# Psy-Fer/SquiggleKit

Hardware: AMD Instinct MI355X
Metric: reads/sec MotifSeq DTW (4k-sample read x 200-sample motif) (higher is better)
Workload: dtype f64 results; u32 fixed-point screening

## Files before the change

squigglekit_amd/csrc/sk_common.h:

```cpp
#pragma once
#include <hip/hip_runtime.h>
#include <stdint.h>
#include <stddef.h>
#include <stdarg.h>
#include <vector>
#include "squigglekit_hip.h"

#define SK_MAX_DEVICES 16
#define SK_WAVE 64

struct sk_prep {
    int32_t n;
    int32_t flags;
    double  center;
    double  scale;
    double  top;
    double  bot;
};

#define SK_IFLAG_INPLACE 0x100
#define SK_FLAG_PUBLIC   0xff

enum sk_prep_mode { SK_PREP_MEDMAD = 0, SK_PREP_ZSCALE = 1, SK_PREP_SEGMENT = 2, SK_PREP_DRNA = 3 };

enum sk_redo_route { SK_REDO_NONE = 0, SK_REDO_I16 = 1, SK_REDO_F64 = 2, SK_REDO_PA = 3 };

struct sk_buf {
    void  *p = nullptr;
    size_t cap = 0;
};

struct sk_panel_motif {
    int32_t xoff;
    int32_t P;
    int32_t k;
    int32_t pad;
};
struct sk_panel_group {
    int32_t L, R;
    int32_t first, count;
};

struct sk_pair_entry {
    int64_t toff;
    int64_t xoff;
    int32_t n;
    int32_t P;
    int32_t pair;
    int32_t pad;
};
struct sk_pair_query {
    int64_t src, xoff;
    int32_t N, L, R, pad;
};

struct sk_map_entry {
    int64_t toff;
    int64_t xoff;
    int64_t soff;
    int32_t n;
    int32_t P;
    int32_t rec;
    int32_t cont;
};

struct sk_rowhit_entry {
    int64_t col0;
    int64_t list;
    int32_t n;
    int32_t flags;
};
#define SK_ROWHIT_NOROW 0x100

struct sk_pairpath_entry {
    int64_t qoff, toff;
    int64_t span_off;
    int32_t N, M;
};

struct sk_band_entry {
    int64_t qoff, toff;
    int64_t span_off;
    int32_t N, M;
    int32_t pair, pad;
};

struct sk_ctx {
    int         device = -1;
    bool        ready = false;
    hipStream_t stream = nullptr;
    hipStream_t stream2 = nullptr;
    hipStream_t stream3 = nullptr;
    hipEvent_t  ev_r[2] = {nullptr, nullptr};
    hipStream_t stream4 = nullptr;
    hipEvent_t  ev_a = nullptr;
    hipEvent_t  ev_s[2] = {nullptr, nullptr};
    uint32_t    dtw_sparse_calls = 0;
    uint32_t    dtw_audit_calls = 0;
    hipEvent_t  ev_chunk[9] = {};
    hipEvent_t  ev[4] = {nullptr, nullptr, nullptr, nullptr};
    bool        ev_valid = false;
    int         num_cu = 0;
    sk_buf sig;
    sk_buf len;
    sk_buf rlen;
    sk_buf off;
    sk_buf comp;
    sk_buf prep;
    sk_buf mask;
    sk_buf motif;
    sk_buf out;
    sk_buf out2;
    sk_buf misc;
    sk_buf seghints;
    sk_buf pacal;
    sk_buf pull;
    sk_buf pulltext;
    sk_buf sweep;
    sk_buf sweeprec;
    sk_buf hitrows;
    sk_buf bgrec;
    sk_buf pathcnt;
    bool   path_valid = false;
    sk_buf pathlist;
    sk_buf pathscratch;
    sk_buf pathmotif;
    sk_buf pathspans;
    sk_buf events;
    sk_buf poolev;
    sk_buf pool;
    sk_buf panel;
    sk_buf panelwin;
    sk_buf panelaux;
    sk_buf panelrec;
    sk_buf seglev;
    sk_buf seglevwork;
    sk_buf detect;
    sk_buf detectout;
    sk_buf hmm;
    sk_buf hmmpath;
    sk_buf hmmseg;
    sk_buf hmmpost;
    sk_buf hmmpostout;
    std::vector<double> panel_host;
    std::vector<sk_panel_motif> panel_table;
    std::vector<sk_panel_group> panel_groups;
    std::vector<int32_t> panel_long;
    sk_buf pairs;
    sk_buf pairsval;
    std::vector<sk_pair_query> pairs_query;
    std::vector<sk_pair_entry> pairs_table;
    sk_buf rowhit;
    std::vector<sk_rowhit_entry> rowhit_table;
    std::vector<sk_map_entry>    pairhits_sweep;
    int64_t pairhits_row_bytes = 0, pairhits_slices = 0, pairhits_long_rows = 0;
    sk_buf pairpath;
    std::vector<sk_pairpath_entry> pairpath_table;
    int64_t pairpath_listed = 0, pairpath_slab_bytes = 0, pairpath_waves = 0;
    sk_buf band;
    sk_buf bandslab;
    std::vector<sk_band_entry> band_table;
    int64_t band_slab_bytes = 0, band_waves = 0, band_steps = 0;
    sk_buf ckpt;
    sk_buf motifq;
    sk_buf motif64;
    bool   motif64_valid = false;
    std::vector<double> motif64_host;
    sk_buf lastq;
    sk_buf qflag;
    sk_buf wsoft;
    sk_buf lsum;
    sk_buf wstate;
    sk_buf wrec;
    sk_buf wrecq;
    sk_buf order;
    sk_buf motifw;
    std::vector<double> motifw_host;
    int    motifq_L = 0;
    sk_buf retry;
    sk_buf dtwcnt;
    sk_buf audit;
    sk_buf sib;
    sk_buf sibout;
    sk_buf sibstate;
    bool   retry_dev = false;
    std::vector<unsigned> motifq_host;
    bool   motifq_valid = false;
    sk_buf redo;
    int    redo_route = SK_REDO_NONE;
    std::vector<size_t> redo_off;
    size_t redo_used = 0;
    std::vector<int64_t> pa_off_host;
    int    last_retry = 0;
    std::vector<hipEvent_t> evpool;
    int    prof_chunks = 0;
    int    prof_reads[64] = {0};
    std::vector<double> motif_host;
    std::vector<double> motif_src;
    int    motif_L = 0;
    void  *comm = nullptr;
    void  *sessions[SK_STREAM_MAX_SESSIONS] = {};
    void  *map_sessions[SK_MAP_MAX_SESSIONS] = {};
    int64_t map_state_bytes = 0, map_entries = 0, map_launches = 0;
    void  *evs_sessions[SK_EVS_MAX_SESSIONS] = {};
    sk_buf evscnt;
    int64_t evs_state_bytes = 0, evs_staged = 0;
    bool   evs_valid = false;
    void  *hmms_sessions[SK_HMMS_MAX_SESSIONS] = {};
    sk_buf hmmscnt;
    int64_t hmms_state_bytes = 0;
    bool   hmms_valid = false;
    void  *live_sessions[SK_LIVE_MAX_SESSIONS] = {};
    int64_t live_state_bytes = 0, live_levels = 0, live_launches = 0;
    sk_buf commbuf;
    sk_buf pile;
    sk_buf pileent;
    sk_buf pilealt;
    sk_buf pilein;
    sk_buf pileout;
    int64_t pile_entries = 0, pile_longest = 0, pile_long_lists = 0, pile_scratch_bytes = 0;
};

const char *sk_tune(const char *name);

struct sk_entry {
    sk_ctx *c = nullptr;
    sk_entry();
    explicit sk_entry(int slot);
    ~sk_entry();
    sk_entry(const sk_entry &) = delete;
    sk_entry &operator=(const sk_entry &) = delete;
};
#define SK_ENTER(c)                                                                     \
    sk_entry c##_entry_;                                                                \
    sk_ctx *const c = c##_entry_.c;                                                     \
    if (!c) return SK_ERR_NO_DEVICE
sk_ctx *sk_ctx_of(int device);
int  sk_bound_device(void);
int  sk_fail(int code, const char *fmt, ...);
int  sk_reserve(sk_ctx *c, sk_buf *b, size_t bytes);
int  sk_second_stream(sk_ctx *c);
int64_t sk_dtw_chunk_reads(size_t per_read, int64_t nreads);
void    sk_dtw_scratch_shrink(int reset);
#define SK_HIP(call)                                                                    \
    do {                                                                                \
        hipError_t e_ = (call);                                                         \
        if (e_ != hipSuccess)                                                           \
            return sk_fail(SK_ERR_HIP, "%s failed: %s (%s:%d)", #call,                 \
                           hipGetErrorString(e_), __FILE__, __LINE__);                  \
    } while (0)

int sk_launch_prep_i16(sk_ctx *c, const int16_t *d_sig, int64_t stride, const int32_t *d_len,
                       int32_t nreads, int32_t lo, int32_t hi, int mode, double std_scale,
                       int16_t *d_comp, sk_prep *d_prep, uint64_t *d_mask, int64_t mask_stride,
                       int32_t t0 = 0, int32_t t1 = 0x7fffffff,
                       const int32_t *d_list = nullptr, const int32_t *d_count = nullptr,
                       void *d_mask2 = nullptr, int row16 = 0);
int sk_launch_prepw_medmad(sk_ctx *c, const int16_t *d_sig, int64_t stride, const int32_t *d_len,
                           int32_t nreads, int32_t lo, int32_t hi, int16_t *d_comp, sk_prep *d_prep);
int sk_launch_prep_f64(sk_ctx *c, const double *d_sig, const int64_t *d_off, int32_t nreads,
                       double lo, double hi, int mode, double std_scale,
                       double *d_comp, sk_prep *d_prep, void *d_mask2 = nullptr, int row16 = 0,
                       int32_t *d_len_out = nullptr,
                       const int32_t *d_rlen = nullptr);

enum sk_feed { SK_FEED_I16 = 0,
               SK_FEED_F64_NORM = 1,
               SK_FEED_F64_RAW = 2 };
struct sk_prep_fuse {
    const int16_t *raw = nullptr;
    const int32_t *len = nullptr;
    int32_t lo = 0, hi = 0;
    int     mode = SK_PREP_MEDMAD;
};
bool sk_sdtw_fuse_ok(int32_t lo, int32_t hi, int mode = SK_PREP_MEDMAD, int64_t stride = 0);

struct sk_sdtw_args {
    int           feed;
    const void   *samples;
    int64_t       stride;
    const int64_t *off;
    const sk_prep *prep;
    int32_t       nreads;
    const double *motif;
    int32_t       nmotif;
    sk_hit       *out;
    double       *last_row;
    int64_t       max_len;
    int           force_single;
    int           accumulate = 0;
    const void   *samples_raw = nullptr;
    const sk_prep_fuse *fuse = nullptr;
};
int sk_launch_sdtw(sk_ctx *c, const sk_sdtw_args *a);
void sk_exact_shape(int N, int64_t count, int *L, int *R);
int sk_launch_sdtw_panel(sk_ctx *c, const sk_sdtw_args *a, int L, int R, const double *d_xlay, const sk_panel_motif *d_mt,
                         int32_t count, sk_hit *d_all, int64_t out_stride);
int sk_launch_sdtw_pairs(sk_ctx *c, int L, int R, int global, const double *d_values, const double *d_xlay,
                         const sk_pair_entry *d_pt, int32_t count, sk_hit *d_out);
int sk_launch_sdtw_map(sk_ctx *c, int L, int R, const double *d_targets, const double *d_xlay, const sk_map_entry *d_mp,
                       int32_t count, double *stD, int32_t *stS, sk_hit *d_last);
int sk_launch_pairs_layout(sk_ctx *c, const double *d_values, const sk_pair_query *d_qt, int nq, double *d_lay);
int sk_pairs_check(const int64_t *off, int32_t nseq, const sk_pair *pairs, int64_t npairs, int32_t mode, const void *out);
int sk_pairs_run(sk_ctx *c, const double *d_values, const int64_t *off, int64_t off0, int32_t nseq, const sk_pair *pairs,
                 int64_t npairs, int32_t mode, sk_hit *d_out);
int sk_pair_paths_run(sk_ctx *c, const double *d_values, const int64_t *off, int64_t off0, int32_t nseq, const sk_pair *pairs,
                      int64_t npairs, int32_t mode, sk_hit *d_rec, int32_t have_records, int32_t *d_spans);
int sk_launch_sdtw_rows(sk_ctx *c, const sk_sdtw_args *a, double *rowD, int32_t *rowS);
int sk_launch_hits_select(sk_ctx *c, const double *rowD, const int32_t *rowS, int64_t row_stride, const sk_hit *rec,
                          int32_t nreads, int32_t K, double max_dist, sk_hit *out, int32_t *count);
int sk_rowhits_reserve(sk_ctx *c, int64_t nrows);
int sk_launch_rowhits(sk_ctx *c, sk_rowhit_entry *tab, int64_t at, int32_t nrows, const double *rowD, const int32_t *rowS,
                      int32_t K, double max_dist, sk_hit *out, int32_t *count, int64_t *long_rows);
int sk_pairs_hits_run(sk_ctx *c, const double *d_values, const int64_t *off, int64_t off0, int32_t nseq, const sk_pair *pairs,
                      int64_t npairs, int32_t K, double max_dist, sk_hit *d_out, int32_t *d_count);
int sk_launch_row_background(sk_ctx *c, const double *rowD, int64_t row_stride, const sk_hit *rec, int32_t nreads,
                             sk_bg_rec *out);
struct sk_path_args {
    int            feed;
    const void    *samples;
    const void    *samples_raw = nullptr;
    int64_t        stride = 0;
    const int64_t *off = nullptr;
    const sk_prep *prep = nullptr;
    int32_t        nreads = 0;
    int64_t        max_len = 0;
    const double  *d_motif = nullptr;
    int32_t        nmotif = 0;
    const sk_hit  *hits = nullptr;
    int32_t        K = 1;
    int32_t       *spans = nullptr;
};
int sk_path_begin(sk_ctx *c);
int sk_launch_paths(sk_ctx *c, const sk_path_args *p);
int sk_launch_events(sk_ctx *c, const sk_path_args *p, sk_event *events);
int sk_launch_events_pool(sk_ctx *c, const sk_event *d_ev, const uint8_t *d_use, int64_t nhits, int32_t N,
                          int32_t *d_idx, int32_t *d_cnt, sk_pool_rec *d_out);
int sk_launch_sdtw_screen(sk_ctx *c, const sk_sdtw_args *a, int ck, int span, int span2,
                          int32_t *d_retry_cnt, int32_t *d_retry, int32_t *d_early_cnt, int32_t *d_early);

int sk_band_check(const int64_t *off, int32_t nseq, const sk_pair *pairs, int64_t npairs, int32_t band, int32_t end_mode,
                  const void *out);
int sk_band_run(sk_ctx *c, const double *d_values, const int64_t *off, int64_t off0, int32_t nseq, const sk_pair *pairs,
                int64_t npairs, int32_t band, int32_t end_mode, sk_hit *d_rec, int32_t *d_spans);

__host__ __device__ static inline void sk_slice_indices(int32_t len, int32_t begin, int32_t end, int32_t *lo, int32_t *hi, int *clamped = nullptr)
{
    int64_t s = begin, e = end;
    int cl = 0;
    if (s < 0) { s += len; if (s < 0) { s = 0; cl |= 1; } } else if (s > len) { s = len; cl |= 1; }
    if (e < 0) { e += len; if (e < 0) { e = 0; cl |= 2; } } else if (e > len) { e = len; cl |= 2; }
    *lo = (int32_t)s; *hi = (int32_t)e;
    if (clamped) *clamped = cl;
}
int sk_launch_region_rows_i16(sk_ctx *c, const int16_t *d_sig, int64_t stride, const int32_t *d_len, int32_t nreads,
                              int32_t begin, int32_t end, const int32_t *d_win, int16_t *d_rows, int64_t wstride,
                              int32_t *d_wlen, int32_t *d_from);
int sk_launch_region_rows_f64(sk_ctx *c, const double *d_sig, const int64_t *d_src, const int64_t *d_woff, int32_t nreads,
                              double *d_out);
int sk_panel_plan(sk_ctx *c, const double *motifs, const int32_t *motif_off, int32_t nmotifs, const double *mean,
                  const double *sd, int64_t pairs);
int sk_launch_panel_dtw(sk_ctx *c, const sk_sdtw_args *base, const double *motifs, const int32_t *motif_off,
                        sk_hit *d_all, int64_t out_stride);
int sk_launch_panel_rank(sk_ctx *c, const sk_hit *d_all, int64_t out_stride, int32_t nreads, int32_t nmotifs,
                         sk_panel_rec *d_out);

struct sk_roll_params;
bool sk_roll_stream_ok(int64_t stride, int32_t w, int32_t lo, int32_t hi);
int sk_launch_roll_stream(sk_ctx *c, const int16_t *d_sig, int64_t stride, const int32_t *d_len, int32_t nreads, int32_t lo,
                          int32_t hi, int32_t w, double std_scale, sk_prep *d_prep, uint64_t *d_below, uint64_t *d_above,
                          int32_t *d_redo );
size_t sk_roll_one_lds(int64_t stride, int32_t w);
int sk_launch_roll_one(sk_ctx *c, const int16_t *d_sig, int64_t stride, const int32_t *d_len, int32_t nreads, int32_t lo,
                       int32_t hi, int32_t w, double std_scale, sk_prep *d_prep, uint64_t *d_below, uint64_t *d_above);
int sk_launch_roll_stats(sk_ctx *c, const int16_t *d_comp, int64_t stride, sk_prep *d_prep, int32_t nreads,
                         int32_t w, double std_scale, int64_t *d_psum, uint64_t *d_below, uint64_t *d_above);
int sk_launch_roll_walk(sk_ctx *c, const uint64_t *d_below, const uint64_t *d_above, const sk_prep *d_prep,
                        int32_t nreads, const sk_roll_params *p, int32_t *d_xy, int32_t *d_found, int64_t row_words = 0);

int  sk_segment_fast_row16(int64_t stride);
bool sk_segment_fast_applies(const void *d_sig, int64_t stride, int32_t lo, int32_t hi, double std_scale);
int  sk_launch_segment_fast(sk_ctx *c, const int16_t *d_sig, int64_t stride, const int32_t *d_len, int32_t nreads,
                            const sk_seg_params *p, int32_t lo, int32_t hi, sk_prep *d_prep, void *d_mask2,
                            int32_t *d_retry, int32_t *d_segs, int32_t *d_nsegs, int32_t max_segs,
                            const double *d_cal = nullptr, double *d_scratch = nullptr);
bool sk_segment_pa_applies(const void *d_sig, int64_t stride, double std_scale);
int  sk_launch_prep_pa_listed(sk_ctx *c, const int16_t *d_sig, int64_t stride, const int32_t *d_len, const double *d_cal,
                              const int32_t *d_list, const int32_t *d_count, int grid, double lo, double hi, double std_scale,
                              double *d_scratch, int64_t scratch_stride, sk_prep *d_prep, void *d_mask2, int row16);

int  sk_launch_segment_masks(sk_ctx *c, const int16_t *d_sig, int64_t stride, const int32_t *d_len, int32_t nreads,
                             double std_scale, int32_t lo, int32_t hi, sk_prep *d_prep, void *d_mask2, int32_t *d_retry);

struct sk_sweep_lane {
    int32_t error, corrector, window, seg_dist, first_len, stall_start, gap_dist, index;
};
struct sk_sweep_group {
    int32_t rep, first, nfast, ngen;
};
void sk_sweep_plan(const sk_seg_sweep_set *sets, int32_t nsets, std::vector<sk_sweep_group> &groups,
                   std::vector<sk_sweep_lane> &lanes);
int  sk_launch_seg_sweep_walk(sk_ctx *c, const void *d_mask2, int row16, const int32_t *d_len, int64_t mmax, int32_t nreads,
                              const sk_sweep_lane *d_lanes, int32_t nlanes, bool fast, sk_seg_sweep_sum *d_sums,
                              sk_seg_sweep_rec *d_recs, int64_t rec_stride);

struct sk_drna_params;
int sk_launch_drna_walk(sk_ctx *c, const uint64_t *d_mask, int64_t mask_rows, const sk_prep *d_prep,
                        int32_t nreads, const sk_drna_params *p, int32_t *d_segs, int32_t *d_nsegs,
                        int32_t max_segs);

int sk_launch_synth(sk_ctx *c, int16_t *d_sig, int64_t stride, int32_t nreads, int32_t nsamples,
                    uint64_t seed, const int16_t *d_motif_i16, int32_t nmotif, int64_t row0 = 0,
                    int hit_pm = 500, int stretch_pm = 0, int stretch = 1);
int sk_launch_synth_windows(sk_ctx *c, int16_t *d_sig, int64_t stride, int32_t nreads, int32_t nsamples,
                            uint64_t seed, int64_t row0, const int16_t *d_tmpl, int32_t ntmpl, float sigma);
int sk_launch_raw_to_pa(sk_ctx *c, const int16_t *d_sig, int64_t stride, int32_t nreads, int32_t nsamples,
                        double offset, double raw_unit, double *d_out, int64_t *d_off);
int sk_launch_centi_to_f64(sk_ctx *c, const int32_t *d_centi, int64_t total, double *d_out);
int sk_launch_rows_to_pa(sk_ctx *c, const int16_t *d_sig, int64_t stride, int32_t nreads, const int64_t *d_off,
                         const double *d_cal, double *d_out);

bool sk_f64_fast_applies(int64_t maxlen, double std_scale);
int  sk_f64_row16(int64_t maxlen);
int  sk_launch_f64_stats(sk_ctx *c, const double *d_sig, const int64_t *d_off, const int32_t *d_rlen, int32_t nreads, int64_t maxlen,
                         double lo, double hi, int mode, double std_scale, sk_prep *d_prep, void *d_mask2, int row16,
                         int32_t *d_len, int32_t *d_retry, double *d_comp);
int  sk_launch_prep_f64_listed(sk_ctx *c, const double *d_sig, const int64_t *d_off, const int32_t *d_list,
                               const int32_t *d_count, int grid, double lo, double hi, int mode, double std_scale,
                               double *d_comp_or_scratch, int64_t scratch_stride, sk_prep *d_prep, void *d_mask2,
                               int row16, const int32_t *d_rlen = nullptr);
int  sk_launch_seg_walk_masks(sk_ctx *c, const void *d_mask2, int row16, const int32_t *d_len, int32_t nreads,
                              const sk_seg_params *p, int32_t *d_segs, int32_t *d_nsegs, int32_t max_segs);

size_t sk_seglev_work_bytes(sk_ctx *c, int32_t nreads, int32_t max_segs, int64_t mmax);
int sk_launch_seg_levels(sk_ctx *c, int feed, const void *samples, int64_t stride, const int64_t *d_off,
                         const void *d_mask2, int row16, const int32_t *d_len, int64_t mmax, int32_t nreads,
                         const int32_t *d_segs, const int32_t *d_nsegs, int32_t max_segs, void *d_work,
                         sk_seg_level *levels, sk_seg_level *read_level);

int64_t sk_detect_words(int64_t stride);
size_t  sk_detect_work_bytes(int32_t nreads, int64_t stride);
int sk_launch_detect_mark(sk_ctx *c, const int16_t *d_sig, int64_t stride, const int32_t *d_len, int32_t nreads,
                          const sk_det_params *p, void *d_words, int64_t *d_cnt);
int sk_launch_detect_scan(sk_ctx *c, int32_t nreads, int64_t *d_bsum, int64_t *d_off);
int sk_launch_detect_fill(sk_ctx *c, const int16_t *d_sig, int64_t stride, const int32_t *d_len, int32_t nreads,
                          const sk_det_params *p, const void *d_words, const int64_t *d_off, sk_det_event *d_rec, int64_t cap);

__host__ __device__ static inline double sk_raw_to_pa(double raw, double offset, double unit)
{
    const double x = raw + offset;
    return x * unit;
}
const char *sk_hmm_model_error(const sk_hmm_model *m);
int sk_launch_hmm_i16(sk_ctx *c, const int16_t *d_sig, int64_t stride, const int32_t *d_len, int32_t nreads,
                      const double *d_cal, const sk_hmm_model *m, int32_t limit, sk_hmm_rec *d_rec);
int sk_launch_hmm_f64(sk_ctx *c, const double *d_values, const int64_t *d_off, int32_t nreads, const sk_hmm_model *m,
                      int32_t limit, sk_hmm_rec *d_rec);
int64_t sk_hmm_npad(int64_t maxlen, int32_t limit);
int64_t sk_hmm_slice_groups(int32_t nreads, int64_t npad);
size_t  sk_hmm_path_work_bytes(int32_t nreads, int64_t npad);
int sk_launch_hmm_paths(sk_ctx *c, int feed, const void *d_sig, int64_t stride, const int32_t *d_len, const int64_t *d_roff,
                        int32_t nreads, const double *d_cal, const sk_hmm_model *m, int32_t limit, int64_t npad, void *d_work,
                        int first, sk_hmm_rec *d_rec, int64_t *d_off, sk_hmm_seg *d_seg, int64_t cap);
int sk_launch_hmm_stats(sk_ctx *c, int feed, const void *d_sig, int64_t stride, const int64_t *d_roff, int32_t nreads,
                        const double *d_cal, const sk_hmm_model *m, const int64_t *d_off, void *d_seg, int64_t cap);

size_t sk_hmm_post_work_bytes(int32_t nreads, int64_t npad);
int sk_launch_hmm_post(sk_ctx *c, int feed, const void *d_sig, int64_t stride, const int32_t *d_len, const int64_t *d_roff,
                       int32_t nreads, const double *d_cal, const sk_hmm_model *m, int32_t limit, int64_t npad, void *d_work,
                       sk_hmm_post *d_post, sk_hmm_counts *d_counts, const int64_t *d_goff, double *d_gamma);

int sk_stream_session_open(sk_ctx *c, const double *motifs, const int32_t *motif_off, int32_t nmotifs,
                           const sk_stream_params *p, int32_t *handle);
int sk_stream_session_info(sk_ctx *c, int32_t handle, int32_t *nslots, int32_t *nmotifs);
int sk_stream_session_push(sk_ctx *c, int32_t handle, const int32_t *d_slots, int32_t m, const int16_t *d_rows,
                           int64_t stride, const int32_t *d_len, int flush, sk_stream_rec *d_out);
int sk_stream_session_reset(sk_ctx *c, int32_t handle, const int32_t *d_slots, int32_t m, const double *d_center,
                            const double *d_scale);
int sk_stream_session_stage(sk_ctx *c, int32_t handle, int which, size_t bytes, void **p);
int sk_stream_session_close(sk_ctx *c, int32_t handle);
void sk_stream_close_all(sk_ctx *c);

int sk_map_session_open(sk_ctx *c, const double *targets, const int64_t *target_off, int32_t ntargets, int32_t nslots,
                        int32_t *handle);
int sk_map_session_info(sk_ctx *c, int32_t handle, int32_t *nslots, int32_t *ntargets);
int sk_map_session_check_slots(sk_ctx *c, int32_t handle, const int32_t *slots, int32_t m);
int sk_map_session_push(sk_ctx *c, int32_t handle, const int32_t *slots, int32_t m, const double *d_values,
                        const int64_t *off, sk_map_rec *d_out);
int sk_map_session_reset(sk_ctx *c, int32_t handle, const int32_t *slots, int32_t m);
int sk_map_session_hits(sk_ctx *c, int32_t handle, const int32_t *slots, int32_t m, int32_t K, double max_dist, sk_hit *d_out,
                        int32_t *d_count);
int sk_map_session_stage(sk_ctx *c, int32_t handle, int which, size_t bytes, void **p);
int sk_map_session_close(sk_ctx *c, int32_t handle);
void sk_map_close_all(sk_ctx *c);

int64_t sk_evs_session_rows(sk_ctx *c, int32_t handle, int64_t maxlen);
int sk_evs_session_open(sk_ctx *c, const sk_det_params *p, int32_t nslots, int32_t *handle);
int sk_evs_session_info(sk_ctx *c, int32_t handle, int32_t *nslots);
int sk_evs_session_check(sk_ctx *c, int32_t handle, const int32_t *slots, int32_t m, const int32_t *len);
int sk_evs_session_check_cap(sk_ctx *c, int32_t handle, const int32_t *slots, int32_t m, const int32_t *len, int64_t cap);
int sk_evs_session_stage(sk_ctx *c, int32_t handle, int which, size_t bytes, void **p);
int sk_evs_session_push(sk_ctx *c, int32_t handle, const int32_t *d_slots, int32_t m, const int16_t *d_rows, int64_t stride,
                        const int32_t *d_len, const int32_t *d_end, int64_t per, int64_t *d_off, const int32_t *host_slots,
                        const int32_t *host_len, const int32_t *host_end);
int sk_evs_session_gather(sk_ctx *c, int32_t handle, sk_det_event *d_rec, int64_t cap);
int sk_evs_session_last(sk_ctx *c, int32_t handle, const int64_t **d_off, int32_t *m);
int sk_evs_session_staging(sk_ctx *c, int32_t handle, const sk_det_event **d_stage, int64_t *per);
int sk_evs_session_reset(sk_ctx *c, int32_t handle, const int32_t *slots, int32_t m);
int sk_evs_session_close(sk_ctx *c, int32_t handle);
void sk_evs_close_all(sk_ctx *c);

#define SK_HMMS_CAP 0x7fffff00
void sk_hmms_close_all(sk_ctx *c);
int sk_hmms_session_open(sk_ctx *c, const sk_hmm_model *model, int32_t nslots, int32_t *handle);
int sk_hmms_session_push_dev_i16(sk_ctx *c, int32_t handle, const int32_t *d_slots, int32_t m, const int16_t *d_rows,
                                 int64_t stride, const int32_t *d_len, sk_hmms_rec *d_out);
int sk_hmms_session_reset_dev(sk_ctx *c, int32_t handle, const int32_t *d_slots, int32_t m, const double *d_cal2);
int64_t sk_hmms_session_bytes(sk_ctx *c, int32_t handle);
int sk_hmms_session_close(sk_ctx *c, int32_t handle);

int sk_live_session_open(sk_ctx *c, const sk_det_params *p, int32_t calib, const double *targets, const int64_t *target_off,
                         int32_t ntargets, int32_t nslots, const sk_hmm_model *model ,
                         const sk_live_gate *gate, int32_t *handle);
int sk_live_session_info(sk_ctx *c, int32_t handle, int32_t *nslots, int32_t *ntargets, int32_t *evs, int32_t *map);
int sk_live_session_gate_last(sk_ctx *c, int32_t handle, const sk_live_gate_info **d_gate, const sk_hmms_rec **d_rec, int32_t *m);
int sk_live_session_check(sk_ctx *c, int32_t handle, const int32_t *slots, int32_t m, int64_t stride, const int32_t *len);
int sk_live_session_stage(sk_ctx *c, int32_t handle, int which, size_t bytes, void **p);
int sk_live_session_push(sk_ctx *c, int32_t handle, const int32_t *host_slots, const int32_t *d_slots, int32_t m,
                         const int16_t *d_rows, int64_t stride, const int32_t *d_len, const int32_t *d_end, int64_t per,
                         const int32_t *host_len, const int32_t *host_end, const sk_live_rule *rule, sk_map_rec *d_out,
                         sk_live_info *d_info, sk_live_best *d_best);
int sk_live_session_last(sk_ctx *c, int32_t handle, const int64_t **d_off, const double **d_values, int32_t *m);
int sk_live_session_best_ms(sk_ctx *c, int32_t handle, float *ms);
int sk_live_session_gate_ms(sk_ctx *c, int32_t handle, float *hmm_ms, float *gate_ms);
int sk_live_session_reset(sk_ctx *c, int32_t handle, const int32_t *slots, int32_t m, const double *cal2 );
int sk_live_session_close(sk_ctx *c, int32_t handle);
void sk_live_close_all(sk_ctx *c);

struct sk_gate_slot {
    sk_live_gate_info g;
    int32_t last_drop;
    int32_t pad;
};
struct sk_gate_args {
    sk_gate_slot        *state;
    sk_det_event        *ring;
    const sk_live_info  *live;
    int32_t              nslots, G;
    const int32_t       *slots;
    int32_t              m;
    const int32_t       *len, *end;
    const sk_hmms_rec   *hrec;
    const sk_det_event  *stage;
    int64_t              per;
    const int64_t       *eoff;
    sk_det_event        *rel;
    int64_t             *rcnt;
    sk_live_gate_info   *ginfo;
    sk_live_gate         rule;
};
int sk_livegate_reset(sk_ctx *c, sk_gate_slot *state, int32_t nslots, const int32_t *d_slots, int32_t m);
int sk_livegate_lengths(sk_ctx *c, const sk_gate_args &a, int32_t *d_hlen);
int sk_livegate_release(sk_ctx *c, const sk_gate_args &a);

int sk_pileup_run(sk_ctx *c, const int64_t *d_span_off, const int32_t *d_spans, const double *d_value, const int32_t *d_dwell,
                  const int32_t *d_target, const int32_t *d_shift, const uint8_t *d_use, int32_t npairs, int64_t nrows,
                  const int64_t *tlen, int32_t ntargets, sk_pile_rec *d_out, int64_t *d_ent_off, int32_t *d_ent_row,
                  int64_t ent_cap);

int64_t sk_scan_blocks(int64_t n);
int     sk_launch_scan_i64(sk_ctx *c, const int64_t *v, int64_t n, int64_t *bsum, int64_t *out);
int64_t sk_pull_tile_cap(int32_t nreads, int64_t stride);
int sk_launch_pull_count(sk_ctx *c, const int16_t *d_sig, int64_t stride, const int32_t *d_len, int32_t nreads,
                         const double *d_cal, const int64_t *d_poff, int64_t *d_tile0, int64_t *d_tb, int64_t tile_cap,
                         int64_t *d_bsum, int64_t *d_line_off, int32_t *d_err);
int sk_launch_pull_write(sk_ctx *c, const int16_t *d_sig, int64_t stride, const int32_t *d_len, int32_t nreads,
                         const double *d_cal, const char *d_prefix, const int64_t *d_poff, const int64_t *d_tile0,
                         const int64_t *d_tb, int64_t tile_cap, const int64_t *d_line_off, char *d_out);
```

squigglekit_amd/csrc/sk_runtime.hip:

```cpp
#include "sk_common.h"
#include <string>
#include <string.h>
#include <mutex>
#include <stdio.h>
#include <stdlib.h>
#include <string.h>

static thread_local char  g_err[512] = "";
static thread_local int   g_cur = -1;
static sk_ctx             g_ctx[SK_MAX_DEVICES];
static std::mutex         g_mu;
static std::recursive_mutex g_ctx_mu[SK_MAX_DEVICES];

int sk_fail(int code, const char *fmt, ...)
{
    va_list ap;
    va_start(ap, fmt);
    vsnprintf(g_err, sizeof g_err, fmt, ap);
    va_end(ap);
    return code;
}

sk_entry::sk_entry() : sk_entry(g_cur) {}

sk_entry::sk_entry(int slot)
{
    if (slot >= 0 && slot < SK_MAX_DEVICES) {
        g_ctx_mu[slot].lock();
        sk_ctx *ctx = &g_ctx[slot];
        if (ctx->ready) {
            if (hipSetDevice(ctx->device) == hipSuccess) { c = ctx; return; }
            sk_fail(SK_ERR_NO_DEVICE, "hipSetDevice(%d) failed", ctx->device);
            g_ctx_mu[slot].unlock();
            return;
        }
        g_ctx_mu[slot].unlock();
    }
    sk_fail(SK_ERR_NO_DEVICE, "no device bound: call sk_init(device) first (no CPU fallback exists)");
}

sk_entry::~sk_entry() { if (c) g_ctx_mu[c - g_ctx].unlock(); }

sk_ctx *sk_ctx_of(int device) { return (device >= 0 && device < SK_MAX_DEVICES) ? &g_ctx[device] : nullptr; }
int sk_bound_device(void) { return g_cur; }

int sk_reserve(sk_ctx *c, sk_buf *b, size_t bytes)
{
    (void)c;
    if (bytes <= b->cap) return SK_OK;
    if (b->p) { SK_HIP(hipFree(b->p)); b->p = nullptr; b->cap = 0; }
    size_t want = bytes + bytes / 8 + 256;
    hipError_t e = hipMalloc(&b->p, want);
    if (e != hipSuccess) {
        b->p = nullptr;
        return sk_fail(SK_ERR_NOMEM, "hipMalloc(%zu) failed: %s", want, hipGetErrorString(e));
    }
    b->cap = want;
    return SK_OK;
}

int sk_second_stream(sk_ctx *c)
{
    if (!c->stream2) {
        SK_HIP(hipStreamCreateWithFlags(&c->stream2, hipStreamNonBlocking));
        for (int i = 0; i < 9; i++) SK_HIP(hipEventCreateWithFlags(&c->ev_chunk[i], hipEventDisableTiming));
    }
    return SK_OK;
}

struct sk_tunable { const char *name, *test_values, *what; };
static const sk_tunable SK_TUNABLES[] = {
    {"SK_DTW_SCHEME",         "full exact2", "DTW scheme: full = one exact pass, exact2 = two exact passes (default: fixed-point screening + certified window)"},
    {"SK_DTW_QL",             "8 16 64",     "lanes per read of the screening scheme (default: by motif length and batch size)"},
    {"SK_DTW_NOFUSE",         "1",           "filter + medmad as their own kernel instead of the screening pass's prologue"},
    {"SK_DTW_FORCE_RETRY_PM", "100 1000",    "per-mille of reads sent through the exact retry whatever the window pass certified (sensitivity runs)"},
    {"SK_DTW_SPAN",           "150 300",     "look-back of the window pass in columns (one tier)"},
    {"SK_DTW_SPAN2",          "0 500",       "look-back of the window pass's second tier (0: none)"},
    {"SK_DTW_CK",             "64 256",      "steps between checkpoints of the screening pass (multiple of 64)"},
    {"SK_DTW_NOSORT",         "1",           "window passes take the reads in file order"},
    {"SK_DTW_NOHINT",         "1",           "no start hint: the plain screening sweep, every read's exact window looks back the same number of columns"},
    {"SK_DTW_HINT_MIN",       "1",           "the start hint is on for calls of at least this many reads (default 500000)"},
    {"SK_DTW_SORT_MIN",       "1",           "window passes sort chunks of at least this many reads"},
    {"SK_DTW_NO_EARLY",       "1",           "no early exact retry beside the window passes"},
    {"SK_DTW_NO_SIBLINGS",    "1",           "reads whose candidate columns fall into two clusters take the exact pass (no second window)"},
    {"SK_DTW_NOGUARD",        "1",           "screening scheme without its run-time guard (premise test in the window pass, audit, gated exact fallback): A/B cost runs"},
    {"SK_DTW_AUDIT_PERIOD",   "0 1 64",      "the audit re-runs one read in this many with the exact pass (default 4096; 0: no audit)"},
    {"SK_DTW_HOLE",           "qerr1 fma64 fma64x", "tests: a known precision hole put back (E = 1; the fma sample image for float64 reads, with / without the image-error guard) -- the guard has to notice and the records must not change"},
    {"SK_DTW_SCRATCH_MB",     "8 64",        "checkpoint scratch budget in MB (small values force many chunks)"},
    {"SK_DTW_NO_SMALL",       "1",           "small batches keep the batch lane layout"},
    {"SK_DTW_SMALL_MAX",      "0 100000",    "largest batch that spreads a read over 64 lanes"},
    {"SK_PREP_BLOCK",         "1",           "medmad statistics by the workgroup-per-read kernel"},
    {"SK_PREP_ROUNDS",        "1 3",         "grid rounds of the persistent statistics kernels"},
    {"SK_PREP_PERCU",         "1 2",         "workgroups per CU of the persistent statistics kernels"},
    {"SK_SEG_OLD",            "1",           "segmenter: numpy-order statistics kernels for every read"},
    {"SK_SEG_DELTA_SCALE",    "1e13",        "segmenter: certification margin multiplier (large: every read takes the numpy-order redo)"},
    {"SK_SEG_PA_F64",         "1",           "segmenter, raw reads through the pA conversion: expand to float64 and take the float64 kernels instead of the raw-domain kernel"},
    {"SK_SEG_NO_WG",          "1",           "segmenter, reads of 4 097 .. 65 536 samples: the wavefront-per-read statistics kernel (two looks at a read) instead of the workgroup-per-read one"},
    {"SK_SEG_WG_ALL",         "1",           "segmenter: the workgroup-per-read statistics kernel for every row of 4 097 .. 65 536 samples (default: where it is faster)"},
    {"SK_SEG_OCC",            "7 8",         "segmenter statistics kernel: waves per SIMD the registers are sized for"},
    {"SK_SEG_CHUNKS",         "2 8",         "segmenter: chunks of a large batch (walk of one beside the statistics of the next)"},
    {"SK_WALK_GENERAL",       "1",           "segmenter walk: general step (corrector test live)"},
    {"SK_WALK_SYNC",          "1",           "segmenter walk: run hopping with the 64 lanes of a wavefront on the same word (k_seg_walk3)"},
    {"SK_WALK_OWNPASS",       "1",           "segmenter walk: finds the quiet stretches and anchors in a pass of its own instead of taking the statistics kernel's hints"},
    {"SK_WALK_NOJUMP",        "1",           "segmenter walk: every run is hopped through, no jumps between the stretches of quiet entries"},
    {"SK_WALK_NOWAVE",        "1",           "segmenter walk: a lane per read also for long rows / small batches (no wavefront-per-read walk)"},
    {"SK_WALK_WAVE_MAXREADS", "0 1000000",   "segmenter walk: batches of up to this many reads take the wavefront-per-read walk (default: 16384, 131072 for rows beyond 4 096 samples)"},
    {"SK_DRNA_STEP",          "1",           "dRNA_segmenter, both branches: the per-sample scans instead of the scans by runs / by transitions"},
    {"SK_ROLL_TWO_KERNELS",   "1",           "dRNA_segmenter rolling-mean branch: filter kernel + prefix sums through HBM instead of the one-look kernel (prefix sums in LDS)"},
    {"SK_ROLL_ONE_LOOK",      "1",           "dRNA_segmenter rolling-mean branch: the workgroup-per-read kernel in numpy's order for every read instead of the streaming kernel with certified thresholds"},
    {"SK_ROLL_DELTA_SCALE",   "1e13",        "dRNA_segmenter rolling-mean branch: multiplier of the certification margin (large: every read is redone in numpy's order)"},
    {"SK_HITS_ROW_BYTES",     "1000000",     "hit lists: bytes of the last-row buffer (12 B per column and read; default 2 GiB; small values force many chunks of reads)"},
    {"SK_ROWHITS_ONE_WAVE",   "1",           "pair / session hit lists: rows beyond 4 096 columns through one wavefront each instead of a workgroup of 16 (A/B runs)"},
    {"SK_PANEL_EXACT",        "1",           "motif panel: the one-grid exact kernel also for long windows over many reads (default: those take the screening scheme, one launch set per motif)"},
    {"SK_PATH_LDS_BYTES",     "0",           "alignment paths: bytes of direction words a hit may keep in LDS (default and most 25600; 0: every hit takes the scratch tier)"},
    {"SK_PATH_SCRATCH_BYTES", "1000000",     "alignment paths: byte budget of the scratch tier's slabs (default 1 GiB; small values leave one wavefront)"},
    {"SK_BAND_WAVES",         "1",           "adaptive-band DTW: wavefronts of the launch (default: one per pair up to what the device holds at a time and the slab budget; 1: one wavefront with one slab works through the list)"},
    {"SK_PILE_LDS_ENTRIES",   "64",          "reference pile-up: entries of a point's list that are put in order inside one wavefront's LDS (default and most 4096, at least 2; longer lists take the merge tier)"},
    {"SK_INGEST_MB",          "1 4",        "sub-batch size of the host entry points in MB"},
    {"SK_HMM_SCRATCH_MB",     "1",           "signal HMM state paths and posteriors: scratch budget in MB (default 16384; small values force slices of one or two 64-read groups)"},
    {"SK_HMM_POST_BLOCK",     "256",         "signal HMM posteriors: samples between alpha checkpoints, a multiple of 128 (default 128)"},
    {"SK_F64_OLD",            "1",           "float64 reads: numpy-order statistics kernel for every read"},
    {"SK_F64_LONG_LOOKS",     "1",           "float64 reads of 4 097 .. 40 960 samples: the window-by-window kernel (three to five looks at a read) instead of the workgroup-per-read one (one look)"},
};

const char *sk_tune(const char *name)
{
    const char *on = getenv("SK_TUNING");
    if (!on || on[0] != '1') return nullptr;
    for (const sk_tunable &t : SK_TUNABLES)
        if (strcmp(t.name, name) == 0) return getenv(name);
    return nullptr;
}

static thread_local int g_dtw_shrink = 0;
void sk_dtw_scratch_shrink(int reset) { g_dtw_shrink = reset ? 0 : (g_dtw_shrink < 12 ? g_dtw_shrink + 1 : 12); }

int64_t sk_dtw_chunk_reads(size_t per_read, int64_t nreads)
{
    size_t budget = (size_t)64 << 30;
    int64_t floor_reads = 1024;
    if (const char *e = sk_tune("SK_DTW_SCRATCH_MB")) {
        const long v = atol(e);
        if (v > 0) { budget = (size_t)v << 20; floor_reads = 64; }
    }
    budget >>= g_dtw_shrink;
    int64_t chunk = (int64_t)(budget / (per_read ? per_read : 1));
    if (chunk < floor_reads) chunk = floor_reads;
    if (chunk > nreads) chunk = nreads;
    return chunk > 0 ? chunk : 1;
}

extern "C" {

int sk_tunables(char *buf, int cap)
{
    std::string out;
    for (const sk_tunable &t : SK_TUNABLES) { out += t.name; out += '\t'; out += t.test_values; out += '\t'; out += t.what; out += '\n'; }
    if (buf && cap > 0) { const size_t n = out.size() < (size_t)cap - 1 ? out.size() : (size_t)cap - 1; memcpy(buf, out.data(), n); buf[n] = 0; }
    return (int)out.size() + 1;
}

const char *sk_version(void) { return "squigglekit-hip 0.1.0 (gfx950)"; }
const char *sk_last_error(void) { return g_err; }

int sk_device_count(void)
{
    int n = 0;
    hipError_t e = hipGetDeviceCount(&n);
    if (e != hipSuccess) {
        sk_fail(SK_ERR_NO_DEVICE, "hipGetDeviceCount: %s", hipGetErrorString(e));
        return 0;
    }
    return n;
}

int sk_init(int device) { return sk_init_slot(device, device); }

int sk_init_slot(int slot, int device)
{
    int n = sk_device_count();
    if (n <= 0) return sk_fail(SK_ERR_NO_DEVICE, "no HIP device visible (this library has no CPU fallback)");
    if (device < 0 || device >= n || device >= SK_MAX_DEVICES)
        return sk_fail(SK_ERR_INVALID, "device %d out of range (0..%d)", device, n - 1);
    if (slot < 0 || slot >= SK_MAX_DEVICES)
        return sk_fail(SK_ERR_INVALID, "context slot %d out of range (0..%d)", slot, SK_MAX_DEVICES - 1);
    std::lock_guard<std::mutex> lk(g_mu);
    sk_ctx *c = &g_ctx[slot];
    std::lock_guard<std::recursive_mutex> c_lock(g_ctx_mu[slot]);
    if (c->ready && c->device != device)
        return sk_fail(SK_ERR_INVALID, "context slot %d already serves device %d", slot, c->device);
    SK_HIP(hipSetDevice(device));
    if (!c->ready) {
        hipDeviceProp_t prop;
        SK_HIP(hipGetDeviceProperties(&prop, device));
        if (strncmp(prop.gcnArchName, "gfx950", 6) != 0)
            return sk_fail(SK_ERR_NO_DEVICE, "device %d is %s; this build targets gfx950 only",
                           device, prop.gcnArchName);
        c->device = device;
        c->num_cu = prop.multiProcessorCount;
        SK_HIP(hipStreamCreateWithFlags(&c->stream, hipStreamNonBlocking));
        for (int i = 0; i < 4; i++) SK_HIP(hipEventCreate(&c->ev[i]));
        c->ready = true;
    }
    g_cur = slot;
    return SK_OK;
}

static void free_buf(sk_buf *b) { if (b->p) (void)hipFree(b->p); b->p = nullptr; b->cap = 0; }

int sk_shutdown(void)
{
    std::lock_guard<std::mutex> lk(g_mu);
    for (int d = 0; d < SK_MAX_DEVICES; d++) {
        sk_ctx *c = &g_ctx[d];
        std::lock_guard<std::recursive_mutex> c_lock(g_ctx_mu[d]);
        if (!c->ready) continue;
        (void)hipSetDevice(c->device);
        (void)hipStreamSynchronize(c->stream);
        sk_stream_close_all(c);
        sk_live_close_all(c);
        sk_map_close_all(c);
        sk_evs_close_all(c);
        sk_hmms_close_all(c);
        sk_buf *bufs[] = {&c->sig, &c->len, &c->off, &c->comp, &c->prep, &c->mask,
                          &c->motif, &c->out, &c->out2, &c->misc, &c->ckpt, &c->retry, &c->motifq, &c->lastq, &c->qflag,
                          &c->motif64, &c->commbuf, &c->dtwcnt, &c->wsoft, &c->wstate, &c->wrec, &c->motifw, &c->lsum, &c->wrecq, &c->order, &c->pacal, &c->seghints, &c->audit, &c->rlen, &c->redo, &c->sib, &c->sibout, &c->sibstate, &c->pull, &c->pulltext, &c->sweep, &c->sweeprec, &c->hitrows, &c->bgrec, &c->pathcnt, &c->pathlist, &c->pathscratch, &c->pathmotif, &c->pathspans, &c->events, &c->poolev, &c->pool, &c->panel, &c->panelwin, &c->panelaux, &c->panelrec, &c->seglev, &c->seglevwork, &c->detect, &c->detectout, &c->hmm, &c->hmmpath, &c->hmmseg, &c->hmmpost, &c->hmmpostout, &c->pairs, &c->pairsval, &c->pairpath, &c->rowhit, &c->band, &c->bandslab, &c->evscnt, &c->hmmscnt,
                          &c->pile, &c->pileent, &c->pilealt, &c->pilein, &c->pileout};
        for (sk_buf *b : bufs) free_buf(b);
        for (int i = 0; i < 4; i++) (void)hipEventDestroy(c->ev[i]);
        for (hipEvent_t e : c->evpool) (void)hipEventDestroy(e);
        if (c->stream2) {
            (void)hipStreamSynchronize(c->stream2);
            for (int i = 0; i < 9; i++) if (c->ev_chunk[i]) (void)hipEventDestroy(c->ev_chunk[i]);
            (void)hipStreamDestroy(c->stream2);
        }
        if (c->stream3) {
            (void)hipStreamSynchronize(c->stream3);
            for (int i = 0; i < 2; i++) if (c->ev_r[i]) (void)hipEventDestroy(c->ev_r[i]);
            (void)hipStreamDestroy(c->stream3);
        }
        for (int i = 0; i < 2; i++) if (c->ev_s[i]) (void)hipEventDestroy(c->ev_s[i]);
        if (c->stream4) {
            (void)hipStreamSynchronize(c->stream4);
            if (c->ev_a) (void)hipEventDestroy(c->ev_a);
            (void)hipStreamDestroy(c->stream4);
        }
        (void)hipStreamDestroy(c->stream);
        *c = sk_ctx();
    }
    g_cur = -1;
    return SK_OK;
}

int sk_sync(void)
{
    SK_ENTER(c);
    SK_HIP(hipStreamSynchronize(c->stream));
    return SK_OK;
}

int sk_device_name(char *buf, int cap)
{
    SK_ENTER(c);
    if (!buf || cap <= 0) return sk_fail(SK_ERR_INVALID, "bad buffer");
    hipDeviceProp_t prop;
    SK_HIP(hipGetDeviceProperties(&prop, c->device));
    snprintf(buf, (size_t)cap, "%s (%s, %d CUs)", prop.name, prop.gcnArchName, prop.multiProcessorCount);
    return SK_OK;
}

int sk_device_pci_bus_id(char *buf, int cap)
{
    SK_ENTER(c);
    if (!buf || cap < 16) return sk_fail(SK_ERR_INVALID, "bad buffer");
    SK_HIP(hipDeviceGetPCIBusId(buf, cap, c->device));
    return SK_OK;
}

void *sk_dev_alloc(size_t bytes)
{
    sk_entry entry;
    if (!entry.c) return nullptr;
    void *p = nullptr;
    hipError_t e = hipMalloc(&p, bytes ? bytes : 1);
    if (e != hipSuccess) {
        sk_fail(SK_ERR_NOMEM, "hipMalloc(%zu) failed: %s", bytes, hipGetErrorString(e));
        return nullptr;
    }
    return p;
}

int sk_dev_free(void *dptr)
{
    SK_ENTER(c);
    if (dptr) SK_HIP(hipFree(dptr));
    return SK_OK;
}

int sk_dev_upload(void *dst_dev, const void *src_host, size_t bytes)
{
    SK_ENTER(c);
    if (bytes && (!dst_dev || !src_host)) return sk_fail(SK_ERR_INVALID, "NULL pointer");
    SK_HIP(hipMemcpyAsync(dst_dev, src_host, bytes, hipMemcpyHostToDevice, c->stream));
    SK_HIP(hipStreamSynchronize(c->stream));
    return SK_OK;
}

int sk_dev_download(void *dst_host, const void *src_dev, size_t bytes)
{
    SK_ENTER(c);
    if (bytes && (!dst_host || !src_dev)) return sk_fail(SK_ERR_INVALID, "NULL pointer");
    SK_HIP(hipMemcpyAsync(dst_host, src_dev, bytes, hipMemcpyDeviceToHost, c->stream));
    SK_HIP(hipStreamSynchronize(c->stream));
    return SK_OK;
}

int sk_last_kernel_ms(float *prep_ms, float *main_ms)
{
    SK_ENTER(c);
    if (!c->ev_valid) return sk_fail(SK_ERR_INVALID, "no timed call yet");
    SK_HIP(hipEventSynchronize(c->ev[3]));
    float a = 0.f, b = 0.f;
    SK_HIP(hipEventElapsedTime(&a, c->ev[0], c->ev[1]));
    SK_HIP(hipEventElapsedTime(&b, c->ev[2], c->ev[3]));
    if (prep_ms) *prep_ms = a;
    if (main_ms) *main_ms = b;
    return SK_OK;
}

int sk_last_dtw_profile(float *dist_ms, int *dist_launches, float *start_ms, int *start_launches,
                        int *reads_per_launch)
{
    SK_ENTER(c);
    float a = 0.f, b = 0.f;
    int mx = 0;
    for (int i = 0; i < c->prof_chunks; i++) {
        hipEvent_t *ev = &c->evpool[3 * (size_t)i];
        SK_HIP(hipEventSynchronize(ev[2]));
        float t = 0.f;
        SK_HIP(hipEventElapsedTime(&t, ev[0], ev[1])); a += t;
        SK_HIP(hipEventElapsedTime(&t, ev[1], ev[2])); b += t;
        const int rr = c->prof_reads[i < 64 ? i : 63];
        if (rr > mx) mx = rr;
    }
    if (dist_ms) *dist_ms = a;
    if (start_ms) *start_ms = b;
    if (dist_launches) *dist_launches = c->prof_chunks;
    if (start_launches) *start_launches = c->prof_chunks;
    if (reads_per_launch) *reads_per_launch = mx;
    return SK_OK;
}

int sk_last_dtw_retries(void)
{
    SK_ENTER(c);
    if (c->retry_dev && c->dtwcnt.p) {
        int32_t n = 0;
        if (hipMemcpyAsync(&n, c->dtwcnt.p, sizeof n, hipMemcpyDeviceToHost, c->stream) != hipSuccess ||
            hipStreamSynchronize(c->stream) != hipSuccess)
            return sk_fail(SK_ERR_HIP, "reading the retry count failed");
        c->last_retry = n;
    }
    return c->last_retry;
}

int sk_last_dtw_clock(double *ghz)
{
    SK_ENTER(c);
    if (!ghz) return sk_fail(SK_ERR_INVALID, "NULL pointer");
    *ghz = 0.0;
    if (!(c->retry_dev && c->dtwcnt.p)) return SK_OK;
    unsigned long long t[2] = {0, 0};
    if (hipMemcpyAsync(t, (const char *)c->dtwcnt.p + 16, sizeof t, hipMemcpyDeviceToHost, c->stream) != hipSuccess ||
        hipStreamSynchronize(c->stream) != hipSuccess)
        return sk_fail(SK_ERR_HIP, "reading the clock sample failed");
    if (t[1]) *ghz = (double)t[0] / ((double)t[1] / 100e6) / 1e9;
    return SK_OK;
}

int sk_last_dtw_guard(int32_t *out)
{
    SK_ENTER(c);
    if (!out) return sk_fail(SK_ERR_INVALID, "NULL pointer");
    memset(out, 0, 8 * sizeof(int32_t));
    if (!(c->retry_dev && c->dtwcnt.p)) return SK_OK;
    if (hipMemcpyAsync(out, (const int32_t *)c->dtwcnt.p + 8, 8 * sizeof(int32_t), hipMemcpyDeviceToHost, c->stream) != hipSuccess ||
        hipStreamSynchronize(c->stream) != hipSuccess)
        return sk_fail(SK_ERR_HIP, "reading the guard counters failed");
    return SK_OK;
}

int sk_last_dtw_premise_violations(void)
{
    int32_t g[8];
    const int rc = sk_last_dtw_guard(g);
    return rc ? rc : g[0];
}

int sk_last_dtw_audit_mismatches(void)
{
    int32_t g[8];
    const int rc = sk_last_dtw_guard(g);
    return rc ? rc : g[2];
}

int sk_last_dtw_window_steps(uint64_t *out)
{
    SK_ENTER(c);
    if (!out) return sk_fail(SK_ERR_INVALID, "NULL pointer");
    out[0] = out[1] = 0;
    if (!(c->retry_dev && c->dtwcnt.p && c->dtwcnt.cap >= 128)) return SK_OK;
    if (hipMemcpyAsync(out, (const char *)c->dtwcnt.p + 64, 16, hipMemcpyDeviceToHost, c->stream) != hipSuccess ||
        hipStreamSynchronize(c->stream) != hipSuccess)
        return sk_fail(SK_ERR_HIP, "reading the window-step counters failed");
    return SK_OK;
}

int sk_last_dtw_tier2(void)
{
    SK_ENTER(c);
    if (!(c->retry_dev && c->dtwcnt.p)) return 0;
    int32_t n = 0;
    if (hipMemcpyAsync(&n, (const int32_t *)c->dtwcnt.p + 1, sizeof n, hipMemcpyDeviceToHost, c->stream) != hipSuccess ||
        hipStreamSynchronize(c->stream) != hipSuccess)
        return sk_fail(SK_ERR_HIP, "reading the second-tier count failed");
    return n;
}

}
```

squigglekit_amd/csrc/sk_sdtw.hip:

```cpp
#include "sk_sdtw_dev.h"
#include <math.h>
#include <stdlib.h>
#include <string.h>
#include <vector>

namespace {

template <int L, int R, int FEED, int MODE>
__global__ __launch_bounds__(256)
void k_sdtw(const sdtw_kargs a)
{
    static_assert(L == 16 || L == 64, "lanes per read");
    constexpr int G = 64 / L;
    constexpr int SHR = (L == 16) ? DPP_ROW_SHR1 : DPP_WAVE_SHR1;
    constexpr int ROL = (L == 16) ? DPP_ROW_ROL1 : DPP_WAVE_ROL1;
    constexpr bool PAIRS = (MODE == MODE_PAIRS || MODE == MODE_PAIRS_GLOBAL);
    constexpr bool GLOBAL = (MODE == MODE_PAIRS_GLOBAL);
    constexpr bool MAPC = (MODE == MODE_PAIRS_CHAIN);
    static_assert(!(PAIRS || MAPC) || FEED == SK_FEED_F64_RAW, "pair lists take the pool as given");
    constexpr bool TRACK = (MODE != MODE_DIST && !GLOBAL);
    constexpr int CKW = R + 3;
    const double INF = __builtin_huge_val();

    const int lane = threadIdx.x & 63;
    const int wave = blockIdx.x * (blockDim.x >> 6) + (threadIdx.x >> 6);
    const int g = lane / L, l = lane % L;
    int slot = wave * G + g;
    int nreads = a.nreads;
    if constexpr (MODE != MODE_PANEL && !PAIRS && !MAPC) {
        if (a.gate_ptr) {
            if (*a.gate_ptr == 0) return;
            if (a.guard && blockIdx.x == 0 && threadIdx.x == 0) a.guard[SK_GUARD_FELLBACK] = 1;
        }
        if (a.count_ptr) {
            const int cnt = *a.count_ptr;
            if (a.total_ptr && blockIdx.x == 0 && threadIdx.x == 0) atomicAdd(a.total_ptr, cnt);
            nreads = min(cnt - a.list_off, a.nreads);
            if (nreads <= 0) return;
        }
    }
    const bool live = slot < nreads;
    if (!live) slot = nreads - 1;
    int r;
    if constexpr (MODE == MODE_PANEL || PAIRS || MAPC) r = slot;
    else r = a.ridx ? a.ridx[a.list_off + slot] : a.read0 + slot;
    sk_panel_motif mt = {};
    if constexpr (MODE == MODE_PANEL) mt = a.mt[blockIdx.y];
    sk_pair_entry pe = {};
    if constexpr (PAIRS) pe = a.pt[r];
    sk_map_entry me = {};
    if constexpr (MAPC) me = a.mp[r];

    int n, flags = 0;
    double center = 0.0, scale = 1.0, rc1 = 0.0, rc2 = 0.0;
    const int16_t *s16 = nullptr;
    const double  *s64 = nullptr;
    if constexpr (FEED == SK_FEED_I16) {
        const sk_prep pr = a.prep[r];
        n = pr.n; flags = pr.flags & SK_FLAG_PUBLIC; center = pr.center; scale = pr.scale;
        s16 = (const int16_t *)a.samples + (int64_t)r * a.stride;
    } else if constexpr (FEED == SK_FEED_F64_NORM) {
        const sk_prep pr = a.prep[r];
        n = pr.n; flags = pr.flags & SK_FLAG_PUBLIC; center = pr.center; scale = pr.scale;
        rc1 = pr.top; rc2 = pr.bot;
        s64 = (const double *)(((pr.flags & SK_IFLAG_INPLACE) && a.samples_raw) ? a.samples_raw : a.samples) + a.off[r];
    } else if constexpr (PAIRS) {
        n = pe.n;
        if (n == 0) flags = SK_FLAG_EMPTY;
        s64 = (const double *)a.samples + pe.toff;
    } else if constexpr (MAPC) {
        n = me.n;
        s64 = (const double *)a.samples + me.toff;
    } else {
        n = (int)(a.off[r + 1] - a.off[r]);
        if (n == 0) flags = SK_FLAG_EMPTY;
        s64 = (const double *)a.samples + a.off[r];
    }
    if (!live) n = 0;

    int tbase = 0, tlast = n - 1 + L - 1, end = -1, c0 = 0;
    if (n <= 0) tlast = -1;
    if constexpr (MODE == MODE_START) {
        end = a.out[r].end;
        if (n > 0 && end >= 0) {
            c0 = max(0, end - a.span) / a.ck;
            if (c0 > a.nck) c0 = a.nck;
            tbase = c0 * a.ck;
            tlast = end + L - 1;
        } else {
            tlast = -1;
        }
    }
    int nsteps = tlast - tbase + 1;
    if (nsteps < 0) nsteps = 0;
#pragma unroll
    for (int d = L; d < 64; d <<= 1) nsteps = max(nsteps, __shfl_xor(nsteps, d));
    nsteps = __builtin_amdgcn_readfirstlane(nsteps);
    const int nblk = (nsteps + L - 1) / L;

    double x[R];
#pragma unroll
    for (int k = 0; k < R; k++) {
        if constexpr (MODE == MODE_PANEL) x[k] = a.xlay[mt.xoff + l * R + k];
        else if constexpr (PAIRS) x[k] = a.xlay[pe.xoff + l * R + k];
        else if constexpr (MAPC) x[k] = a.xlay[me.xoff + l * R + k];
        else x[k] = a.xlay[l * R + k];
    }
    const bool shortlane = l < (MODE == MODE_PANEL ? mt.P : PAIRS ? pe.P : MAPC ? me.P : a.P);

    double D[R];
    int    S[R];
#pragma unroll
    for (int k = 0; k < R; k++) { D[k] = INF; S[k] = -1; }
    double botD = (R == 1 && l == 0 && shortlane) ? 0.0 : INF;
    int    botS = (R == 1 && l == 0 && shortlane) ? 0 : -1;
    double diagD = (l == 0) ? 0.0 : INF;
    int    diagS = (l == 0) ? tbase : -1;
    bool chained = false;
    const double *pD = nullptr;  const int32_t *pS = nullptr;
    double PFD = 0.0;  int PFS = 0;
    if constexpr (MODE == MODE_CHAIN) {
        chained = a.prevD != nullptr;
        if (chained) {
            pD = a.prevD + (int64_t)(r - a.read0) * a.row_stride;
            pS = a.prevS + (int64_t)(r - a.read0) * a.row_stride;
            if (l == 0) { diagD = INF; diagS = -1; }
            if (R == 1 && l == 0 && shortlane) { botD = INF; botS = -1; }
            PFD = (l < n) ? pD[l] : INF;
            PFS = (l < n) ? pS[l] : -1;
        }
    }
    if constexpr (MAPC) {
        chained = me.cont != 0;
        if (chained) {
            pD = a.rowD + me.soff;
            pS = a.rowS + me.soff;
            if (l == 0) { diagD = INF; diagS = -1; }
            if (R == 1 && l == 0 && shortlane) { botD = INF; botS = -1; }
            PFD = (l < n) ? pD[l] : INF;
            PFS = (l < n) ? pS[l] : -1;
        }
    }
    double y = INF;
    double best = INF;  int bestS = -1, bestJ = -1;

    if constexpr (MODE == MODE_START) {
        if (c0 > 0) {
            const double *cp = a.ckpt + (((int64_t)(r - a.read0) * a.nck + (c0 - 1)) * L + l) * CKW;
#pragma unroll
            for (int k = 0; k < R; k++) D[k] = cp[k];
            y = cp[R]; botD = cp[R + 1]; diagD = cp[R + 2];
        }
    }

    auto fetch = [&](int idx) -> double {
        if constexpr (FEED == SK_FEED_I16) {
            int16_t raw = (idx < n) ? s16[idx] : (int16_t)0;
            double v = ((double)raw - center) / scale;
            return (idx < n) ? v : INF;
        } else if constexpr (FEED == SK_FEED_F64_NORM) {
            double raw = (idx < n) ? s64[idx] : 0.0;
            double v = ((raw - center) - rc1) / scale - rc2;
            return (idx < n) ? v : INF;
        } else {
            return (idx < n) ? s64[idx] : INF;
        }
    };

    double F = fetch(tbase + l);
    for (int blk = 0; blk < nblk; blk++) {
        const double Fnext = fetch(tbase + (blk + 1) * L + l);
        double PFDn = 0.0;  int PFSn = 0;
        if constexpr (MODE == MODE_CHAIN || MAPC) {
            if (chained) {
                const int idx = tbase + (blk + 1) * L + l;
                PFDn = (idx < n) ? pD[idx] : INF;
                PFSn = (idx < n) ? pS[idx] : -1;
            }
        }
        if constexpr (MODE == MODE_DIST) {
            const int t0 = blk * L;
            if (t0 > 0 && (t0 % a.ck) == 0 && t0 / a.ck <= a.nck && live) {
                double *cp = a.ckpt + (((int64_t)(r - a.read0) * a.nck + (t0 / a.ck - 1)) * L + l) * CKW;
#pragma unroll
                for (int k = 0; k < R; k++) cp[k] = D[k];
                cp[R] = y; cp[R + 1] = botD; cp[R + 2] = diagD;
            }
        }
#pragma unroll 2
        for (int q = 0; q < L; q++) {
            const int t = tbase + blk * L + q;
            y = dpp_f64<SHR>(F, y);
            F = dpp_f64<ROL>(F, F);
            double topD = 0.0;  int topS = t + 1;
            if constexpr (GLOBAL) topD = INF;
            if constexpr (MODE == MODE_CHAIN || MAPC) {
                if (chained) { topD = PFD; topS = PFS; }
                PFD = dpp_f64<ROL>(PFD, PFD);
                PFS = dpp_i32<ROL>(PFS, PFS);
            }
            const double upD = dpp_f64<SHR>(topD, botD);
            int upS = 0;
            if constexpr (TRACK) upS = dpp_i32<SHR>(topS, botS);
            double dgD = diagD;  int dgS = diagS;
            double uD = upD;     int uS = upS;
#pragma unroll
            for (int k = 0; k < R; k++) {
                const double lfD = D[k];
                const double c = fabs(x[k] - y);
                double nd;
                if constexpr (TRACK) {
                    const int lfS = S[k];
                    const bool lt1 = lfD < dgD;
                    double m1;
                    if constexpr (FEED == SK_FEED_I16) m1 = vmin(lfD, dgD); else m1 = lt1 ? lfD : dgD;
                    const int    s1 = lt1 ? lfS : dgS;
                    const bool lt2 = uD < m1;
                    double m;
                    if constexpr (FEED == SK_FEED_I16) m = vmin(uD, m1); else m = lt2 ? uD : m1;
                    const int    s = lt2 ? uS : s1;
                    nd = c + m;
                    dgS = lfS;  S[k] = s;  uS = s;
                } else {
                    nd = c + vmin(vmin(dgD, lfD), uD);
                }
                dgD = lfD;
                D[k] = nd;
                uD = nd;
            }
            diagD = upD;  diagS = upS;
            if constexpr (R >= 2) {
                botD = shortlane ? D[R - 2] : D[R - 1];
                if constexpr (TRACK) botS = shortlane ? S[R - 2] : S[R - 1];
            } else {
                botD = shortlane ? upD : D[0];
                if constexpr (TRACK) botS = shortlane ? upS : S[0];
            }
            const int j = t - l;
            if constexpr (MODE == MODE_START) {
                if (j == end) bestS = S[R - 1];
            } else if constexpr (GLOBAL) {
                if (j == n - 1) best = D[R - 1];
            } else {
                if (D[R - 1] < best) {
                    best = D[R - 1]; bestJ = j;
                    if constexpr (TRACK) bestS = S[R - 1];
                }
                if constexpr (MODE == MODE_FULL || MODE == MODE_CHAIN) {
                    if (a.last_row != nullptr) {
                        if (l == L - 1 && slot == 0 && j >= 0 && j < n) a.last_row[j] = D[R - 1];
                    }
                }
                if constexpr (MODE == MODE_CHAIN || MODE == MODE_ROWS) {
                    if (a.rowD != nullptr && live && l == L - 1 && j >= 0 && j < n) {
                        a.rowD[(int64_t)(r - a.read0) * a.row_stride + j] = D[R - 1];
                        a.rowS[(int64_t)(r - a.read0) * a.row_stride + j] = S[R - 1];
                    }
                }
                if constexpr (MAPC) {
                    if (live && l == L - 1 && j >= 0 && j < n) {
                        a.rowD[me.soff + j] = D[R - 1];
                        a.rowS[me.soff + j] = S[R - 1];
                    }
                }
            }
        }
        F = Fnext;
        if constexpr (MODE == MODE_CHAIN || MAPC) { PFD = PFDn; PFS = PFSn; }
    }

    if (live && l == L - 1) {
        if constexpr (MODE == MODE_START) {
            if (n > 0 && end >= 0) {
                if (bestS >= 0) a.out[r].start = bestS;
                else a.retry[atomicAdd(a.retry_cnt, 1)] = r;
            }
        } else {
            sk_hit h;
            if (n > 0) { h.dist = best; h.start = GLOBAL ? 0 : bestS; h.end = GLOBAL ? n - 1 : bestJ; }
            else       { h.dist = __builtin_nan(""); h.start = -1; h.end = -1; }
            h.n = n;
            h.flags = flags;
            if constexpr (MODE == MODE_PANEL) a.out[(int64_t)mt.k * a.out_stride + r] = h;
            else if constexpr (PAIRS) a.out[pe.pair] = h;
            else if constexpr (MAPC) a.out[me.rec] = h;
            else a.out[a.out_by_slot ? a.list_off + slot : r] = h;
        }
    }
}

__global__ void k_audit_pick(int32_t *list, int naudit, int period, int nreads, unsigned salt)
{
    const int s = blockIdx.x * blockDim.x + threadIdx.x;
    if (s == 0) { list[0] = naudit; list[1] = 0; }
    if (s >= naudit) return;
    const int64_t base = (int64_t)s * period;
    const int span = (int)min((int64_t)period, (int64_t)nreads - base);
    unsigned h = (unsigned)s * 2654435761u + 0x9E3779B9u;
    h ^= salt * 0x9E3779B9u;
    h ^= h >> 15; h *= 0x85EBCA6Bu; h ^= h >> 13;
    list[2 + s] = (int)(base + (int64_t)(h % (unsigned)span));
}

__global__ void k_audit_compare(const int32_t *list, const sk_hit *exact, sk_hit *out, int naudit, int32_t *guard)
{
    const int s = blockIdx.x * blockDim.x + threadIdx.x;
    if (s >= naudit) return;
    const int r = list[2 + s];
    const sk_hit e = exact[s], g = out[r];
    const bool same_d = (__double_as_longlong(e.dist) == __double_as_longlong(g.dist)) || (e.dist != e.dist && g.dist != g.dist);
    if (same_d && e.start == g.start && e.end == g.end && e.n == g.n) return;
    out[r] = e;
    atomicAdd(&guard[SK_GUARD_MISMATCH], 1);
    atomicAdd(&guard[SK_GUARD_ALARM], 1);
}

static void sk_audit_pick(int32_t *list, int naudit, int period, int nreads, unsigned salt, hipStream_t st)
{
    hipLaunchKernelGGL(k_audit_pick, dim3((naudit + 255) / 256), dim3(256), 0, st, list, naudit, period, nreads, salt);
}
static void sk_audit_compare(const int32_t *list, const sk_hit *exact, sk_hit *out, int naudit, int32_t *guard, hipStream_t st)
{
    hipLaunchKernelGGL(k_audit_compare, dim3((naudit + 255) / 256), dim3(256), 0, st, list, exact, out, naudit, guard);
}

typedef void (*sdtw_fn)(const sdtw_kargs);

template <int L, int FEED, int MODE>
sdtw_fn pick_r(int R)
{
#define SK_KERNEL(RR) k_sdtw<L, RR, FEED, MODE>
    switch (R) { SK_R_CASES_1_16(SK_KERNEL) }
#undef SK_KERNEL
    return nullptr;
}

template <int FEED>
sdtw_fn pick(int L, int R, int mode)
{
    if (L == 16) {
        if (mode == MODE_FULL) return pick_r<16, FEED, MODE_FULL>(R);
        if (mode == MODE_DIST) return pick_r<16, FEED, MODE_DIST>(R);
        if (mode == MODE_ROWS) return pick_r<16, FEED, MODE_ROWS>(R);
        return pick_r<16, FEED, MODE_START>(R);
    }
    if (mode == MODE_FULL) return pick_r<64, FEED, MODE_FULL>(R);
    if (mode == MODE_ROWS) return pick_r<64, FEED, MODE_ROWS>(R);
    if (mode == MODE_DIST) return pick_r<64, FEED, MODE_DIST>(R);
    if (mode == MODE_CHAIN) return pick_r<64, FEED, MODE_CHAIN>(R);
    return pick_r<64, FEED, MODE_START>(R);
}

sdtw_fn pick_any(int feed, int L, int R, int mode)
{
    switch (feed) {
        case SK_FEED_I16:      return pick<SK_FEED_I16>(L, R, mode);
        case SK_FEED_F64_NORM: return pick<SK_FEED_F64_NORM>(L, R, mode);
        case SK_FEED_F64_RAW:  return pick<SK_FEED_F64_RAW>(L, R, mode);
    }
    return nullptr;
}

int launch(sk_ctx *c, sdtw_fn fn, const sdtw_kargs &k, int L, hipStream_t stream = nullptr)
{
    if (k.nreads <= 0) return SK_OK;
    const int reads_per_block = 4 * (64 / L);
    const int grid = (k.nreads + reads_per_block - 1) / reads_per_block;
    hipLaunchKernelGGL(fn, dim3(grid), dim3(256), 0, stream ? stream : c->stream, k);
    SK_HIP(hipGetLastError());
    return SK_OK;
}

}

static int launch_chained(sk_ctx *c, const sk_sdtw_args *a, double *finD = nullptr, int32_t *finS = nullptr)
{
    const int N = a->nmotif;
    const int CH = 64 * 16;
    const int nchunks = (N + CH - 1) / CH;
    std::vector<size_t> lay_off(nchunks);
    std::vector<int> Rc(nchunks), Pc(nchunks);
    size_t total = 0;
    for (int i = 0; i < nchunks; i++) {
        const int rows = (i + 1 < nchunks) ? CH : N - i * CH;
        Rc[i] = (rows + 63) / 64;
        Pc[i] = 64 * Rc[i] - rows;
        lay_off[i] = total;
        total += (size_t)64 * Rc[i];
    }
    const bool same = c->motif.p && c->motif_L == -1 && c->motif_src.size() == (size_t)N &&
                      memcmp(c->motif_src.data(), a->motif, (size_t)N * sizeof(double)) == 0;
    if (!same) {
        SK_HIP(hipStreamSynchronize(c->stream));
        c->motif_host.assign(total, 0.0);
        for (int i = 0; i < nchunks; i++)
            if (!sk_lane_layout(a->motif + (size_t)i * CH, 64 * Rc[i] - Pc[i], 64, Rc[i], &c->motif_host[lay_off[i]]))
                return sk_fail(SK_ERR_INVALID, "internal: motif layout mismatch");
        int rc = sk_reserve(c, &c->motif, total * sizeof(double));
        if (rc) return rc;
        SK_HIP(hipMemcpyAsync(c->motif.p, c->motif_host.data(), total * sizeof(double), hipMemcpyHostToDevice,
                              c->stream));
        c->motif_src.assign(a->motif, a->motif + N);
        c->motif_L = -1;
        c->motif64_valid = false;
        c->motifq_valid = false;
    }
    const int64_t row_stride = (a->max_len > 0 ? a->max_len : 1);
    const size_t per_read = (size_t)row_stride * 12 * 2;
    int64_t batch = (int64_t)(((size_t)6 << 30) / per_read);
    if (batch > a->nreads) batch = a->nreads;
    if (batch < 1) batch = 1;
    int rc = sk_reserve(c, &c->ckpt, (size_t)batch * per_read);
    if (rc) return rc;
    double  *bufD[2] = {(double *)c->ckpt.p, (double *)c->ckpt.p + (size_t)batch * row_stride};
    int32_t *bufS[2] = {(int32_t *)(bufD[1] + (size_t)batch * row_stride),
                        (int32_t *)(bufD[1] + (size_t)batch * row_stride) + (size_t)batch * row_stride};
    sdtw_kargs k = kargs_of(a);
    k.out = a->out; k.last_row = nullptr; k.row_stride = row_stride;
    c->last_retry = 0;
    c->retry_dev = false;
    c->prof_chunks = 0;
    SK_HIP(hipEventRecord(c->ev[2], c->stream));
    for (int64_t r0 = 0; r0 < a->nreads; r0 += batch) {
        k.read0 = (int)r0;
        k.nreads = (int)((a->nreads - r0 < batch) ? a->nreads - r0 : batch);
        for (int i = 0; i < nchunks; i++) {
            sdtw_fn fn = pick_any(a->feed, 64, Rc[i], MODE_CHAIN);
            if (!fn) return sk_fail(SK_ERR_UNSUPPORTED, "no chained kernel for R=%d", Rc[i]);
            k.xlay = (const double *)c->motif.p + lay_off[i];
            k.P = Pc[i];
            k.prevD = (i > 0) ? bufD[(i - 1) & 1] : nullptr;
            k.prevS = (i > 0) ? bufS[(i - 1) & 1] : nullptr;
            k.rowD = (i + 1 < nchunks) ? bufD[i & 1] : (finD ? finD + r0 * row_stride : nullptr);
            k.rowS = (i + 1 < nchunks) ? bufS[i & 1] : (finS ? finS + r0 * row_stride : nullptr);
            k.last_row = (i + 1 == nchunks && r0 == 0) ? a->last_row : nullptr;
            if ((rc = launch(c, fn, k, 64))) return rc;
        }
    }
    SK_HIP(hipEventRecord(c->ev[3], c->stream));
    return SK_OK;
}

bool sk_sdtw_fuse_ok(int32_t lo, int32_t hi, int mode, int64_t stride)
{
    if (sk_tune("SK_PREP_BLOCK") || sk_tune("SK_DTW_NOFUSE")) return false;
    if (mode == SK_PREP_ZSCALE) return stride > 0 && stride <= 4096 && hi > lo;
    const int64_t nbins = (int64_t)hi - lo - 1;
    return nbins > 1024 && nbins <= 1280;
}

static bool screens(const sk_sdtw_args *a, int span, int ck)
{
    const int N = a->nmotif;
    if (N > 64 * 16 || a->last_row || a->force_single || a->nreads < 256) return false;
    if (a->max_len < 4 * (int64_t)(span + ck)) return false;
    if (const char *e = sk_tune("SK_DTW_SCHEME")) if (strcmp(e, "full") == 0 || strcmp(e, "exact2") == 0) return false;
    for (int i = 0; i < N; i++) if (!(fabs(a->motif[i]) < QLIM)) return false;
    return true;
}

static int upload_layout(sk_ctx *c, const double *motif, int N, int L, int R)
{
    const bool same = c->motif.p && c->motif_L == L && c->motif_src.size() == (size_t)N &&
                      memcmp(c->motif_src.data(), motif, (size_t)N * sizeof(double)) == 0;
    if (!same) {
        SK_HIP(hipStreamSynchronize(c->stream));
        c->motif_host.resize((size_t)L * R);
        if (!sk_lane_layout(motif, N, L, R, c->motif_host.data()))
            return sk_fail(SK_ERR_INVALID, "internal: motif layout mismatch");
        int rc = sk_reserve(c, &c->motif, c->motif_host.size() * sizeof(double));
        if (rc) return rc;
        SK_HIP(hipMemcpyAsync(c->motif.p, c->motif_host.data(), c->motif_host.size() * sizeof(double),
                              hipMemcpyHostToDevice, c->stream));
        c->motif_src.assign(motif, motif + N);
        c->motif_L = L;
        c->motif64_valid = false;
        c->motifq_valid = false;
    }
    return SK_OK;
}

void sk_exact_shape(int N, int64_t count, int *L, int *R)
{
    if (N <= 16 * 16) { *L = 16; *R = (N + 15) / 16; }
    else              { *L = 64; *R = (N + 63) / 64; }
    int small_max = 2048;
    if (const char *e = sk_tune("SK_DTW_SMALL_MAX")) { int v = atoi(e); if (v >= 0) small_max = v; }
    if (*L == 16 && N >= 32 && count <= small_max && !sk_tune("SK_DTW_NO_SMALL")) { *L = 64; *R = (N + 63) / 64; }
}

int sk_launch_sdtw_rows(sk_ctx *c, const sk_sdtw_args *a, double *rowD, int32_t *rowS)
{
    const int N = a->nmotif;
    if (N <= 0) return sk_fail(SK_ERR_INVALID, "empty motif");
    if (a->nreads <= 0) return SK_OK;
    if (a->fuse) return sk_fail(SK_ERR_INVALID, "internal: fused prologue without a screening pass");
    if (N > 64 * 16) return launch_chained(c, a, rowD, rowS);
    int L, R;
    sk_exact_shape(N, a->nreads, &L, &R);
    int rc = upload_layout(c, a->motif, N, L, R);
    if (rc) return rc;
    sdtw_kargs k = kargs_of(a);
    k.nreads = a->nreads; k.read0 = 0; k.xlay = (const double *)c->motif.p; k.P = L * R - N;
    k.out = a->out; k.rowD = rowD; k.rowS = rowS; k.row_stride = a->max_len > 0 ? a->max_len : 1;
    sdtw_fn fn = pick_any(a->feed, L, R, MODE_ROWS);
    if (!fn) return sk_fail(SK_ERR_UNSUPPORTED, "no kernel for L=%d R=%d", L, R);
    return launch(c, fn, k, L);
}

int sk_launch_sdtw_panel(sk_ctx *c, const sk_sdtw_args *a, int L, int R, const double *d_xlay, const sk_panel_motif *d_mt,
                         int32_t count, sk_hit *d_all, int64_t out_stride)
{
    sdtw_fn fn = nullptr;
    if (a->feed == SK_FEED_I16)
        fn = L == 16 ? pick_r<16, SK_FEED_I16, MODE_PANEL>(R) : pick_r<64, SK_FEED_I16, MODE_PANEL>(R);
    else if (a->feed == SK_FEED_F64_NORM)
        fn = L == 16 ? pick_r<16, SK_FEED_F64_NORM, MODE_PANEL>(R) : pick_r<64, SK_FEED_F64_NORM, MODE_PANEL>(R);
    if (!fn) return sk_fail(SK_ERR_UNSUPPORTED, "no panel kernel for L=%d R=%d", L, R);
    sdtw_kargs k = kargs_of(a);
    k.nreads = a->nreads; k.xlay = d_xlay; k.mt = d_mt; k.out = d_all; k.out_stride = out_stride;
    const int reads_per_block = 4 * (64 / L);
    const dim3 grid((a->nreads + reads_per_block - 1) / reads_per_block, count);
    hipLaunchKernelGGL(fn, grid, dim3(256), 0, c->stream, k);
    SK_HIP(hipGetLastError());
    return SK_OK;
}

int sk_launch_sdtw_pairs(sk_ctx *c, int L, int R, int global, const double *d_values, const double *d_xlay,
                         const sk_pair_entry *d_pt, int32_t count, sk_hit *d_out)
{
    sdtw_fn fn;
    if (global) fn = L == 16 ? pick_r<16, SK_FEED_F64_RAW, MODE_PAIRS_GLOBAL>(R) : pick_r<64, SK_FEED_F64_RAW, MODE_PAIRS_GLOBAL>(R);
    else        fn = L == 16 ? pick_r<16, SK_FEED_F64_RAW, MODE_PAIRS>(R) : pick_r<64, SK_FEED_F64_RAW, MODE_PAIRS>(R);
    if (!fn || (L != 16 && L != 64)) return sk_fail(SK_ERR_UNSUPPORTED, "no pairs kernel for L=%d R=%d", L, R);
    sdtw_kargs k;
    memset(&k, 0, sizeof k);
    k.samples = d_values; k.nreads = count; k.xlay = d_xlay; k.pt = d_pt; k.out = d_out;
    return launch(c, fn, k, L);
}

int sk_launch_sdtw_map(sk_ctx *c, int L, int R, const double *d_targets, const double *d_xlay, const sk_map_entry *d_mp,
                       int32_t count, double *stD, int32_t *stS, sk_hit *d_last)
{
    sdtw_fn fn = L == 16 ? pick_r<16, SK_FEED_F64_RAW, MODE_PAIRS_CHAIN>(R) : pick_r<64, SK_FEED_F64_RAW, MODE_PAIRS_CHAIN>(R);
    if (!fn || (L != 16 && L != 64)) return sk_fail(SK_ERR_UNSUPPORTED, "no mapping-session kernel for L=%d R=%d", L, R);
    sdtw_kargs k;
    memset(&k, 0, sizeof k);
    k.samples = d_targets; k.nreads = count; k.xlay = d_xlay; k.mp = d_mp; k.rowD = stD; k.rowS = stS; k.out = d_last;
    return launch(c, fn, k, L);
}

int sk_launch_sdtw(sk_ctx *c, const sk_sdtw_args *a_in)
{
    const sk_sdtw_args *a = a_in;
    sk_sdtw_args a_unfused;
    const int N = a->nmotif;
    if (N <= 0) return sk_fail(SK_ERR_INVALID, "empty motif");
    if (a->nreads <= 0) return SK_OK;
    if (a->fuse) {
        int ck0 = 128, span0 = N + N / 8 + 8;
        if (const char *e = sk_tune("SK_DTW_CK")) { int v = atoi(e); if (v >= 64 && v % 64 == 0) ck0 = v; }
        if (const char *e = sk_tune("SK_DTW_SPAN")) { int v = atoi(e); if (v > 0) span0 = v; }
        if (!screens(a, span0, ck0) || !sk_sdtw_fuse_ok(a->fuse->lo, a->fuse->hi, a->fuse->mode, a->stride)) {
            SK_HIP(hipEventRecord(c->ev[0], c->stream));
            int rc0 = sk_launch_prep_i16(c, a->fuse->raw, a->stride, a->fuse->len, a->nreads, a->fuse->lo, a->fuse->hi,
                                         a->fuse->mode, 0.0, (int16_t *)a->samples, (sk_prep *)a->prep, nullptr, 0);
            if (rc0) return rc0;
            SK_HIP(hipEventRecord(c->ev[1], c->stream));
            a_unfused = *a;
            a_unfused.fuse = nullptr;
            a = &a_unfused;
        }
    }
    if (N > 64 * 16) return launch_chained(c, a);
    int L, R;
    sk_exact_shape(N, a->nreads, &L, &R);
    const int P = L * R - N;

    if (int rc = upload_layout(c, a->motif, N, L, R)) return rc;

    sdtw_kargs k = kargs_of(a);
    k.nreads = a->nreads; k.read0 = 0; k.ridx = nullptr; k.xlay = (const double *)c->motif.p; k.P = P;
    k.out = a->out; k.last_row = a->last_row;

    int ck = 128;
    int span = N + N / 8 + 8, span_q = N + 8, span2 = 2 * N + N / 4 + 16;
    if (const char *e = sk_tune("SK_DTW_CK")) { int v = atoi(e); if (v >= 64 && v % 64 == 0) ck = v; }
    if (const char *e = sk_tune("SK_DTW_SPAN")) { int v = atoi(e); if (v > 0) { span = span_q = v; span2 = 0; } }
    if (const char *e = sk_tune("SK_DTW_SPAN2")) { int v = atoi(e); if (v >= 0) span2 = v; }
    const int64_t maxlen = a->max_len;
    const char *scheme = sk_tune("SK_DTW_SCHEME");
    const bool two_pass = !a->last_row && !a->force_single && maxlen >= 4 * (int64_t)(span + ck) &&
                          a->nreads >= 256 && !(scheme && strcmp(scheme, "full") == 0);
    SK_HIP(hipEventRecord(c->ev[2], c->stream));
    if (a->fuse && !two_pass) return sk_fail(SK_ERR_INVALID, "internal: fused prologue without a screening pass");
    if (!two_pass) {
        c->last_retry = 0;
        c->retry_dev = false;
        c->prof_chunks = 0;
        sdtw_fn fn = pick_any(a->feed, L, R, MODE_FULL);
        if (!fn) return sk_fail(SK_ERR_UNSUPPORTED, "no kernel for L=%d R=%d", L, R);
        int rc = launch(c, fn, k, L);
        if (rc) return rc;
        SK_HIP(hipEventRecord(c->ev[3], c->stream));
        return SK_OK;
    }

    sdtw_fn fa = pick_any(a->feed, L, R, MODE_DIST);
    sdtw_fn fb = pick_any(a->feed, L, R, MODE_START);
    sdtw_fn ff = pick_any(a->feed, L, R, MODE_FULL);
    if (!fa || !fb || !ff) return sk_fail(SK_ERR_UNSUPPORTED, "no kernel for L=%d R=%d", L, R);

    bool qok = true;
    for (int i = 0; i < N; i++) qok = qok && (fabs(a->motif[i]) < QLIM);
    if (const char *e = sk_tune("SK_DTW_SCHEME")) qok = qok && strcmp(e, "exact2") != 0;
    int rc;
    if ((rc = sk_reserve(c, &c->retry, 2 * ((size_t)a->nreads + 2) * sizeof(int32_t)))) return rc;
    if ((rc = sk_reserve(c, &c->dtwcnt, 128))) return rc;
    int32_t *cnt = (int32_t *)c->retry.p;
    int32_t *ecnt = cnt + a->nreads + 2;
    SK_HIP(hipMemsetAsync(cnt, 0, sizeof(int32_t), c->stream));
    SK_HIP(hipMemsetAsync(ecnt, 0, sizeof(int32_t), c->stream));
    if (!a->accumulate) SK_HIP(hipMemsetAsync(c->dtwcnt.p, 0, 128, c->stream));
    c->retry_dev = true;
    if (L == 16 && !c->motif64_valid && pick_any(a->feed, 64, (N + 63) / 64, MODE_FULL)) {
        const int R64 = (N + 63) / 64;
        SK_HIP(hipStreamSynchronize(c->stream));
        if (c->stream3) SK_HIP(hipStreamSynchronize(c->stream3));
        if (c->stream4) SK_HIP(hipStreamSynchronize(c->stream4));
        c->motif64_host.resize((size_t)64 * R64);
        if (!sk_lane_layout(a->motif, N, 64, R64, c->motif64_host.data()))
            return sk_fail(SK_ERR_INVALID, "internal: motif layout mismatch");
        if ((rc = sk_reserve(c, &c->motif64, c->motif64_host.size() * sizeof(double)))) return rc;
        SK_HIP(hipMemcpyAsync(c->motif64.p, c->motif64_host.data(),
                              c->motif64_host.size() * sizeof(double), hipMemcpyHostToDevice, c->stream));
        c->motif64_valid = true;
    }
    auto launch_retry = [&](int32_t *list = nullptr, hipStream_t stream = nullptr) -> int {
        if (!list) list = cnt;
        sdtw_kargs kr = k;
        kr.read0 = 0; kr.ridx = list + 2; kr.count_ptr = list; kr.ckpt = nullptr;
        kr.total_ptr = (int32_t *)c->dtwcnt.p; kr.list_off = 0;
        const int R64 = (N + 63) / 64, P64 = 64 * R64 - N;
        sdtw_fn f64 = (L == 16) ? pick_any(a->feed, 64, R64, MODE_FULL) : nullptr;
        if (f64) {
            sdtw_kargs k64 = kr;
            k64.xlay = (const double *)c->motif64.p; k64.P = P64;
            k64.nreads = a->nreads < 8192 ? a->nreads : 8192;
            int rc2;
            if ((rc2 = launch(c, f64, k64, 64, stream))) return rc2;
            if (a->nreads <= 8192) return SK_OK;
            kr.list_off = 8192; kr.total_ptr = nullptr; kr.nreads = a->nreads - 8192;
            return launch(c, ff, kr, L, stream);
        }
        kr.nreads = a->nreads;
        return launch(c, ff, kr, L, stream);
    };
    if (a->fuse && !qok) return sk_fail(SK_ERR_INVALID, "internal: fused prologue without a screening pass");
    int32_t *guard = (int32_t *)c->dtwcnt.p + 8;
    const bool guarded = qok && sk_tune("SK_DTW_NOGUARD") == nullptr;
    int audit_period = 4096;
    if (const char *e = sk_tune("SK_DTW_AUDIT_PERIOD")) { const int v = atoi(e); if (v >= 0) audit_period = v; }
    int naudit = (guarded && audit_period > 0) ? (int)((a->nreads + audit_period - 1) / audit_period) : 0;
    if (naudit && sk_tune("SK_DTW_AUDIT_PERIOD") == nullptr) {
        const double audit_ms = (double)(maxlen + 64) * (8.0 * ((N + 63) / 64) + 20.0) * 5.0 / 2.4e6;
        const double window_ms = (double)a->nreads * N * 5.85e-8;
        const double call_ms = (double)a->nreads * (double)maxlen * N * 7.4e-11;
        const double exposed = audit_ms - window_ms;
        if (exposed > 0.02 * call_ms) {
            double kd = exposed / (0.02 * call_ms + 1e-9);
            const uint32_t K = kd > 64.0 ? 64u : (uint32_t)kd + 1u;
            if (c->dtw_sparse_calls++ % K) naudit = 0;
        }
    }
    int32_t *alist = nullptr;  sk_hit *aout = nullptr;
    if (naudit) {
        if ((rc = sk_reserve(c, &c->audit, ((size_t)naudit + 2) * sizeof(int32_t) + 16 + (size_t)naudit * sizeof(sk_hit)))) return rc;
        alist = (int32_t *)c->audit.p;
        aout = (sk_hit *)((char *)c->audit.p + ((((size_t)naudit + 2) * sizeof(int32_t) + 15) & ~(size_t)15));
    }
    auto launch_audit = [&](hipStream_t stream) -> int {
        if (!naudit) return SK_OK;
        sk_audit_pick(alist, naudit, audit_period, a->nreads, c->dtw_audit_calls++, stream ? stream : c->stream);
        SK_HIP(hipGetLastError());
        sdtw_kargs kr = k;
        kr.read0 = 0; kr.ridx = alist + 2; kr.count_ptr = alist; kr.ckpt = nullptr; kr.out = aout; kr.out_by_slot = 1;
        kr.total_ptr = guard + SK_GUARD_AUDITED; kr.list_off = 0;
        const int R64 = (N + 63) / 64, P64 = 64 * R64 - N;
        sdtw_fn f64 = (L == 16) ? pick_any(a->feed, 64, R64, MODE_FULL) : nullptr;
        if (f64) {
            sdtw_kargs k64 = kr;
            k64.xlay = (const double *)c->motif64.p; k64.P = P64;
            k64.nreads = naudit < 8192 ? naudit : 8192;
            int rc2;
            if ((rc2 = launch(c, f64, k64, 64, stream))) return rc2;
            if (naudit <= 8192) return SK_OK;
            kr.list_off = 8192; kr.total_ptr = nullptr; kr.nreads = naudit - 8192;
            return launch(c, ff, kr, L, stream);
        }
        kr.nreads = naudit;
        return launch(c, ff, kr, L, stream);
    };
    auto finish_guard = [&]() -> int {
        if (!guarded) return SK_OK;
        if (naudit) {
            sk_audit_compare(alist, aout, a->out, naudit, guard, c->stream);
            SK_HIP(hipGetLastError());
        }
        sdtw_kargs kf = k;
        kf.read0 = 0; kf.nreads = a->nreads; kf.ridx = nullptr; kf.count_ptr = nullptr; kf.ckpt = nullptr;
        kf.gate_ptr = guard + SK_GUARD_ALARM; kf.guard = guard;
        return launch(c, ff, kf, L);
    };
    if (qok) {
        const bool early = sk_tune("SK_DTW_NO_EARLY") == nullptr;
        if (early && !c->stream3) {
            SK_HIP(hipStreamCreateWithFlags(&c->stream3, hipStreamNonBlocking));
            for (int i = 0; i < 2; i++) SK_HIP(hipEventCreateWithFlags(&c->ev_r[i], hipEventDisableTiming));
        }
        if (early && naudit && !c->stream4) {
            SK_HIP(hipStreamCreateWithFlags(&c->stream4, hipStreamNonBlocking));
            SK_HIP(hipEventCreateWithFlags(&c->ev_a, hipEventDisableTiming));
        }
        if ((rc = sk_launch_sdtw_screen(c, a, ck, span_q, span2, cnt, cnt + 2, early ? ecnt : nullptr,
                                        early ? ecnt + 2 : nullptr))) return rc;
        if (early) {
            SK_HIP(hipStreamWaitEvent(c->stream3, c->ev_r[0], 0));
            if ((rc = launch_retry(ecnt, c->stream3))) return rc;
            SK_HIP(hipEventRecord(c->ev_r[1], c->stream3));
            if (naudit) {
                SK_HIP(hipStreamWaitEvent(c->stream4, c->ev_r[0], 0));
                if ((rc = launch_audit(c->stream4))) return rc;
                SK_HIP(hipEventRecord(c->ev_a, c->stream4));
            }
        }
        if ((rc = launch_retry())) return rc;
        if (early) {
            SK_HIP(hipStreamWaitEvent(c->stream, c->ev_r[1], 0));
            if (naudit) SK_HIP(hipStreamWaitEvent(c->stream, c->ev_a, 0));
        } else if ((rc = launch_audit(nullptr))) return rc;
        if ((rc = finish_guard())) return rc;
        SK_HIP(hipEventRecord(c->ev[3], c->stream));
        return SK_OK;
    }
    const int nck = (int)((maxlen + L - 1) / ck);
    const size_t per_read = (size_t)(nck > 0 ? nck : 1) * L * (R + 3) * sizeof(double);
    int64_t chunk;
    while (true) {
        chunk = sk_dtw_chunk_reads(per_read, a->nreads);
        rc = sk_reserve(c, &c->ckpt, (size_t)chunk * per_read);
        if (rc != SK_ERR_NOMEM || chunk <= 1024) break;
        sk_dtw_scratch_shrink(0);
    }
    if (rc) return rc;
    k.ckpt = (double *)c->ckpt.p; k.nck = nck; k.ck = ck; k.span = span;
    k.retry = cnt + 2; k.retry_cnt = cnt;
    const size_t nchunks = (size_t)((a->nreads + chunk - 1) / chunk);
    while (c->evpool.size() < 3 * nchunks) {
        hipEvent_t e;
        SK_HIP(hipEventCreate(&e));
        c->evpool.push_back(e);
    }
    c->prof_chunks = 0;
    for (int64_t r0 = 0; r0 < a->nreads; r0 += chunk) {
        k.read0 = (int)r0;
        k.nreads = (int)((a->nreads - r0 < chunk) ? a->nreads - r0 : chunk);
        hipEvent_t *ev = &c->evpool[3 * (size_t)c->prof_chunks];
        SK_HIP(hipEventRecord(ev[0], c->stream));
        if ((rc = launch(c, fa, k, L))) return rc;
        SK_HIP(hipEventRecord(ev[1], c->stream));
        if ((rc = launch(c, fb, k, L))) return rc;
        SK_HIP(hipEventRecord(ev[2], c->stream));
        c->prof_reads[c->prof_chunks < 64 ? c->prof_chunks : 63] = k.nreads;
        c->prof_chunks++;
    }
    if ((rc = launch_retry())) return rc;
    SK_HIP(hipEventRecord(c->ev[3], c->stream));
    return SK_OK;
}
```

squigglekit_amd/csrc/sk_sdtwq.hip:

```cpp
#include "sk_sdtw_dev.h"
#include "sk_prepw_dev.h"
#include <math.h>
#include <stdlib.h>
#include <string.h>
#include <vector>

#ifndef SK_SDTWQ_FEED
#define SK_SDTWQ_FEED 0
#define SK_SDTWQ_MAIN 1
#endif

namespace {

template <int R>
__device__ __forceinline__ void qcolumn(const unsigned (&old)[R], unsigned (&nw)[R], const unsigned (&xq)[R],
                                        unsigned yq, unsigned dg, unsigned up)
{
    constexpr int R4 = R & ~3;
#pragma unroll
    for (int k = 0; k < R4; k += 4) {
        asm("v_min3_u32 %0, %12, %4, %13\n\t"
            "v_sad_u32 %0, %8, %14, %0 clamp\n\t"
            "v_min3_u32 %1, %4, %5, %0\n\t"
            "v_sad_u32 %1, %9, %14, %1 clamp\n\t"
            "v_min3_u32 %2, %5, %6, %1\n\t"
            "v_sad_u32 %2, %10, %14, %2 clamp\n\t"
            "v_min3_u32 %3, %6, %7, %2\n\t"
            "v_sad_u32 %3, %11, %14, %3 clamp"
            : "=&v"(nw[k]), "=&v"(nw[k + 1]), "=&v"(nw[k + 2]), "=&v"(nw[k + 3])
            : "v"(old[k]), "v"(old[k + 1]), "v"(old[k + 2]), "v"(old[k + 3]),
              "v"(xq[k]), "v"(xq[k + 1]), "v"(xq[k + 2]), "v"(xq[k + 3]),
              "v"(dg), "v"(up), "v"(yq));
        dg = old[k + 3];
        up = nw[k + 3];
    }
#pragma unroll
    for (int k = R4; k < R; k++) {
        asm("v_min3_u32 %0, %3, %1, %4\n\t"
            "v_sad_u32 %0, %2, %5, %0 clamp"
            : "=&v"(nw[k])
            : "v"(old[k]), "v"(xq[k]), "v"(dg), "v"(up), "v"(yq));
        dg = old[k];
        up = nw[k];
    }
}

__device__ __forceinline__ unsigned qimg(double v)
{
    return (unsigned)((int)rint(v * QSCALE)) + 0x80000000u;
}

template <int L>
__device__ __forceinline__ unsigned shr0(unsigned v, unsigned notfirst)
{
    if constexpr (L >= 16) {
        (void)notfirst;
        return (unsigned)__builtin_amdgcn_update_dpp(0, (int)v, (L == 16) ? DPP_ROW_SHR1 : DPP_WAVE_SHR1, 0xF, 0xF, true);
    } else {
        unsigned r;
        asm("s_nop 1\n\t"
            "v_and_b32_dpp %0, %1, %2 row_shr:1 row_mask:0xf bank_mask:0xf bound_ctrl:0"
            : "=v"(r) : "v"(v), "v"(notfirst));
        return r;
    }
}

constexpr int HINT_T = 5, HINT_G = 4, HINT_MARGIN = 8;
constexpr int HINT_MAX_PLEN = 8192;
constexpr int HINT_MIN_READS = 500000;
constexpr int HINT_MAX_R = 25;
constexpr int HINT_MIN_N = 1 << HINT_G;
constexpr unsigned HINT_MASK = (1u << HINT_T) - 1u;

template <int L>
__device__ __forceinline__ unsigned shrtag(unsigned v, unsigned tag)
{
    static_assert(L == 8 || L == 16, "groups of 8 or 16 lanes in DPP rows of 16");
    unsigned r;
    asm("s_mov_b32 vcc_lo, %3\n\t"
        "s_mov_b32 vcc_hi, %3\n\t"
        "v_cndmask_b32_dpp %0, %1, %2, vcc row_shr:1 row_mask:0xf bank_mask:0xf bound_ctrl:0"
        : "=v"(r) : "v"(v), "v"(tag), "i"(L == 8 ? 0x01010101 : 0x00010001) : "vcc");
    return r;
}

struct wrec {
    int32_t tbase;
    int32_t jlo, jhi;
    int32_t flags;
};
struct sibrec {
    int32_t r;
    int32_t jlo, jhi;
    int32_t pad;
};

template <int L>
__device__ __forceinline__ void candidate_columns(const sdtw_kargs &a, int r, int n, unsigned b, int l, int &jlo_out, int &jhi_out,
                                                  int clo = 0, int chi = 0x7fffffff)
{
    const unsigned *lastq = a.lastq + (int64_t)(r - a.read0) * a.lq_stride;
    const unsigned *ls = a.lsum + (int64_t)(r - a.read0) * (a.nck + 1) * L + l;
    const unsigned thr = (b > QINF - 2u * a.qerr) ? QINF : b + 2u * a.qerr;
    int jlo = 0x7fffffff, jhi = -1;
    if (n > 0 && b < QSAFE) {
        for (int cc = 0; cc <= a.nck; cc++) {
            if (ls[(int64_t)cc * L] > thr) continue;
            const int j0 = cc * a.ck + l - (L - 1);
            for (int q = 0; q < a.ck / L; q++) {
                const int j = j0 + q * L;
                if (j >= clo && j <= chi && j >= 0 && j < n && lastq[j + L] <= thr) { jlo = min(jlo, j); jhi = max(jhi, j); }
            }
        }
    }
#pragma unroll
    for (int d = 1; d < L; d <<= 1) { jlo = min(jlo, __shfl_xor(jlo, d)); jhi = max(jhi, __shfl_xor(jhi, d)); }
    jlo_out = jlo; jhi_out = jhi;
}

template <int L>
__device__ __forceinline__ int hint_start(const sdtw_kargs &a, int r, unsigned b, int l, int jlo, int jhi)
{
    const unsigned *lastq = a.lastq + (int64_t)(r - a.read0) * a.lq_stride;
    const unsigned *ls = a.lsum + (int64_t)(r - a.read0) * (a.nck + 1) * L + l;
    const unsigned thr = (b > QINF - 2u * a.qerr) ? QINF : b + 2u * a.qerr;
    int hs = 0x7fffffff;
    for (int cc = jlo / a.ck; cc <= min(a.nck, (jhi + L - 1) / a.ck); cc++) {
        if (ls[(int64_t)cc * L] > thr) continue;
        const int j0 = cc * a.ck + l - (L - 1);
        for (int q = 0; q < a.ck / L; q++) {
            const int j = j0 + q * L;
            if (j < jlo || j > jhi) continue;
            const unsigned w = lastq[j + L];
            if (w > thr) continue;
            const int gj = j >> HINT_G;
            const int gs = gj - (int)((unsigned)(gj - (int)(w & HINT_MASK)) & HINT_MASK);
            hs = min(hs, max(gs, 0) << HINT_G);
        }
    }
#pragma unroll
    for (int d = 1; d < L; d <<= 1) hs = min(hs, __shfl_xor(hs, d));
    return hs;
}

#ifndef SK_Q_WAVES
#define SK_Q_WAVES(R) 4
#endif
#ifdef SK_SDTWQ_HINT
#define SK_Q_KERNEL k_sdtw_qh
#define SK_P_KERNEL k_sdtw_ph
constexpr bool HINT = true;
#else
#define SK_Q_KERNEL k_sdtw_q
#define SK_P_KERNEL k_sdtw_p
constexpr bool HINT = false;
#endif
template <int L, int R, int FEED, bool P0>
__global__ __launch_bounds__(256) __attribute__((amdgpu_waves_per_eu(SK_Q_WAVES(R), 8)))
void SK_Q_KERNEL(const sdtw_kargs a)
{
    static_assert(L == 8 || L == 16 || L == 64, "lanes per read");
    static_assert(!HINT || (FEED == SK_FEED_I16 && L <= (1 << HINT_G) && (1 << HINT_G) % L == 0),
                  "tagged sweep: int16 feed, a block of L steps inside one granule");
    constexpr int G = 64 / L;
    constexpr int CKH = (R + 3) / 2;
    constexpr int U = (L < 16) ? L : 16;

    const int lane = threadIdx.x & 63;
    const int wave = blockIdx.x * (blockDim.x >> 6) + (threadIdx.x >> 6);
    const int g = lane / L, l = lane % L;
    int slot = wave * G + g;
    const bool live = slot < a.nreads;
    if (!live) slot = a.nreads - 1;
    const int r = a.read0 + slot;
    const bool timer = a.clk && blockIdx.x == 0 && threadIdx.x < 64;
    unsigned long long tc0 = 0, tr0 = 0;
    if (timer) { tc0 = __builtin_amdgcn_s_memtime(); tr0 = __builtin_amdgcn_s_memrealtime(); }

    extern __shared__ __align__(16) unsigned char lds_dyn[];
    __shared__ __align__(16) unsigned lds_all[4][5 * 64];
    int n;
    double center = 0.0, scale = 1.0;
    const int16_t *s16 = nullptr;
    const double  *s64 = nullptr;
    if constexpr (FEED == SK_FEED_I16) {
        if (a.fz_raw) {
            unsigned *wlds = (unsigned *)lds_dyn + (size_t)(threadIdx.x >> 6) * a.lds_wave_words;
            n = 0;
            if (a.fz_mode == 0) {
                const prepw_env E = prepw_setup<5>(wlds, lane, a.fz_lo, a.fz_hi, a.fz_vec);
                for (int gg = 0; gg < G; gg++) {
                    if (wave * G + gg >= a.nreads) break;
                    const sk_prep pr = prepw_read<5>(E, a.fz_raw, a.stride, a.fz_len, a.read0 + wave * G + gg, lane,
                                                     (int16_t *)a.samples, (sk_prep *)a.prep);
                    if (g == gg) { n = pr.n; center = pr.center; scale = pr.scale; }
                }
            } else {
                const zs_env E = zs_setup((int16_t *)wlds, (double *)lds_all[threadIdx.x >> 6], a.fz_lo, a.fz_hi, a.fz_vec);
#pragma unroll 1
                for (int gg = 0; gg < G; gg++) {
                    if (wave * G + gg >= a.nreads) break;
                    const sk_prep pr = zs_read(E, a.fz_raw, a.stride, a.fz_len, a.read0 + wave * G + gg, lane,
                                               (int16_t *)a.samples, (sk_prep *)a.prep);
                    if (g == gg) { n = pr.n; center = pr.center; scale = pr.scale; }
                    __builtin_amdgcn_wave_barrier();
                }
            }
            __builtin_amdgcn_fence(__ATOMIC_RELEASE, "workgroup");
            __builtin_amdgcn_fence(__ATOMIC_ACQUIRE, "workgroup");
        } else {
            const sk_prep pr = a.prep[r];
            n = pr.n; center = pr.center; scale = pr.scale;
        }
        s16 = (const int16_t *)a.samples + (int64_t)r * a.stride;
    } else if constexpr (FEED == SK_FEED_F64_NORM) {
        const sk_prep pr = a.prep[r];
        n = pr.n; center = pr.center; scale = pr.scale;
        s64 = (const double *)(((pr.flags & SK_IFLAG_INPLACE) && a.samples_raw) ? a.samples_raw : a.samples) + a.off[r];
    } else {
        n = (int)(a.off[r + 1] - a.off[r]);
        s64 = (const double *)a.samples + a.off[r];
    }
    if (!live) n = 0;
    const double inv_scale = 1.0 / scale;

    int nsteps = (n > 0) ? n - 1 + L : 0;
#pragma unroll
    for (int d = L; d < 64; d <<= 1) nsteps = max(nsteps, __shfl_xor(nsteps, d));
    nsteps = __builtin_amdgcn_readfirstlane(nsteps);
    const int nblk = (nsteps + L - 1) / L;

    unsigned xq[R];
#pragma unroll
    for (int k = 0; k < R; k++) xq[k] = HINT ? (a.xlayq[l * R + k] & ~HINT_MASK) : a.xlayq[l * R + k];
    const bool shortlane = l < a.P;
    const unsigned notfirst = (l == 0) ? 0u : 0xffffffffu;
    [[maybe_unused]] unsigned tagv = 0;

    unsigned Da[R], Db[R];
#pragma unroll
    for (int k = 0; k < R; k++) { Da[k] = QINF; Db[k] = QINF; }
    unsigned botq = (R == 1 && l == 0 && shortlane) ? 0u : QINF;
    unsigned diagq = (l == 0) ? 0u : QINF;
    int bad = 0;
    if constexpr (FEED == SK_FEED_F64_NORM) {
        if (live && (a.prep[r].flags & SK_FLAG_RECENTRE)) bad = 1;
    }
    unsigned qmin = QINF;
    unsigned smin = QINF;

    const int nlast = max(n - 1, 0);
    if (n == 0) { s16 = (const int16_t *)a.xlayq; s64 = (const double *)a.xlayq; }
    auto loadraw = [&](int idx) {
        if constexpr (FEED == SK_FEED_I16) return (int)s16[min(idx, nlast)];
        else                               return s64[min(idx, nlast)];
    };
    const double qa = inv_scale * QSCALE, qb = -center * qa;
    const bool fma64 = FEED == SK_FEED_F64_NORM && a.hole >= SK_HOLE_FMA64;
    if (live && n > 0) {
        double imgerr = 0.0;
        if (FEED == SK_FEED_I16 || fma64)            imgerr = 3.8e-7 + fabs(center) * qa * 1.2e-16;
        else if constexpr (FEED == SK_FEED_F64_NORM) imgerr = 5.7e-7;
        const bool rej = !(imgerr * (double)(HINT ? a.qplen : a.qerr) <= 1.0) && a.hole != SK_HOLE_FMA64_UNGUARDED;
        if (rej) {
            bad = 1;
            if (l == 0 && a.guard) atomicAdd(&a.guard[SK_GUARD_IMGREJ], 1);
        }
    }
    auto toq = [&](auto raw_, int idx) -> unsigned {
        const double raw = (double)raw_;
        double t;
        if constexpr (FEED == SK_FEED_I16)           t = __builtin_fma(raw, qa, qb);
        else if constexpr (FEED == SK_FEED_F64_NORM) t = fma64 ? __builtin_fma(raw, qa, qb) : (raw - center) * qa;
        else                                         t = raw * QSCALE;
        const bool ok = fabs(t) < QLIM * QSCALE;
        unsigned q = (unsigned)__double2loint(t + 6755399441055744.0) ^ 0x80000000u;
        if constexpr (HINT) q &= ~HINT_MASK;
        const bool in = idx < n;
        bad |= (in && !ok) ? 1 : 0;
        return (in && ok) ? q : QINF;
    };

    const unsigned smask = shortlane ? 0xffffffffu : 0u;
    unsigned *lastq = a.lastq + (int64_t)(r - a.read0) * a.lq_stride;
    unsigned *ybuf = lds_all[threadIdx.x >> 6] + g * 5 * L;
    unsigned *dump = ybuf + 3 * L;
    unsigned *ibuf = (unsigned *)lds_dyn + (size_t)(threadIdx.x >> 6) * a.lds_wave_words + g * a.ck;
    int ioff = 0;
    unsigned gmin = QINF;
    ybuf[L + l] = QINF;
    unsigned F = toq(loadraw(l), l);
    auto step = [&](const unsigned (&old)[R], unsigned (&nw)[R], unsigned yq, unsigned *hslot) {
        unsigned upq;
        if constexpr (HINT) upq = shrtag<L>(botq, tagv);
        else                upq = shr0<L>(botq, notfirst);
        qcolumn<R>(old, nw, xq, yq, diagq, upq);
        diagq = upq;
        if constexpr (P0)          botq = nw[R - 1];
        else if constexpr (R >= 2) asm("v_bitop3_b32 %0, %1, %2, %3 bitop3:0xe4" : "=v"(botq) : "v"(nw[R - 2]), "v"(nw[R - 1]), "v"(smask));
        else                       asm("v_bitop3_b32 %0, %1, %2, %3 bitop3:0xe4" : "=v"(botq) : "v"(upq), "v"(nw[0]), "v"(smask));
        *hslot = nw[R - 1];
    };
    auto flush = [&](int c, int nb) {
        unsigned im = smin;
#pragma unroll
        for (int d = 1; d < L; d <<= 1) im = min(im, (unsigned)__shfl_xor((int)im, d));
        const unsigned lim = (gmin > QINF - 2u * a.qerr) ? QINF : gmin + 2u * a.qerr;
        const bool keep = live && im <= lim;
        gmin = min(gmin, im);
        if (keep) {
            unsigned *dst = lastq + (int64_t)c * a.ck + l + 1;
            for (int q = 0; q < nb; q++) dst[q * L] = ibuf[q * L + l];
        }
    };
    for (int blk = 0; blk < nblk; blk++) {
        const auto rawnext = loadraw((blk + 1) * L + l);
        const int t0 = blk * L;
        if (t0 > 0 && (t0 % a.ck) == 0) {
          if (t0 / a.ck <= a.nck && live) {
            unsigned *cp = a.ckq + (((int64_t)(r - a.read0) * a.nck + (t0 / a.ck - 1)) * L + l) * CKH;
            auto hi2 = [](unsigned lo_word, unsigned hi_word) -> unsigned {
                return __builtin_amdgcn_perm(hi_word, lo_word, 0x07060302u);
            };
#pragma unroll
            for (int k = 0; k + 1 < R; k += 2) cp[k / 2] = hi2(Da[k], Da[k + 1]);
            if constexpr (R % 2) { cp[R / 2] = hi2(Da[R - 1], botq); cp[R / 2 + 1] = hi2(diagq, 0u); }
            else                 { cp[R / 2] = hi2(botq, diagq); }
            a.lsum[((int64_t)(r - a.read0) * (a.nck + 1) + (t0 / a.ck - 1)) * L + l] = smin;
          }
            flush(t0 / a.ck - 1, a.ck / L);
            smin = QINF;
            ioff = 0;
        }
        unsigned *hw = (l == L - 1) ? ibuf + ioff : dump;
        if constexpr (HINT) tagv = (unsigned)(t0 >> HINT_G) & HINT_MASK;
        const unsigned *yr;
        if (blk & 1) { ybuf[L + l] = F; yr = ybuf + L - l; }
        else         { ybuf[l] = F; ybuf[2 * L + l] = F; yr = ybuf + 2 * L - l; }
#pragma unroll 1
        for (int qq = 0; qq < L; qq += U) {
            unsigned yv[U];
#pragma unroll
            for (int q = 0; q < U; q++) yv[q] = yr[qq + q];
#pragma unroll
            for (int q = 0; q < U; q += 2) {
                step(Da, Db, yv[q], hw + qq + q);
                step(Db, Da, yv[q + 1], hw + qq + q + 1);
            }
        }
        F = toq(rawnext, (blk + 1) * L + l);
        { const unsigned hv = ibuf[ioff + l]; smin = min(smin, hv); }
        ioff += L;
    }
    {
        const int cl = nblk > 0 ? min((nblk * L - 1) / a.ck, a.nck) : 0;
        if (live) a.lsum[((int64_t)(r - a.read0) * (a.nck + 1) + cl) * L + l] = smin;
        if (nblk > 0) flush(cl, ioff / L);
        for (int cc = cl + 1; cc <= a.nck; cc++)
            if (live) a.lsum[((int64_t)(r - a.read0) * (a.nck + 1) + cc) * L + l] = QINF;
    }
    if (live) {
        const unsigned *ls = a.lsum + (int64_t)(r - a.read0) * (a.nck + 1) * L + l;
        for (int cc = 0; cc <= a.nck; cc++) qmin = min(qmin, ls[(int64_t)cc * L]);
    }
#pragma unroll
    for (int d = 1; d < L; d <<= 1) {
        bad |= __shfl_xor(bad, d);
        qmin = min(qmin, (unsigned)__shfl_xor((int)qmin, d));
    }
    const unsigned bq = bad ? QINF : qmin;
    if (live && l == 0) a.qflag[r - a.read0] = (int32_t)bq;
    if (a.wrec_q) {
        int jlo, jhi;
        candidate_columns<L>(a, r, n, bq, l, jlo, jhi);
        int sjlo = 0, sjhi = -1;
        if (a.sib && live && bq < QSAFE && jhi >= jlo && jhi - jlo > a.wmax) {
            int alo, ahi, blo, bhi;
            candidate_columns<L>(a, r, n, bq, l, alo, ahi, jlo, jlo + a.wmax);
            candidate_columns<L>(a, r, n, bq, l, blo, bhi, jlo + a.wmax + 1);
            if (bhi >= blo && bhi - blo <= a.wmax) {
                int slot_ok = 0;
                if (l == 0) {
                    const int idx = atomicAdd(a.sib_cnt, 1);
                    if (idx < a.sib_cap) {
                        sibrec sb;
                        sb.r = r; sb.jlo = blo; sb.jhi = bhi; sb.pad = 0;
                        ((sibrec *)a.sib)[idx] = sb;
                        slot_ok = 1;
                    }
                }
                slot_ok = __shfl(slot_ok, lane - l);
                if (slot_ok) { jhi = ahi; sjlo = blo; sjhi = bhi; }
            }
        }
        int tx = 0;
        if constexpr (HINT) {
            tx = max(0, jlo - a.span);
            if (live && bq < QSAFE && jhi >= jlo && jhi - jlo <= a.wmax && sjhi < sjlo) {
                const int hs = hint_start<L>(a, r, bq, l, jlo, jhi);
                if (hs <= jlo) tx = min(max(hs - HINT_MARGIN, 0), max(jlo - 1, 0));
            }
        }
        if (live && l == 0) {
            wrec w;
            w.tbase = tx; w.jlo = jlo; w.jhi = jhi; w.flags = (sjhi >= sjlo) ? 4 : 0;
            ((wrec *)a.wrec_q)[r - a.read0] = w;
            const bool screened = (bq < QSAFE) && (jhi >= jlo) && (jhi - jlo <= a.wmax);
            if (a.early_cnt && n > 0 && !screened) a.early[atomicAdd(a.early_cnt, 1)] = r;
        }
    }
    if (timer && lane == 0) {
        a.clk[0] = __builtin_amdgcn_s_memtime() - tc0;
        a.clk[1] = __builtin_amdgcn_s_memrealtime() - tr0;
    }
}

template <int L, int R, int FEED>
__global__ __launch_bounds__(256)
void SK_P_KERNEL(const sdtw_kargs a)
{
    constexpr int G = 64 / L;
    constexpr int CKW = R + 2;

    const int lane = threadIdx.x & 63;
    const int wave = blockIdx.x * (blockDim.x >> 6) + (threadIdx.x >> 6);
    const int g = lane / L, l = lane % L;
    int slot = wave * G + g;
    int nreads = a.nreads;
    if (a.wl_count) {
        nreads = min(*a.wl_count, a.nreads);
        if (a.total_ptr && blockIdx.x == 0 && threadIdx.x == 0) atomicAdd(a.total_ptr, nreads);
        if (nreads <= 0) return;
    }
    const bool live = slot < nreads;
    if (!live) slot = nreads - 1;
    const int r = a.tier2 == 2 ? ((const sibrec *)a.sib)[slot].r : a.wl_list ? a.wl_list[slot] : a.read0 + slot;

    int n;
    double center = 0.0, scale = 1.0;
    const int16_t *s16 = nullptr;
    const double  *s64 = nullptr;
    if constexpr (FEED == SK_FEED_I16) {
        const sk_prep pr = a.prep[r];
        n = pr.n; center = pr.center; scale = pr.scale;
        s16 = (const int16_t *)a.samples + (int64_t)r * a.stride;
    } else if constexpr (FEED == SK_FEED_F64_NORM) {
        const sk_prep pr = a.prep[r];
        n = pr.n; center = pr.center; scale = pr.scale;
        s64 = (const double *)(((pr.flags & SK_IFLAG_INPLACE) && a.samples_raw) ? a.samples_raw : a.samples) + a.off[r];
    } else {
        n = (int)(a.off[r + 1] - a.off[r]);
        s64 = (const double *)a.samples + a.off[r];
    }
    if (!live) n = 0;

    const unsigned b = (unsigned)a.qflag[r - a.read0];
    int jlo, jhi, clustered = 0;
    [[maybe_unused]] int txq = 0;
    if (!a.tier2) {
        const wrec q = ((const wrec *)a.wrec_q)[r - a.read0];
        jlo = q.jlo; jhi = q.jhi; clustered = q.flags & 4; txq = q.tbase;
    } else if (a.tier2 == 2) {
        const sibrec q = ((const sibrec *)a.sib)[slot];
        jlo = q.jlo; jhi = q.jhi; clustered = 4;
    } else {
        candidate_columns<L>(a, r, n, b, l, jlo, jhi);
    }
    const bool screened = (n > 0) && (b < QSAFE) && (jhi >= jlo) && (jhi - jlo <= a.wmax);

    int tbase = 0, c0 = 0, npre = 0;
    if (screened) {
        const int tx = (HINT && !a.tier2) ? min(max(txq, 0), jlo) : max(0, jlo - a.span);
        c0 = tx / a.ck;
        if (c0 > a.nck) c0 = a.nck;
        tbase = c0 * a.ck;
        if (c0 > 0) npre = (tx - tbase) / L;
    }
    const bool shortlane = l < a.P;
    const unsigned notfirst = (l == 0) ? 0u : 0xffffffffu;

    unsigned Qs[R];
    unsigned botq = QINF, diagq = QINF;
#pragma unroll
    for (int k = 0; k < R; k++) Qs[k] = QINF;
    constexpr int CKH = (R + 3) / 2;
    const unsigned *cp = a.ckq + (((int64_t)(r - a.read0) * a.nck + (c0 > 0 ? c0 - 1 : 0)) * L + l) * CKH;
    auto load_ckpt = [&]() {
        auto word = [&](int k) -> unsigned { const unsigned w2 = cp[k / 2]; return (k & 1) ? (w2 & 0xffff0000u) : (w2 << 16); };
#pragma unroll
        for (int k = 0; k < R; k++) Qs[k] = word(k);
        botq = word(R); diagq = word(R + 1);
    };
    int maxpre = npre;
#pragma unroll
    for (int d = L; d < 64; d <<= 1) maxpre = max(maxpre, __shfl_xor(maxpre, d));
    maxpre = __builtin_amdgcn_readfirstlane(maxpre);
    if (maxpre > 0) {
        const double inv_scale = 1.0 / scale;
        const int nlast = max(n - 1, 0);
        if (n == 0) { s16 = (const int16_t *)a.xlayq; s64 = (const double *)a.xlayq; }
        auto toq = [&](int idx) -> unsigned {
            const int ci = min(max(idx, 0), nlast);
            double v;
            if constexpr (FEED == SK_FEED_I16)           v = ((double)s16[ci] - center) * inv_scale;
            else if constexpr (FEED == SK_FEED_F64_NORM) v = (s64[ci] - center) * inv_scale;
            else                                         v = s64[ci];
            return (idx >= 0 && idx < n && fabs(v) < QLIM) ? qimg(v) : QINF;
        };
        unsigned xq[R];
#pragma unroll
        for (int k = 0; k < R; k++) xq[k] = a.xlayq[l * R + k];
        unsigned Qn[R];
#pragma unroll
        for (int k = 0; k < R; k++) Qn[k] = QINF;
        const unsigned smask = shortlane ? 0xffffffffu : 0u;
        __shared__ unsigned lds_p[4][3 * 64];
        unsigned *ybuf = lds_p[threadIdx.x >> 6] + g * 3 * L;
        unsigned Fq = QINF;
        const int startblk = maxpre - npre;
        auto qstep = [&](const unsigned (&old)[R], unsigned (&nw)[R], unsigned yq) {
            const unsigned upq = shr0<L>(botq, notfirst);
            qcolumn<R>(old, nw, xq, yq, diagq, upq);
            diagq = upq;
            if constexpr (R >= 2) asm("v_bitop3_b32 %0, %1, %2, %3 bitop3:0xe4" : "=v"(botq) : "v"(nw[R - 2]), "v"(nw[R - 1]), "v"(smask));
            else                  asm("v_bitop3_b32 %0, %1, %2, %3 bitop3:0xe4" : "=v"(botq) : "v"(upq), "v"(nw[0]), "v"(smask));
        };
        for (int pb = 0; pb < maxpre; pb++) {
            const int t0 = tbase + (pb - startblk) * L;
            if (pb == startblk && npre > 0) {
                load_ckpt();
                const unsigned prev = toq(t0 - L + l);
                if (pb & 1) ybuf[l] = prev; else ybuf[L + l] = prev;
                Fq = toq(t0 + l);
            }
            const unsigned Fnext = toq(t0 + L + l);
            const unsigned *yr;
            if (pb & 1) { ybuf[L + l] = Fq; yr = ybuf + L - l; }
            else        { ybuf[l] = Fq; ybuf[2 * L + l] = Fq; yr = ybuf + 2 * L - l; }
#pragma unroll 1
            for (int q = 0; q < L; q += 2) {
                const unsigned y0 = yr[q], y1 = yr[q + 1];
                qstep(Qs, Qn, y0);
                qstep(Qn, Qs, y1);
            }
            Fq = Fnext;
        }
    }
    if (c0 > 0 && npre == 0) load_ckpt();
    tbase += npre * L;

    if (live) {
        if (c0 > 0) {
            unsigned *ws = a.wstate + ((int64_t)slot * L + l) * CKW;
#pragma unroll
            for (int k = 0; k < R; k++) ws[k] = Qs[k];
            ws[R] = botq; ws[R + 1] = diagq;
        }
        if (l == 0) {
            wrec w;
            w.tbase = tbase; w.jlo = jlo; w.jhi = jhi;
            w.flags = (screened ? 1 : 0) | (c0 > 0 ? 2 : 0) | clustered;
            ((wrec *)a.wrec)[slot] = w;
        }
    }
}

template <int L, int R, int FEED>
__global__ __launch_bounds__(256) __attribute__((amdgpu_waves_per_eu(R <= 13 ? 4 : (R <= 26 ? 3 : 2), 8)))
void k_sdtw_w(const sdtw_kargs a)
{
    constexpr int G = 64 / L;
    constexpr bool XLDS = R > 16;
    constexpr int SHR = (L == 64) ? DPP_WAVE_SHR1 : DPP_ROW_SHR1;
    constexpr int CKW = R + 2;
    constexpr int U = (L < 16) ? L : 8;
    const double INF = __builtin_huge_val();

    const int lane = threadIdx.x & 63;
    const int wave = blockIdx.x * (blockDim.x >> 6) + (threadIdx.x >> 6);
    const int g = lane / L, l = lane % L;
    int slot = wave * G + g;
    int nreads = a.nreads;
    if (a.wl_count) {
        nreads = min(*a.wl_count, a.nreads);
        if (nreads <= 0) return;
    }
    const bool live = slot < nreads;
    if (!live) slot = nreads - 1;
    const int r = a.tier2 == 2 ? ((const sibrec *)a.sib)[slot].r : a.wl_list ? a.wl_list[slot] : a.read0 + slot;

    int n, flags = 0;
    double center = 0.0, scale = 1.0;
    const int16_t *s16 = nullptr;
    const double  *s64 = nullptr;
    if constexpr (FEED == SK_FEED_I16) {
        const sk_prep pr = a.prep[r];
        n = pr.n; flags = pr.flags & SK_FLAG_PUBLIC; center = pr.center; scale = pr.scale;
        s16 = (const int16_t *)a.samples + (int64_t)r * a.stride;
    } else if constexpr (FEED == SK_FEED_F64_NORM) {
        const sk_prep pr = a.prep[r];
        n = pr.n; flags = pr.flags & SK_FLAG_PUBLIC; center = pr.center; scale = pr.scale;
        s64 = (const double *)(((pr.flags & SK_IFLAG_INPLACE) && a.samples_raw) ? a.samples_raw : a.samples) + a.off[r];
    } else {
        n = (int)(a.off[r + 1] - a.off[r]);
        if (n == 0) flags = SK_FLAG_EMPTY;
        s64 = (const double *)a.samples + a.off[r];
    }
    if (!live) n = 0;

    const wrec rec = ((const wrec *)a.wrec)[slot];
    const bool screened = live && (rec.flags & 1);
    const bool restored = screened && (rec.flags & 2);
    const int tbase = screened ? rec.tbase : 0;
    const int jlo = rec.jlo, jhi = rec.jhi;
    const int tlast = screened ? jhi + L - 1 : -1;
    const bool shortlane = l < a.P;
    const unsigned notfirst = (l == 0) ? 0u : 0xffffffffu;
    const unsigned first = ~notfirst;

    int nsteps = tlast - tbase + 1;
    if (nsteps < 0) nsteps = 0;
    const int own_steps = nsteps;
#pragma unroll
    for (int d = L; d < 64; d <<= 1) nsteps = max(nsteps, __shfl_xor(nsteps, d));
    nsteps = __builtin_amdgcn_readfirstlane(nsteps);
    const int nblk = (nsteps + L - 1) / L;
    if (a.wsteps) {
        if (lane == 0 && nblk > 0) atomicAdd(&a.wsteps[0], (unsigned long long)(nblk * L));
        if (live && l == 0 && own_steps > 0) atomicAdd(&a.wsteps[1], (unsigned long long)own_steps);
    }

    double x[XLDS ? 1 : R];
    constexpr int RP = R | 1;
    __shared__ double lds_x[XLDS ? L * RP : 1];
    if constexpr (XLDS) {
        for (int i = threadIdx.x; i < L * R; i += blockDim.x) lds_x[(i / R) * RP + i % R] = a.xlay[i];
        __syncthreads();
    } else {
#pragma unroll
        for (int k = 0; k < R; k++) x[k] = a.xlay[l * R + k];
    }
    const double *xl = lds_x + (XLDS ? l * RP : 0);

    const int nlast = max(n - 1, 0);
    if (n == 0) { s16 = (const int16_t *)a.xlay; s64 = (const double *)a.xlay; }
    auto fetch = [&](int idx) -> double {
        const int ci = min(max(idx, 0), nlast);
        double v;
        if constexpr (FEED == SK_FEED_I16)           v = ((double)s16[ci] - center) / scale;
        else if constexpr (FEED == SK_FEED_F64_NORM) v = (s64[ci] - center) / scale;
        else                                         v = s64[ci];
        return (idx < 0 || idx >= n) ? INF : v;
    };
    auto lb = [&](unsigned q) -> double { return (double)(q > a.qerr ? q - a.qerr : 0u) * QUNIT; };

    double D[R];
    int    S[R];
#pragma unroll
    for (int k = 0; k < R; k++) { D[k] = INF; S[k] = -1; }
    double botD = (R == 1 && l == 0 && shortlane) ? 0.0 : INF;
    int    botS = (R == 1 && l == 0 && shortlane) ? 0 : -1;
    double diagD = (l == 0) ? 0.0 : INF;
    int    diagS = (l == 0) ? tbase : -1;
    if (restored) {
        const unsigned *ws = a.wstate + ((int64_t)slot * L + l) * CKW;
#pragma unroll
        for (int k = 0; k < R; k++) D[k] = lb(ws[k]);
        botD = lb(ws[R]);
        if (l > 0) diagD = lb(ws[R + 1]);
        if (R == 1 && l == 0 && shortlane) { botD = 0.0; botS = tbase; }
    }
    double best = INF;  int bestS = -1, bestJ = -1;
    int s0 = screened ? max(jlo - tbase + L - 1, 0) : 0x7fffffff;
#pragma unroll
    for (int d = L; d < 64; d <<= 1) s0 = min(s0, __shfl_xor(s0, d));
    s0 = __builtin_amdgcn_readfirstlane(s0);

    __shared__ double lds_w[4][3 * 64];
    double *ybuf = lds_w[threadIdx.x >> 6] + g * 3 * L;
    ybuf[L + l] = fetch(tbase - L + l);
    double F = fetch(tbase + l);
    for (int blk = 0; blk < nblk; blk++) {
        const double Fnext = fetch(tbase + (blk + 1) * L + l);
        const double *yr;
        if (blk & 1) { ybuf[L + l] = F; yr = ybuf + L - l; }
        else         { ybuf[l] = F; ybuf[2 * L + l] = F; yr = ybuf + 2 * L - l; }
#pragma unroll 1
        for (int qq = 0; qq < L; qq += U) {
            double yv[U];
#pragma unroll
            for (int q = 0; q < U; q++) yv[q] = yr[qq + q];
#pragma unroll
            for (int q = 0; q < U; q++) {
                const int t = tbase + blk * L + qq + q;
                const double y = yv[q];
                double upD;  int upS;
                if constexpr (L >= 16) {
                    upD = dpp_f64<SHR>(0.0, botD);
                    upS = dpp_i32<SHR>(t + 1, botS);
                } else {
                    const unsigned lo = shr0<L>((unsigned)__double2loint(botD), notfirst);
                    const unsigned hi = shr0<L>((unsigned)__double2hiint(botD), notfirst);
                    upD = __hiloint2double((int)hi, (int)lo);
                    upS = (int)(shr0<L>((unsigned)botS, notfirst) | (first & (unsigned)(t + 1)));
                }
                double dgD = diagD;  int dgS = diagS;
                double uD = upD;     int uS = upS;
#pragma unroll
                for (int k = 0; k < R; k++) {
                    const double lfD = D[k];  const int lfS = S[k];
                    const double xk = XLDS ? xl[k] : x[k];
                    const double c = fabs(xk - y);
                    const bool lt1 = lfD < dgD;
                    const double m1 = vmin(lfD, dgD);
                    const int    s1 = lt1 ? lfS : dgS;
                    const bool lt2 = uD < m1;
                    const double m = vmin(uD, m1);
                    const int    s = lt2 ? uS : s1;
                    const double nd = c + m;
                    dgD = lfD;  dgS = lfS;
                    D[k] = nd;  S[k] = s;
                    uD = nd;    uS = s;
                }
                diagD = upD;  diagS = upS;
                if constexpr (R >= 2) {
                    botD = shortlane ? D[R - 2] : D[R - 1];
                    botS = shortlane ? S[R - 2] : S[R - 1];
                } else {
                    botD = shortlane ? upD : D[0];
                    botS = shortlane ? upS : S[0];
                }
                if (blk * L + qq + q >= s0) {
                    const int j = t - l;
                    if (j >= jlo && j <= jhi && D[R - 1] < best) { best = D[R - 1]; bestS = S[R - 1]; bestJ = j; }
                }
            }
        }
        F = Fnext;
    }

    auto premise_holds = [&](double bestD, int j) -> bool {
        if (!a.guard) return true;
        const unsigned lq = a.lastq[(int64_t)(r - a.read0) * a.lq_stride + j + L];
        const unsigned bq = (unsigned)a.qflag[r - a.read0];
        const double u = bestD * QSCALE, e = (double)a.qerr;
        const double e2 = (rec.flags & 4) ? 3.0 * e : e;
        const bool ok = fabs(u - (double)lq) <= e && u <= (double)bq + e2;
        if (!ok) { atomicAdd(&a.guard[SK_GUARD_VIOL], 1); atomicAdd(&a.guard[SK_GUARD_ALARM], 1); }
        return ok;
    };
    if (live && l == L - 1) {
        sk_hit h;
        h.n = n; h.flags = flags;
        const bool forced = a.force_retry && (((unsigned)r * 2654435761u) >> 22) < (unsigned)a.force_retry;
        bool certified = false;
        if (a.tier2 == 2) {
            h.dist = best; h.start = bestS; h.end = bestJ;
            h.n = (n > 0 && screened && bestS >= 0 && !forced && premise_holds(best, bestJ)) ? 1 : 0;
            a.sib_out[slot] = h;
        } else if (n <= 0) {
            h.dist = __builtin_nan(""); h.start = -1; h.end = -1;
            a.out[r] = h;
        } else if (screened && bestS >= 0 && !forced && (certified = premise_holds(best, bestJ))) {
            h.dist = best; h.start = bestS; h.end = bestJ;
            a.out[r] = h;
        } else if (!screened && a.early_cnt && !a.tier2) {
        } else {
            h.dist = __builtin_nan(""); h.start = -1; h.end = -1;
            a.out[r] = h;
            const bool violated = screened && bestS >= 0 && !forced && !certified;
            if (screened && a.soft && !forced && !violated) a.soft[atomicAdd(a.soft_cnt, 1)] = r;
            else                                            a.retry[atomicAdd(a.retry_cnt, 1)] = r;
        }
    }
}

typedef void (*sdtw_fn)(const sdtw_kargs);

template <int L, int FEED, int WHICH>
sdtw_fn pick_r(int R)
{
#ifndef SK_SDTWQ_HINT
#define SK_KERNEL(RR) (WHICH == 0 ? (sdtw_fn)SK_Q_KERNEL<L, RR, FEED, false> :     \
                       WHICH == 3 ? (sdtw_fn)SK_Q_KERNEL<L, RR, FEED, (RR >= 2)> : \
                       WHICH == 1 ? (sdtw_fn)SK_P_KERNEL<L, RR, FEED> : (sdtw_fn)k_sdtw_w<L, RR, FEED>)
#else
#define SK_KERNEL(RR) (WHICH == 0 ? (sdtw_fn)SK_Q_KERNEL<L, RR, FEED, false> :     \
                       WHICH == 3 ? (sdtw_fn)SK_Q_KERNEL<L, RR, FEED, (RR >= 2)> : (sdtw_fn)SK_P_KERNEL<L, RR, FEED>)
#endif
    switch (R) { SK_R_CASES_1_16(SK_KERNEL) }
    if constexpr (L != 64) {
        switch (R) { SK_R_CASES_17_32(SK_KERNEL) }
    }
#undef SK_KERNEL
    return nullptr;
}

template <int WHICH, int FEED>
sdtw_fn pick_l(int L, int R)
{
    if (L == 8)  return pick_r<8, FEED, WHICH>(R);
    if (L == 16) return pick_r<16, FEED, WHICH>(R);
#ifndef SK_SDTWQ_HINT
    return pick_r<64, FEED, WHICH>(R);
#else
    return nullptr;
#endif
}

}

#if defined(SK_SDTWQ_HINT)
void *sk_sdtwq_pick_hint(int which, int L, int R)
#elif SK_SDTWQ_FEED == 0
void *sk_sdtwq_pick_feed0(int which, int L, int R)
#elif SK_SDTWQ_FEED == 1
void *sk_sdtwq_pick_feed1(int which, int L, int R)
#else
void *sk_sdtwq_pick_feed2(int which, int L, int R)
#endif
{
    switch (which) {
    case 0: return (void *)pick_l<0, SK_SDTWQ_FEED>(L, R);
    case 1: return (void *)pick_l<1, SK_SDTWQ_FEED>(L, R);
    case 3: return (void *)pick_l<3, SK_SDTWQ_FEED>(L, R);
#ifndef SK_SDTWQ_HINT
    default: return (void *)pick_l<2, SK_SDTWQ_FEED>(L, R);
#else
    default: return nullptr;
#endif
    }
}

#ifdef SK_SDTWQ_MAIN
void *sk_sdtwq_pick_feed1(int which, int L, int R);
void *sk_sdtwq_pick_feed2(int which, int L, int R);
void *sk_sdtwq_pick_hint(int which, int L, int R);

static void screen_layout(int N, int64_t nreads, int64_t maxlen, int *L, int *R)
{
    int l = (N <= 8 * 32 && nreads >= (maxlen > 8192 ? 65536 : 49152)) ? 8 : (N <= 16 * 32) ? 16 : 64;
    if (const char *e = sk_tune("SK_DTW_QL")) {
        const int v = atoi(e);
        if ((v == 8 && N <= 8 * 32) || (v == 16 && N <= 16 * 32) || v == 64) l = v;
    }
    *L = l;
    *R = (N + l - 1) / l;
}

constexpr int ORDER_BINS = 1024;

struct order_args {
    const wrec    *rec;
    const int32_t *qflag;
    int nreads, read0, span, ck, nck, L, wmax;
    int hint;
    int32_t *hist;
    int32_t *order;
};

__device__ __forceinline__ int order_key(const order_args &a, int i)
{
    const wrec q = a.rec[i];
    const unsigned b = (unsigned)a.qflag[i];
    if (!((b < QSAFE) && (q.jhi >= q.jlo) && (q.jhi - q.jlo <= a.wmax))) return ORDER_BINS - 1;
    const int tx = a.hint ? min(max(q.tbase, 0), q.jlo) : max(0, q.jlo - a.span);
    int c0 = tx / a.ck;
    if (c0 > a.nck) c0 = a.nck;
    const int npre = c0 > 0 ? (tx - c0 * a.ck) / a.L : 0;
    const int tbase = c0 * a.ck + npre * a.L;
    const int nblk = (q.jhi + a.L - tbase + a.L - 1) / a.L;
    return ORDER_BINS - 1 - (min(max(nblk, 1), 63) * 16 + min(npre, 15));
}

constexpr int ORDER_TPB = 1024, ORDER_IPT = 4;

__global__ __launch_bounds__(ORDER_TPB) void k_order_count(const order_args a)
{
    __shared__ int h[ORDER_BINS];
    for (int b = threadIdx.x; b < ORDER_BINS; b += ORDER_TPB) h[b] = 0;
    __syncthreads();
#pragma unroll
    for (int u = 0; u < ORDER_IPT; u++) {
        const int i = (blockIdx.x * ORDER_IPT + u) * ORDER_TPB + threadIdx.x;
        if (i < a.nreads) atomicAdd(&h[order_key(a, i)], 1);
    }
    __syncthreads();
    for (int b = threadIdx.x; b < ORDER_BINS; b += ORDER_TPB)
        if (h[b]) atomicAdd(&a.hist[b], h[b]);
}

__global__ __launch_bounds__(ORDER_BINS) void k_order_scan(int32_t *hist)
{
    __shared__ int s[ORDER_BINS];
    const int t = threadIdx.x;
    const int v = hist[t];
    s[t] = v;
    __syncthreads();
    for (int d = 1; d < ORDER_BINS; d <<= 1) {
        const int add = t >= d ? s[t - d] : 0;
        __syncthreads();
        s[t] += add;
        __syncthreads();
    }
    hist[t] = s[t] - v;
}

__global__ __launch_bounds__(ORDER_TPB) void k_order_scatter(const order_args a)
{
    __shared__ int h[ORDER_BINS];
    for (int b = threadIdx.x; b < ORDER_BINS; b += ORDER_TPB) h[b] = 0;
    __syncthreads();
    int key[ORDER_IPT], rank[ORDER_IPT];
#pragma unroll
    for (int u = 0; u < ORDER_IPT; u++) {
        const int i = (blockIdx.x * ORDER_IPT + u) * ORDER_TPB + threadIdx.x;
        key[u] = 0; rank[u] = 0;
        if (i < a.nreads) { key[u] = order_key(a, i); rank[u] = atomicAdd(&h[key[u]], 1); }
    }
    __syncthreads();
    for (int b = threadIdx.x; b < ORDER_BINS; b += ORDER_TPB)
        if (h[b]) h[b] = atomicAdd(&a.hist[b], h[b]);
    __syncthreads();
#pragma unroll
    for (int u = 0; u < ORDER_IPT; u++) {
        const int i = (blockIdx.x * ORDER_IPT + u) * ORDER_TPB + threadIdx.x;
        if (i < a.nreads) a.order[h[key[u]] + rank[u]] = a.read0 + i;
    }
}

__global__ void k_sib_combine(const sibrec *sib, const int32_t *cnt, int cap, const sk_hit *so, sk_hit *out,
                              int32_t *retry, int32_t *retry_cnt, int32_t *nsib_total)
{
    const int s = blockIdx.x * blockDim.x + threadIdx.x;
    if (s == 0 && nsib_total) atomicAdd(nsib_total, min(*cnt, cap));
    if (s >= min(*cnt, cap)) return;
    const int r = sib[s].r;
    sk_hit A = out[r];
    const sk_hit B = so[s];
    if (A.start < 0) return;
    if (B.n == 1) {
        if (B.dist < A.dist) { A.dist = B.dist; A.start = B.start; A.end = B.end; out[r] = A; }
    } else {
        A.dist = __builtin_nan(""); A.start = -1; A.end = -1;
        out[r] = A;
        retry[atomicAdd(retry_cnt, 1)] = r;
    }
}

int sk_launch_sdtw_screen(sk_ctx *c, const sk_sdtw_args *a, int ck, int span, int span2,
                          int32_t *d_retry_cnt, int32_t *d_retry, int32_t *d_early_cnt, int32_t *d_early)
{
    const int N = a->nmotif;
    int L, R;
    screen_layout(N, a->nreads, a->max_len, &L, &R);
    const int P = L * R - N;
    int rc;
    if (!c->motifq_valid || c->motifq_L != L) {
        SK_HIP(hipStreamSynchronize(c->stream));
        std::vector<unsigned> &layq = c->motifq_host;
        std::vector<double> &layw = c->motifw_host;
        layq.resize((size_t)L * R);
        layw.resize((size_t)L * R);
        if (!sk_lane_layout(a->motif, N, L, R, layw.data())) return sk_fail(SK_ERR_INVALID, "internal: motif layout mismatch");
        for (size_t i = 0; i < layw.size(); i++)
            layq[i] = (unsigned)((int)rint(layw[i] * QSCALE)) + 0x80000000u;
        if ((rc = sk_reserve(c, &c->motifq, layq.size() * sizeof(unsigned)))) return rc;
        if ((rc = sk_reserve(c, &c->motifw, layw.size() * sizeof(double)))) return rc;
        SK_HIP(hipMemcpyAsync(c->motifq.p, layq.data(), layq.size() * sizeof(unsigned), hipMemcpyHostToDevice, c->stream));
        SK_HIP(hipMemcpyAsync(c->motifw.p, layw.data(), layw.size() * sizeof(double), hipMemcpyHostToDevice, c->stream));
        c->motifq_valid = true;
        c->motifq_L = L;
    }

    const int64_t maxlen = a->max_len;
    const int nck = (int)((maxlen + L - 1) / ck);
    const size_t lq_stride = (size_t)((maxlen + 3 * L + 7) & ~(int64_t)3);
    const size_t state_bytes = (size_t)L * (R + 2) * sizeof(unsigned);
    const size_t ck_bytes = (size_t)L * ((R + 3) / 2) * sizeof(unsigned);
    const size_t per_read = (size_t)(nck > 0 ? nck : 1) * ck_bytes + lq_stride * sizeof(unsigned) + state_bytes +
                            (size_t)(nck + 1) * L * sizeof(unsigned) + 64;
    int64_t chunk;
    while (true) {
        chunk = sk_dtw_chunk_reads(per_read, a->nreads);
        rc = sk_reserve(c, &c->ckpt, (size_t)chunk * (size_t)(nck > 0 ? nck : 1) * ck_bytes);
        if (!rc) rc = sk_reserve(c, &c->lastq, (size_t)chunk * lq_stride * sizeof(unsigned));
        if (!rc) rc = sk_reserve(c, &c->wstate, (size_t)chunk * state_bytes);
        if (!rc) rc = sk_reserve(c, &c->lsum, (size_t)chunk * (size_t)(nck + 1) * L * sizeof(unsigned));
        if (rc != SK_ERR_NOMEM || chunk <= 1024) break;
        sk_dtw_scratch_shrink(0);
    }
    if (rc) return rc;
    if ((rc = sk_reserve(c, &c->qflag, (size_t)chunk * sizeof(int32_t)))) return rc;
    if ((rc = sk_reserve(c, &c->wrec, (size_t)chunk * sizeof(wrec)))) return rc;
    if ((rc = sk_reserve(c, &c->wrecq, (size_t)chunk * sizeof(wrec)))) return rc;
    int sort_min = 32768;
    if (const char *e = sk_tune("SK_DTW_SORT_MIN")) { const int v = atoi(e); if (v > 0) sort_min = v; }
    const bool sorted = chunk >= sort_min && sk_tune("SK_DTW_NOSORT") == nullptr;
    if (sorted && (rc = sk_reserve(c, &c->order, ((size_t)chunk + ORDER_BINS) * sizeof(int32_t)))) return rc;
    const bool tiers = span2 > span;
    if (tiers && (rc = sk_reserve(c, &c->wsoft, ((size_t)chunk + 1) * sizeof(int32_t)))) return rc;
    const bool siblings = sk_tune("SK_DTW_NO_SIBLINGS") == nullptr;
    const int sib_cap = (int)(chunk / 64 + 1024);
    if (siblings) {
        if ((rc = sk_reserve(c, &c->sib, 16 + (size_t)sib_cap * sizeof(sibrec)))) return rc;
        if ((rc = sk_reserve(c, &c->sibout, (size_t)sib_cap * sizeof(sk_hit)))) return rc;
        if ((rc = sk_reserve(c, &c->sibstate, (size_t)sib_cap * (state_bytes + sizeof(wrec))))) return rc;
        if (c->stream3 && !c->ev_s[0])
            for (int i = 0; i < 2; i++) SK_HIP(hipEventCreateWithFlags(&c->ev_s[i], hipEventDisableTiming));
    }

    typedef void *(*pick_fn)(int, int, int);
    const pick_fn pk = a->feed == SK_FEED_I16 ? (pick_fn)sk_sdtwq_pick_feed0
                     : a->feed == SK_FEED_F64_NORM ? (pick_fn)sk_sdtwq_pick_feed1 : (pick_fn)sk_sdtwq_pick_feed2;
    sdtw_fn fq = (sdtw_fn)pk(P == 0 ? 3 : 0, L, R), fp = (sdtw_fn)pk(1, L, R), fw = (sdtw_fn)pk(2, L, R);
    const int64_t plen = (int64_t)N + maxlen + 2;
    int64_t hint_min = HINT_MIN_READS;
    if (const char *e = sk_tune("SK_DTW_HINT_MIN")) { const int v = atoi(e); if (v > 0) hint_min = v; }
    const bool hint = a->feed == SK_FEED_I16 && (L == 8 || L == 16) && plen <= HINT_MAX_PLEN && R <= HINT_MAX_R &&
                      N >= HINT_MIN_N && a->nreads >= hint_min && sk_tune("SK_DTW_NOHINT") == nullptr;
    sdtw_fn fp1 = fp;
    if (hint) { fq = (sdtw_fn)sk_sdtwq_pick_hint(P == 0 ? 3 : 0, L, R); fp1 = (sdtw_fn)sk_sdtwq_pick_hint(1, L, R); }
    if (!fq || !fp || !fp1 || !fw) return sk_fail(SK_ERR_UNSUPPORTED, "no screening kernel for L=%d R=%d", L, R);

    sdtw_kargs k = kargs_of(a);
    k.xlay = (const double *)c->motifw.p; k.xlayq = (const unsigned *)c->motifq.p; k.P = P; k.out = a->out;
    k.nck = nck; k.ck = ck; k.span = span; k.retry = d_retry; k.retry_cnt = d_retry_cnt;
    k.ckq = (unsigned *)c->ckpt.p; k.lastq = (unsigned *)c->lastq.p; k.lq_stride = (int64_t)lq_stride;
    k.qflag = (int32_t *)c->qflag.p; k.lsum = (unsigned *)c->lsum.p;
    k.wstate = (unsigned *)c->wstate.p; k.wrec = c->wrec.p; k.wrec_q = c->wrecq.p;
    k.early_cnt = d_early_cnt; k.early = d_early;
    k.qplen = (unsigned)plen;
    k.qerr = hint ? ((unsigned)plen << HINT_T) + HINT_MASK : (unsigned)plen;
    k.wmax = 4 * ck;
    k.lds_wave_words = (64 / L) * ck;
    k.guard = sk_tune("SK_DTW_NOGUARD") ? nullptr : (int32_t *)c->dtwcnt.p + 8;
    k.wsteps = (unsigned long long *)((char *)c->dtwcnt.p + 64);
    if (const char *e = sk_tune("SK_DTW_HOLE")) {
        k.hole = strcmp(e, "qerr1") == 0 ? SK_HOLE_QERR1 : strcmp(e, "fma64") == 0 ? SK_HOLE_FMA64
               : strcmp(e, "fma64x") == 0 ? SK_HOLE_FMA64_UNGUARDED : SK_HOLE_NONE;
        if (k.hole == SK_HOLE_QERR1) k.qerr = 1;
    }
    if (const char *e = sk_tune("SK_DTW_FORCE_RETRY_PM")) {
        const int pm = atoi(e);
        if (pm > 0) k.force_retry = pm >= 1000 ? 1024 : (pm * 1024 + 999) / 1000;
    }

    size_t fz_lds = 0;
    const sk_prep_fuse fz = a->fuse ? *a->fuse : sk_prep_fuse();
    if (a->fuse) {
        const int need = fz.mode == SK_PREP_ZSCALE ? (int)((a->stride * 2 + 15) / 16 * 4) : (((fz.hi - fz.lo - 1) + 3) & ~3);
        if (need > k.lds_wave_words) k.lds_wave_words = need;
    }
    fz_lds = (size_t)4 * (size_t)k.lds_wave_words * sizeof(unsigned);
    if (fz_lds + 5 * 1024 > 64 * 1024)
        return sk_fail(SK_ERR_INVALID, "SK_DTW_CK=%d with %d lanes per read needs %zu bytes of LDS per workgroup (limit 65536): "
                       "use a smaller multiple of 64", ck, L, fz_lds + 5 * 1024);

    const size_t nchunks = (size_t)((a->nreads + chunk - 1) / chunk);
    while (c->evpool.size() < 3 * nchunks) {
        hipEvent_t e;
        SK_HIP(hipEventCreate(&e));
        c->evpool.push_back(e);
    }
    c->prof_chunks = 0;
    const int reads_per_block = 4 * (64 / L);
    for (int64_t r0 = 0; r0 < a->nreads; r0 += chunk) {
        k.read0 = (int)r0;
        k.nreads = (int)((a->nreads - r0 < chunk) ? a->nreads - r0 : chunk);
        const int grid = (k.nreads + reads_per_block - 1) / reads_per_block;
        if (a->fuse) {
            k.fz_raw = fz.raw; k.fz_len = fz.len; k.fz_lo = fz.lo; k.fz_hi = fz.hi;
            k.fz_mode = fz.mode == SK_PREP_ZSCALE ? 1 : 0;
            k.fz_vec = ((((uintptr_t)fz.raw & 15) == 0 && (a->stride % 8) == 0) ? 1 : 0) |
                       ((((uintptr_t)a->samples & 15) == 0 && (a->stride % 8) == 0) ? 2 : 0);
        }
        hipEvent_t *ev = &c->evpool[3 * (size_t)c->prof_chunks];
        k.sib = nullptr; k.sib_cnt = nullptr; k.sib_out = nullptr; k.tier2 = 0;
        if (siblings) {
            SK_HIP(hipMemsetAsync(c->sib.p, 0, 16, c->stream));
            k.sib_cnt = (int32_t *)c->sib.p; k.sib = (char *)c->sib.p + 16; k.sib_out = (sk_hit *)c->sibout.p;
            k.sib_cap = sib_cap;
        }
        SK_HIP(hipEventRecord(ev[0], c->stream));
        k.clk = (r0 == 0) ? (unsigned long long *)((char *)c->dtwcnt.p + 16) : nullptr;
        hipLaunchKernelGGL(fq, dim3(grid), dim3(256), fz_lds, c->stream, k);
        k.fz_raw = nullptr;
        if (d_early_cnt && r0 + chunk >= a->nreads) SK_HIP(hipEventRecord(c->ev_r[0], c->stream));
        SK_HIP(hipGetLastError());
        if (siblings) {
            sdtw_kargs ks = k;
            ks.tier2 = 2; ks.wl_list = nullptr; ks.wl_count = k.sib_cnt; ks.soft = nullptr; ks.soft_cnt = nullptr;
            ks.span = tiers ? span2 : span; ks.total_ptr = nullptr; ks.nreads = sib_cap;
            ks.wstate = (unsigned *)c->sibstate.p; ks.wrec = (char *)c->sibstate.p + (size_t)sib_cap * state_bytes;
            const int sgrid = (sib_cap + reads_per_block - 1) / reads_per_block;
            hipStream_t ss = c->stream3 ? c->stream3 : c->stream;
            if (c->stream3) {
                SK_HIP(hipEventRecord(c->ev_s[0], c->stream));
                SK_HIP(hipStreamWaitEvent(c->stream3, c->ev_s[0], 0));
            }
            hipLaunchKernelGGL(fp, dim3(sgrid), dim3(256), 0, ss, ks);
            hipLaunchKernelGGL(fw, dim3(sgrid), dim3(256), 0, ss, ks);
            SK_HIP(hipGetLastError());
            if (c->stream3) SK_HIP(hipEventRecord(c->ev_s[1], c->stream3));
        }
        SK_HIP(hipEventRecord(ev[1], c->stream));
        const int32_t *order = nullptr;
        if (sorted && k.nreads >= sort_min) {
            order_args oa;
            oa.rec = (const wrec *)c->wrecq.p; oa.qflag = (const int32_t *)c->qflag.p;
            oa.nreads = k.nreads; oa.read0 = k.read0; oa.span = span; oa.ck = ck; oa.nck = nck; oa.L = L; oa.wmax = k.wmax;
            oa.hint = hint ? 1 : 0;
            oa.hist = (int32_t *)c->order.p; oa.order = oa.hist + ORDER_BINS;
            SK_HIP(hipMemsetAsync(oa.hist, 0, ORDER_BINS * sizeof(int32_t), c->stream));
            const int og = (k.nreads + ORDER_TPB * ORDER_IPT - 1) / (ORDER_TPB * ORDER_IPT);
            hipLaunchKernelGGL(k_order_count, dim3(og), dim3(ORDER_TPB), 0, c->stream, oa);
            hipLaunchKernelGGL(k_order_scan, dim3(1), dim3(ORDER_BINS), 0, c->stream, oa.hist);
            hipLaunchKernelGGL(k_order_scatter, dim3(og), dim3(ORDER_TPB), 0, c->stream, oa);
            SK_HIP(hipGetLastError());
            order = oa.order;
        }
        k.tier2 = 0;
        if (tiers) {
            int32_t *soft = (int32_t *)c->wsoft.p;
            SK_HIP(hipMemsetAsync(soft, 0, sizeof(int32_t), c->stream));
            k.span = span; k.wl_list = order; k.wl_count = nullptr; k.soft = soft + 1; k.soft_cnt = soft;
            hipLaunchKernelGGL(fp1, dim3(grid), dim3(256), 0, c->stream, k);
            hipLaunchKernelGGL(fw, dim3(grid), dim3(256), 0, c->stream, k);
            SK_HIP(hipGetLastError());
            k.span = span2; k.wl_list = soft + 1; k.wl_count = soft; k.soft = nullptr; k.soft_cnt = nullptr;
            k.tier2 = 1;
            k.total_ptr = (int32_t *)c->dtwcnt.p + 1;
        } else {
            k.wl_list = order; k.wl_count = nullptr;
        }
        hipLaunchKernelGGL(tiers ? fp : fp1, dim3(grid), dim3(256), 0, c->stream, k);
        k.total_ptr = nullptr;
        hipLaunchKernelGGL(fw, dim3(grid), dim3(256), 0, c->stream, k);
        SK_HIP(hipGetLastError());
        if (siblings) {
            if (c->stream3) SK_HIP(hipStreamWaitEvent(c->stream, c->ev_s[1], 0));
            hipLaunchKernelGGL(k_sib_combine, dim3((sib_cap + 255) / 256), dim3(256), 0, c->stream,
                               (const sibrec *)k.sib, (const int32_t *)k.sib_cnt, sib_cap, (const sk_hit *)k.sib_out, k.out,
                               d_retry, d_retry_cnt, (int32_t *)c->dtwcnt.p + 8 + 6);
            SK_HIP(hipGetLastError());
        }
        SK_HIP(hipEventRecord(ev[2], c->stream));
        c->prof_reads[c->prof_chunks < 64 ? c->prof_chunks : 63] = k.nreads;
        c->prof_chunks++;
    }
    return SK_OK;
}
#endif
```

Baseline: 17.57 million.

## Pipeline DTW screening sweep segments with window passes on a second stream

Splits each chunk of the screening sweep into segments with up to three scratch slices. Each segment's window, sort and sibling passes then run on a separate stream while the next segment's sweep runs on the main stream. The early exact retry and audit launch in two parts, so work for the first part of the last chunk can start before the final segment is swept. This aims to fill the device while the low-occupancy window passes run, at the cost of more events, launches and cross-stream dependencies.

```diff
diff --git a/squigglekit_amd/csrc/sk_common.h b/squigglekit_amd/csrc/sk_common.h
--- a/squigglekit_amd/csrc/sk_common.h
+++ b/squigglekit_amd/csrc/sk_common.h
@@ -4,10 +4,12 @@
 #include <stddef.h>
 #include <stdarg.h>
 #include <vector>
+#include <functional>
 #include "squigglekit_hip.h"
 
 #define SK_MAX_DEVICES 16
 #define SK_WAVE 64
+#define SK_DTW_SLICES 3
 
 struct sk_prep {
     int32_t n;
@@ -95,6 +97,11 @@
     hipStream_t stream4 = nullptr;
     hipEvent_t  ev_a = nullptr;
     hipEvent_t  ev_s[2] = {nullptr, nullptr};
+    hipStream_t stream_w = nullptr;
+    hipEvent_t  ev_pq[SK_DTW_SLICES] = {};
+    hipEvent_t  ev_pw[SK_DTW_SLICES] = {};
+    hipEvent_t  ev_ps[SK_DTW_SLICES] = {};
+    hipEvent_t  ev_r2 = nullptr;
     uint32_t    dtw_sparse_calls = 0;
     uint32_t    dtw_audit_calls = 0;
     hipEvent_t  ev_chunk[9] = {};
@@ -336,8 +343,14 @@
 int sk_launch_events(sk_ctx *c, const sk_path_args *p, sk_event *events);
 int sk_launch_events_pool(sk_ctx *c, const sk_event *d_ev, const uint8_t *d_use, int64_t nhits, int32_t N,
                           int32_t *d_idx, int32_t *d_cnt, sk_pool_rec *d_out);
+struct sk_screen_early {
+    int32_t *cnt = nullptr, *list = nullptr;
+    int32_t *cnt2 = nullptr, *list2 = nullptr;
+    std::function<int(int part, int64_t split)> swept;
+};
 int sk_launch_sdtw_screen(sk_ctx *c, const sk_sdtw_args *a, int ck, int span, int span2,
-                          int32_t *d_retry_cnt, int32_t *d_retry, int32_t *d_early_cnt, int32_t *d_early);
+                          int32_t *d_retry_cnt, int32_t *d_retry, const sk_screen_early *early);
+int sk_dtw_segments(int64_t chunk_reads, int L, int64_t seg_reads, std::vector<int64_t> *sizes);
 
 int sk_band_check(const int64_t *off, int32_t nseq, const sk_pair *pairs, int64_t npairs, int32_t band, int32_t end_mode,
                   const void *out);
diff --git a/squigglekit_amd/csrc/sk_runtime.hip b/squigglekit_amd/csrc/sk_runtime.hip
--- a/squigglekit_amd/csrc/sk_runtime.hip
+++ b/squigglekit_amd/csrc/sk_runtime.hip
@@ -81,6 +81,8 @@
     {"SK_DTW_NOHINT",         "1",           "no start hint: the plain screening sweep, every read's exact window looks back the same number of columns"},
     {"SK_DTW_HINT_MIN",       "1",           "the start hint is on for calls of at least this many reads (default 500000)"},
     {"SK_DTW_SORT_MIN",       "1",           "window passes sort chunks of at least this many reads"},
+    {"SK_DTW_SEG_READS",      "32 96",       "reads per segment of a chunk, rounded up to a workgroup's (0 or unset: whole sweep rounds, by the size of the chunk); the window passes of a segment run beside the next one's sweep"},
+    {"SK_DTW_NOPIPE",         "1",           "no segments: a chunk's window passes run behind its whole sweep, on the main stream"},
     {"SK_DTW_NO_EARLY",       "1",           "no early exact retry beside the window passes"},
     {"SK_DTW_NO_SIBLINGS",    "1",           "reads whose candidate columns fall into two clusters take the exact pass (no second window)"},
     {"SK_DTW_NOGUARD",        "1",           "screening scheme without its run-time guard (premise test in the window pass, audit, gated exact fallback): A/B cost runs"},
@@ -150,6 +152,27 @@
     return chunk > 0 ? chunk : 1;
 }
 
+int sk_dtw_segments(int64_t chunk_reads, int L, int64_t seg_reads, std::vector<int64_t> *sizes)
+{
+    sizes->clear();
+    if (chunk_reads <= 0) return 0;
+    if (L != 8 && L != 16 && L != 64) L = 64;
+    const int64_t group = 4 * (64 / L), round = 4096 * (int64_t)(64 / L);
+    if (seg_reads > 0) {
+        const int64_t seg = (seg_reads + group - 1) / group * group;
+        int64_t left = chunk_reads;
+        for (; left > seg; left -= seg) sizes->push_back(seg);
+        sizes->push_back(left);
+        return (int)sizes->size();
+    }
+    const int64_t full = (chunk_reads - 1) / round;
+    const int64_t B = full / 8 < 1 ? 1 : full / 8 > 4 ? 4 : full / 8;
+    for (int64_t i = 0; i < full / B; i++) sizes->push_back(B * round);
+    for (int64_t i = 0; i < full % B; i++) sizes->push_back(round);
+    sizes->push_back(chunk_reads - full * round);
+    return (int)sizes->size();
+}
+
 extern "C" {
 
 int sk_tunables(char *buf, int cap)
@@ -240,6 +263,16 @@
             (void)hipStreamDestroy(c->stream3);
         }
         for (int i = 0; i < 2; i++) if (c->ev_s[i]) (void)hipEventDestroy(c->ev_s[i]);
+        if (c->stream_w) {
+            (void)hipStreamSynchronize(c->stream_w);
+            for (int i = 0; i < SK_DTW_SLICES; i++) {
+                if (c->ev_pq[i]) (void)hipEventDestroy(c->ev_pq[i]);
+                if (c->ev_pw[i]) (void)hipEventDestroy(c->ev_pw[i]);
+                if (c->ev_ps[i]) (void)hipEventDestroy(c->ev_ps[i]);
+            }
+            (void)hipStreamDestroy(c->stream_w);
+        }
+        if (c->ev_r2) (void)hipEventDestroy(c->ev_r2);
         if (c->stream4) {
             (void)hipStreamSynchronize(c->stream4);
             if (c->ev_a) (void)hipEventDestroy(c->ev_a);
diff --git a/squigglekit_amd/csrc/sk_sdtw.hip b/squigglekit_amd/csrc/sk_sdtw.hip
--- a/squigglekit_amd/csrc/sk_sdtw.hip
+++ b/squigglekit_amd/csrc/sk_sdtw.hip
@@ -615,12 +615,14 @@
     for (int i = 0; i < N; i++) qok = qok && (fabs(a->motif[i]) < QLIM);
     if (const char *e = sk_tune("SK_DTW_SCHEME")) qok = qok && strcmp(e, "exact2") != 0;
     int rc;
-    if ((rc = sk_reserve(c, &c->retry, 2 * ((size_t)a->nreads + 2) * sizeof(int32_t)))) return rc;
+    if ((rc = sk_reserve(c, &c->retry, 3 * ((size_t)a->nreads + 2) * sizeof(int32_t)))) return rc;
     if ((rc = sk_reserve(c, &c->dtwcnt, 128))) return rc;
     int32_t *cnt = (int32_t *)c->retry.p;
     int32_t *ecnt = cnt + a->nreads + 2;
+    int32_t *ecnt2 = ecnt + a->nreads + 2;
     SK_HIP(hipMemsetAsync(cnt, 0, sizeof(int32_t), c->stream));
     SK_HIP(hipMemsetAsync(ecnt, 0, sizeof(int32_t), c->stream));
+    SK_HIP(hipMemsetAsync(ecnt2, 0, sizeof(int32_t), c->stream));
     if (!a->accumulate) SK_HIP(hipMemsetAsync(c->dtwcnt.p, 0, 128, c->stream));
     c->retry_dev = true;
     if (L == 16 && !c->motif64_valid && pick_any(a->feed, 64, (N + 63) / 64, MODE_FULL)) {
@@ -636,8 +638,10 @@
                               c->motif64_host.size() * sizeof(double), hipMemcpyHostToDevice, c->stream));
         c->motif64_valid = true;
     }
-    auto launch_retry = [&](int32_t *list = nullptr, hipStream_t stream = nullptr) -> int {
+    auto launch_retry = [&](int32_t *list = nullptr, hipStream_t stream = nullptr, int64_t cap64 = -1) -> int {
         if (!list) list = cnt;
+        const int cap = (int)(cap64 < 0 ? a->nreads : cap64);
+        if (cap <= 0) return SK_OK;
         sdtw_kargs kr = k;
         kr.read0 = 0; kr.ridx = list + 2; kr.count_ptr = list; kr.ckpt = nullptr;
         kr.total_ptr = (int32_t *)c->dtwcnt.p; kr.list_off = 0;
@@ -646,14 +650,14 @@
         if (f64) {
             sdtw_kargs k64 = kr;
             k64.xlay = (const double *)c->motif64.p; k64.P = P64;
-            k64.nreads = a->nreads < 8192 ? a->nreads : 8192;
+            k64.nreads = cap < 8192 ? cap : 8192;
             int rc2;
             if ((rc2 = launch(c, f64, k64, 64, stream))) return rc2;
-            if (a->nreads <= 8192) return SK_OK;
-            kr.list_off = 8192; kr.total_ptr = nullptr; kr.nreads = a->nreads - 8192;
+            if (cap <= 8192) return SK_OK;
+            kr.list_off = 8192; kr.total_ptr = nullptr; kr.nreads = cap - 8192;
             return launch(c, ff, kr, L, stream);
         }
-        kr.nreads = a->nreads;
+        kr.nreads = cap;
         return launch(c, ff, kr, L, stream);
     };
     if (a->fuse && !qok) return sk_fail(SK_ERR_INVALID, "internal: fused prologue without a screening pass");
@@ -679,26 +683,33 @@
         alist = (int32_t *)c->audit.p;
         aout = (sk_hit *)((char *)c->audit.p + ((((size_t)naudit + 2) * sizeof(int32_t) + 15) & ~(size_t)15));
     }
-    auto launch_audit = [&](hipStream_t stream) -> int {
+    bool audit_picked = false, audit_counted = false;
+    auto launch_audit = [&](hipStream_t stream, int lo = 0, int hi = -1) -> int {
         if (!naudit) return SK_OK;
-        sk_audit_pick(alist, naudit, audit_period, a->nreads, c->dtw_audit_calls++, stream ? stream : c->stream);
-        SK_HIP(hipGetLastError());
+        if (hi < 0) hi = naudit;
+        if (!audit_picked) {
+            sk_audit_pick(alist, naudit, audit_period, a->nreads, c->dtw_audit_calls++, stream ? stream : c->stream);
+            SK_HIP(hipGetLastError());
+            audit_picked = true;
+        }
+        if (hi <= lo) return SK_OK;
         sdtw_kargs kr = k;
         kr.read0 = 0; kr.ridx = alist + 2; kr.count_ptr = alist; kr.ckpt = nullptr; kr.out = aout; kr.out_by_slot = 1;
-        kr.total_ptr = guard + SK_GUARD_AUDITED; kr.list_off = 0;
+        kr.total_ptr = audit_counted ? nullptr : guard + SK_GUARD_AUDITED; kr.list_off = lo;
+        audit_counted = true;
         const int R64 = (N + 63) / 64, P64 = 64 * R64 - N;
         sdtw_fn f64 = (L == 16) ? pick_any(a->feed, 64, R64, MODE_FULL) : nullptr;
-        if (f64) {
+        if (f64 && lo < 8192) {
             sdtw_kargs k64 = kr;
             k64.xlay = (const double *)c->motif64.p; k64.P = P64;
-            k64.nreads = naudit < 8192 ? naudit : 8192;
+            k64.nreads = (hi < 8192 ? hi : 8192) - lo;
             int rc2;
             if ((rc2 = launch(c, f64, k64, 64, stream))) return rc2;
-            if (naudit <= 8192) return SK_OK;
-            kr.list_off = 8192; kr.total_ptr = nullptr; kr.nreads = naudit - 8192;
+            if (hi <= 8192) return SK_OK;
+            kr.list_off = 8192; kr.total_ptr = nullptr; kr.nreads = hi - 8192;
             return launch(c, ff, kr, L, stream);
         }
-        kr.nreads = naudit;
+        kr.nreads = hi - lo;
         return launch(c, ff, kr, L, stream);
     };
     auto finish_guard = [&]() -> int {
@@ -722,18 +733,32 @@
             SK_HIP(hipStreamCreateWithFlags(&c->stream4, hipStreamNonBlocking));
             SK_HIP(hipEventCreateWithFlags(&c->ev_a, hipEventDisableTiming));
         }
-        if ((rc = sk_launch_sdtw_screen(c, a, ck, span_q, span2, cnt, cnt + 2, early ? ecnt : nullptr,
-                                        early ? ecnt + 2 : nullptr))) return rc;
+        if (early && !c->ev_r2) SK_HIP(hipEventCreateWithFlags(&c->ev_r2, hipEventDisableTiming));
+        sk_screen_early se;
+        int audit_done = 0;
         if (early) {
-            SK_HIP(hipStreamWaitEvent(c->stream3, c->ev_r[0], 0));
-            if ((rc = launch_retry(ecnt, c->stream3))) return rc;
-            SK_HIP(hipEventRecord(c->ev_r[1], c->stream3));
-            if (naudit) {
-                SK_HIP(hipStreamWaitEvent(c->stream4, c->ev_r[0], 0));
-                if ((rc = launch_audit(c->stream4))) return rc;
-                SK_HIP(hipEventRecord(c->ev_a, c->stream4));
-            }
-        }
+            se.cnt = ecnt; se.list = ecnt + 2; se.cnt2 = ecnt2; se.list2 = ecnt2 + 2;
+            se.swept = [&](int part, int64_t split) -> int {
+                int rc2;
+                hipEvent_t ev = part == 0 ? c->ev_r[0] : split > 0 ? c->ev_r2 : c->ev_r[0];
+                SK_HIP(hipStreamWaitEvent(c->stream3, ev, 0));
+                if (part == 0) {
+                    if ((rc2 = launch_retry(ecnt, c->stream3, split))) return rc2;
+                } else {
+                    if ((rc2 = split > 0 ? launch_retry(ecnt2, c->stream3, a->nreads - split) : launch_retry(ecnt, c->stream3))) return rc2;
+                    SK_HIP(hipEventRecord(c->ev_r[1], c->stream3));
+                }
+                if (naudit) {
+                    SK_HIP(hipStreamWaitEvent(c->stream4, ev, 0));
+                    const int upto = part == 0 ? (int)(split / audit_period) : naudit;
+                    if ((rc2 = launch_audit(c->stream4, audit_done, upto))) return rc2;
+                    audit_done = upto;
+                    if (part == 1) SK_HIP(hipEventRecord(c->ev_a, c->stream4));
+                }
+                return SK_OK;
+            };
+        }
+        if ((rc = sk_launch_sdtw_screen(c, a, ck, span_q, span2, cnt, cnt + 2, early ? &se : nullptr))) return rc;
         if ((rc = launch_retry())) return rc;
         if (early) {
             SK_HIP(hipStreamWaitEvent(c->stream, c->ev_r[1], 0));
diff --git a/squigglekit_amd/csrc/sk_sdtwq.hip b/squigglekit_amd/csrc/sk_sdtwq.hip
--- a/squigglekit_amd/csrc/sk_sdtwq.hip
+++ b/squigglekit_amd/csrc/sk_sdtwq.hip
@@ -949,8 +949,9 @@
 }
 
 int sk_launch_sdtw_screen(sk_ctx *c, const sk_sdtw_args *a, int ck, int span, int span2,
-                          int32_t *d_retry_cnt, int32_t *d_retry, int32_t *d_early_cnt, int32_t *d_early)
-{
+                          int32_t *d_retry_cnt, int32_t *d_retry, const sk_screen_early *early)
+{
+    int32_t *const d_early_cnt = early ? early->cnt : nullptr, *const d_early = early ? early->list : nullptr;
     const int N = a->nmotif;
     int L, R;
     screen_layout(N, a->nreads, a->max_len, &L, &R);
@@ -980,34 +981,68 @@
     const size_t ck_bytes = (size_t)L * ((R + 3) / 2) * sizeof(unsigned);
     const size_t per_read = (size_t)(nck > 0 ? nck : 1) * ck_bytes + lq_stride * sizeof(unsigned) + state_bytes +
                             (size_t)(nck + 1) * L * sizeof(unsigned) + 64;
-    int64_t chunk;
+    int64_t seg_reads = 0;
+    if (const char *e = sk_tune("SK_DTW_SEG_READS")) { const long long v = atoll(e); if (v > 0) seg_reads = v; }
+    const bool nopipe = sk_tune("SK_DTW_NOPIPE") != nullptr;
+    std::vector<int64_t> segs;
+    const auto up256 = [](size_t b) { return (b + 255) & ~(size_t)255; };
+    int64_t chunk, segcap = 0;
+    int nslices = 1;
+    size_t sl_ckpt = 0, sl_lastq = 0, sl_wstate = 0, sl_lsum = 0;
     while (true) {
         chunk = sk_dtw_chunk_reads(per_read, a->nreads);
-        rc = sk_reserve(c, &c->ckpt, (size_t)chunk * (size_t)(nck > 0 ? nck : 1) * ck_bytes);
-        if (!rc) rc = sk_reserve(c, &c->lastq, (size_t)chunk * lq_stride * sizeof(unsigned));
-        if (!rc) rc = sk_reserve(c, &c->wstate, (size_t)chunk * state_bytes);
-        if (!rc) rc = sk_reserve(c, &c->lsum, (size_t)chunk * (size_t)(nck + 1) * L * sizeof(unsigned));
+        segcap = chunk;
+        nslices = 1;
+        if (!nopipe && sk_dtw_segments(chunk, L, seg_reads, &segs) > 1) {
+            segcap = segs[0];
+            nslices = (int)segs.size() < SK_DTW_SLICES ? (int)segs.size() : SK_DTW_SLICES;
+        }
+        sl_ckpt = up256((size_t)segcap * (size_t)(nck > 0 ? nck : 1) * ck_bytes);
+        sl_lastq = up256((size_t)segcap * lq_stride * sizeof(unsigned));
+        sl_wstate = up256((size_t)segcap * state_bytes);
+        sl_lsum = up256((size_t)segcap * (size_t)(nck + 1) * L * sizeof(unsigned));
+        rc = sk_reserve(c, &c->ckpt, nslices * sl_ckpt);
+        if (!rc) rc = sk_reserve(c, &c->lastq, nslices * sl_lastq);
+        if (!rc) rc = sk_reserve(c, &c->wstate, nslices * sl_wstate);
+        if (!rc) rc = sk_reserve(c, &c->lsum, nslices * sl_lsum);
         if (rc != SK_ERR_NOMEM || chunk <= 1024) break;
         sk_dtw_scratch_shrink(0);
     }
     if (rc) return rc;
-    if ((rc = sk_reserve(c, &c->qflag, (size_t)chunk * sizeof(int32_t)))) return rc;
-    if ((rc = sk_reserve(c, &c->wrec, (size_t)chunk * sizeof(wrec)))) return rc;
-    if ((rc = sk_reserve(c, &c->wrecq, (size_t)chunk * sizeof(wrec)))) return rc;
+    const size_t sl_qflag = up256((size_t)segcap * sizeof(int32_t)), sl_wrec = up256((size_t)segcap * sizeof(wrec));
+    if ((rc = sk_reserve(c, &c->qflag, nslices * sl_qflag))) return rc;
+    if ((rc = sk_reserve(c, &c->wrec, nslices * sl_wrec))) return rc;
+    if ((rc = sk_reserve(c, &c->wrecq, nslices * sl_wrec))) return rc;
     int sort_min = 32768;
     if (const char *e = sk_tune("SK_DTW_SORT_MIN")) { const int v = atoi(e); if (v > 0) sort_min = v; }
-    const bool sorted = chunk >= sort_min && sk_tune("SK_DTW_NOSORT") == nullptr;
-    if (sorted && (rc = sk_reserve(c, &c->order, ((size_t)chunk + ORDER_BINS) * sizeof(int32_t)))) return rc;
+    const int sort_min_piped = sort_min < 8192 ? sort_min : 8192;
+    const bool nosort = sk_tune("SK_DTW_NOSORT") != nullptr;
+    const bool sorted = chunk >= sort_min && !nosort;
+    const size_t sl_order = up256(((size_t)segcap + ORDER_BINS) * sizeof(int32_t));
+    if (!nosort && (sorted || nslices > 1) && (rc = sk_reserve(c, &c->order, nslices * sl_order))) return rc;
     const bool tiers = span2 > span;
-    if (tiers && (rc = sk_reserve(c, &c->wsoft, ((size_t)chunk + 1) * sizeof(int32_t)))) return rc;
+    const size_t sl_wsoft = up256(((size_t)segcap + 1) * sizeof(int32_t));
+    if (tiers && (rc = sk_reserve(c, &c->wsoft, nslices * sl_wsoft))) return rc;
     const bool siblings = sk_tune("SK_DTW_NO_SIBLINGS") == nullptr;
-    const int sib_cap = (int)(chunk / 64 + 1024);
+    const int sib_cap = (int)(segcap / 64 + 1024);
+    const size_t sl_sib = up256(16 + (size_t)sib_cap * sizeof(sibrec)), sl_sibout = up256((size_t)sib_cap * sizeof(sk_hit));
+    const size_t sl_sibstate = up256((size_t)sib_cap * (state_bytes + sizeof(wrec)));
     if (siblings) {
-        if ((rc = sk_reserve(c, &c->sib, 16 + (size_t)sib_cap * sizeof(sibrec)))) return rc;
-        if ((rc = sk_reserve(c, &c->sibout, (size_t)sib_cap * sizeof(sk_hit)))) return rc;
-        if ((rc = sk_reserve(c, &c->sibstate, (size_t)sib_cap * (state_bytes + sizeof(wrec))))) return rc;
+        if ((rc = sk_reserve(c, &c->sib, nslices * sl_sib))) return rc;
+        if ((rc = sk_reserve(c, &c->sibout, nslices * sl_sibout))) return rc;
+        if ((rc = sk_reserve(c, &c->sibstate, nslices * sl_sibstate))) return rc;
         if (c->stream3 && !c->ev_s[0])
             for (int i = 0; i < 2; i++) SK_HIP(hipEventCreateWithFlags(&c->ev_s[i], hipEventDisableTiming));
+    }
+    if (nslices > 1 && !c->stream_w) {
+        int pr_least = 0, pr_greatest = 0;
+        SK_HIP(hipDeviceGetStreamPriorityRange(&pr_least, &pr_greatest));
+        SK_HIP(hipStreamCreateWithPriority(&c->stream_w, hipStreamNonBlocking, pr_greatest));
+        for (int i = 0; i < SK_DTW_SLICES; i++) {
+            SK_HIP(hipEventCreateWithFlags(&c->ev_pq[i], hipEventDisableTiming));
+            SK_HIP(hipEventCreateWithFlags(&c->ev_pw[i], hipEventDisableTiming));
+            SK_HIP(hipEventCreateWithFlags(&c->ev_ps[i], hipEventDisableTiming));
+        }
     }
 
     typedef void *(*pick_fn)(int, int, int);
@@ -1017,11 +1052,14 @@
     const int64_t plen = (int64_t)N + maxlen + 2;
     int64_t hint_min = HINT_MIN_READS;
     if (const char *e = sk_tune("SK_DTW_HINT_MIN")) { const int v = atoi(e); if (v > 0) hint_min = v; }
-    const bool hint = a->feed == SK_FEED_I16 && (L == 8 || L == 16) && plen <= HINT_MAX_PLEN && R <= HINT_MAX_R &&
-                      N >= HINT_MIN_N && a->nreads >= hint_min && sk_tune("SK_DTW_NOHINT") == nullptr;
-    sdtw_fn fp1 = fp;
-    if (hint) { fq = (sdtw_fn)sk_sdtwq_pick_hint(P == 0 ? 3 : 0, L, R); fp1 = (sdtw_fn)sk_sdtwq_pick_hint(1, L, R); }
-    if (!fq || !fp || !fp1 || !fw) return sk_fail(SK_ERR_UNSUPPORTED, "no screening kernel for L=%d R=%d", L, R);
+    const bool hint_can = a->feed == SK_FEED_I16 && (L == 8 || L == 16) && plen <= HINT_MAX_PLEN && R <= HINT_MAX_R &&
+                          N >= HINT_MIN_N && sk_tune("SK_DTW_NOHINT") == nullptr;
+    const bool hint_call = hint_can && a->nreads >= hint_min;
+    const sdtw_fn fq_plain = fq;
+    sdtw_fn fq_hint = nullptr, fp_hint = nullptr;
+    if (hint_can) { fq_hint = (sdtw_fn)sk_sdtwq_pick_hint(P == 0 ? 3 : 0, L, R); fp_hint = (sdtw_fn)sk_sdtwq_pick_hint(1, L, R); }
+    if (!fq || !fp || !fw || (hint_can && (!fq_hint || !fp_hint)))
+        return sk_fail(SK_ERR_UNSUPPORTED, "no screening kernel for L=%d R=%d", L, R);
 
     sdtw_kargs k = kargs_of(a);
     k.xlay = (const double *)c->motifw.p; k.xlayq = (const unsigned *)c->motifq.p; k.P = P; k.out = a->out;
@@ -1031,7 +1069,7 @@
     k.wstate = (unsigned *)c->wstate.p; k.wrec = c->wrec.p; k.wrec_q = c->wrecq.p;
     k.early_cnt = d_early_cnt; k.early = d_early;
     k.qplen = (unsigned)plen;
-    k.qerr = hint ? ((unsigned)plen << HINT_T) + HINT_MASK : (unsigned)plen;
+    k.qerr = (unsigned)plen;
     k.wmax = 4 * ck;
     k.lds_wave_words = (64 / L) * ck;
     k.guard = sk_tune("SK_DTW_NOGUARD") ? nullptr : (int32_t *)c->dtwcnt.p + 8;
@@ -1039,7 +1077,6 @@
     if (const char *e = sk_tune("SK_DTW_HOLE")) {
         k.hole = strcmp(e, "qerr1") == 0 ? SK_HOLE_QERR1 : strcmp(e, "fma64") == 0 ? SK_HOLE_FMA64
                : strcmp(e, "fma64x") == 0 ? SK_HOLE_FMA64_UNGUARDED : SK_HOLE_NONE;
-        if (k.hole == SK_HOLE_QERR1) k.qerr = 1;
     }
     if (const char *e = sk_tune("SK_DTW_FORCE_RETRY_PM")) {
         const int pm = atoi(e);
@@ -1065,89 +1102,129 @@
     }
     c->prof_chunks = 0;
     const int reads_per_block = 4 * (64 / L);
+    const auto slice = [](const sk_buf &b, size_t bytes, int s) { return (void *)((char *)b.p + (size_t)s * bytes); };
     for (int64_t r0 = 0; r0 < a->nreads; r0 += chunk) {
-        k.read0 = (int)r0;
-        k.nreads = (int)((a->nreads - r0 < chunk) ? a->nreads - r0 : chunk);
-        const int grid = (k.nreads + reads_per_block - 1) / reads_per_block;
+        const int64_t chunk_n = (a->nreads - r0 < chunk) ? a->nreads - r0 : chunk;
+        const bool last_chunk = r0 + chunk >= a->nreads;
+        segs.assign(1, chunk_n);
+        if (nslices > 1) sk_dtw_segments(chunk_n, L, seg_reads, &segs);
+        const int nseg = (int)segs.size();
+        const bool piped = nseg > 1;
+        hipStream_t sw = piped ? c->stream_w : c->stream;
+        hipStream_t ss = c->stream3 ? c->stream3 : sw;
         if (a->fuse) {
-            k.fz_raw = fz.raw; k.fz_len = fz.len; k.fz_lo = fz.lo; k.fz_hi = fz.hi;
+            k.fz_len = fz.len; k.fz_lo = fz.lo; k.fz_hi = fz.hi;
             k.fz_mode = fz.mode == SK_PREP_ZSCALE ? 1 : 0;
             k.fz_vec = ((((uintptr_t)fz.raw & 15) == 0 && (a->stride % 8) == 0) ? 1 : 0) |
                        ((((uintptr_t)a->samples & 15) == 0 && (a->stride % 8) == 0) ? 2 : 0);
         }
         hipEvent_t *ev = &c->evpool[3 * (size_t)c->prof_chunks];
-        k.sib = nullptr; k.sib_cnt = nullptr; k.sib_out = nullptr; k.tier2 = 0;
-        if (siblings) {
-            SK_HIP(hipMemsetAsync(c->sib.p, 0, 16, c->stream));
-            k.sib_cnt = (int32_t *)c->sib.p; k.sib = (char *)c->sib.p + 16; k.sib_out = (sk_hit *)c->sibout.p;
-            k.sib_cap = sib_cap;
-        }
-        SK_HIP(hipEventRecord(ev[0], c->stream));
-        k.clk = (r0 == 0) ? (unsigned long long *)((char *)c->dtwcnt.p + 16) : nullptr;
-        hipLaunchKernelGGL(fq, dim3(grid), dim3(256), fz_lds, c->stream, k);
-        k.fz_raw = nullptr;
-        if (d_early_cnt && r0 + chunk >= a->nreads) SK_HIP(hipEventRecord(c->ev_r[0], c->stream));
-        SK_HIP(hipGetLastError());
-        if (siblings) {
-            sdtw_kargs ks = k;
-            ks.tier2 = 2; ks.wl_list = nullptr; ks.wl_count = k.sib_cnt; ks.soft = nullptr; ks.soft_cnt = nullptr;
-            ks.span = tiers ? span2 : span; ks.total_ptr = nullptr; ks.nreads = sib_cap;
-            ks.wstate = (unsigned *)c->sibstate.p; ks.wrec = (char *)c->sibstate.p + (size_t)sib_cap * state_bytes;
-            const int sgrid = (sib_cap + reads_per_block - 1) / reads_per_block;
-            hipStream_t ss = c->stream3 ? c->stream3 : c->stream;
-            if (c->stream3) {
-                SK_HIP(hipEventRecord(c->ev_s[0], c->stream));
-                SK_HIP(hipStreamWaitEvent(c->stream3, c->ev_s[0], 0));
-            }
-            hipLaunchKernelGGL(fp, dim3(sgrid), dim3(256), 0, ss, ks);
-            hipLaunchKernelGGL(fw, dim3(sgrid), dim3(256), 0, ss, ks);
+        int64_t s0 = r0;
+        for (int sg = 0; sg < nseg; s0 += segs[sg], sg++) {
+            const int sl = sg % nslices;
+            const bool last_seg = sg + 1 == nseg;
+            const bool hint = last_seg ? hint_call : hint_can;
+            const sdtw_fn fq_s = hint ? fq_hint : fq_plain, fp1 = hint ? fp_hint : fp;
+            k.read0 = (int)s0;
+            k.nreads = (int)segs[sg];
+            const int grid = (k.nreads + reads_per_block - 1) / reads_per_block;
+            k.ckq = (unsigned *)slice(c->ckpt, sl_ckpt, sl); k.lastq = (unsigned *)slice(c->lastq, sl_lastq, sl);
+            k.qflag = (int32_t *)slice(c->qflag, sl_qflag, sl); k.lsum = (unsigned *)slice(c->lsum, sl_lsum, sl);
+            k.wstate = (unsigned *)slice(c->wstate, sl_wstate, sl);
+            k.wrec = slice(c->wrec, sl_wrec, sl); k.wrec_q = slice(c->wrecq, sl_wrec, sl);
+            k.qerr = k.hole == SK_HOLE_QERR1 ? 1u : hint ? ((unsigned)plen << HINT_T) + HINT_MASK : (unsigned)plen;
+            const bool split_last = piped && last_chunk && last_seg && early && early->cnt2;
+            k.early_cnt = split_last ? early->cnt2 : d_early_cnt; k.early = split_last ? early->list2 : d_early;
+            k.span = span; k.wl_list = nullptr; k.wl_count = nullptr; k.soft = nullptr; k.soft_cnt = nullptr; k.total_ptr = nullptr;
+            k.fz_raw = a->fuse ? fz.raw : nullptr;
+            k.sib = nullptr; k.sib_cnt = nullptr; k.sib_out = nullptr; k.tier2 = 0;
+            if (piped && sg >= nslices) SK_HIP(hipStreamWaitEvent(c->stream, c->ev_pw[sl], 0));
+            if (siblings) {
+                void *sb = slice(c->sib, sl_sib, sl);
+                SK_HIP(hipMemsetAsync(sb, 0, 16, c->stream));
+                k.sib_cnt = (int32_t *)sb; k.sib = (char *)sb + 16; k.sib_out = (sk_hit *)slice(c->sibout, sl_sibout, sl);
+                k.sib_cap = sib_cap;
+            }
+            if (sg == 0) SK_HIP(hipEventRecord(ev[0], c->stream));
+            k.clk = (s0 == 0) ? (unsigned long long *)((char *)c->dtwcnt.p + 16) : nullptr;
+            hipLaunchKernelGGL(fq_s, dim3(grid), dim3(256), fz_lds, c->stream, k);
+            k.fz_raw = nullptr;
+            k.clk = nullptr;
+            const bool rel0 = piped && last_chunk && sg + 2 == nseg && early;
+            const bool rel1 = last_chunk && last_seg && early;
+            if (rel0) SK_HIP(hipEventRecord(c->ev_r[0], c->stream));
+            if (rel1) SK_HIP(hipEventRecord(piped ? c->ev_r2 : c->ev_r[0], c->stream));
             SK_HIP(hipGetLastError());
-            if (c->stream3) SK_HIP(hipEventRecord(c->ev_s[1], c->stream3));
-        }
-        SK_HIP(hipEventRecord(ev[1], c->stream));
-        const int32_t *order = nullptr;
-        if (sorted && k.nreads >= sort_min) {
-            order_args oa;
-            oa.rec = (const wrec *)c->wrecq.p; oa.qflag = (const int32_t *)c->qflag.p;
-            oa.nreads = k.nreads; oa.read0 = k.read0; oa.span = span; oa.ck = ck; oa.nck = nck; oa.L = L; oa.wmax = k.wmax;
-            oa.hint = hint ? 1 : 0;
-            oa.hist = (int32_t *)c->order.p; oa.order = oa.hist + ORDER_BINS;
-            SK_HIP(hipMemsetAsync(oa.hist, 0, ORDER_BINS * sizeof(int32_t), c->stream));
-            const int og = (k.nreads + ORDER_TPB * ORDER_IPT - 1) / (ORDER_TPB * ORDER_IPT);
-            hipLaunchKernelGGL(k_order_count, dim3(og), dim3(ORDER_TPB), 0, c->stream, oa);
-            hipLaunchKernelGGL(k_order_scan, dim3(1), dim3(ORDER_BINS), 0, c->stream, oa.hist);
-            hipLaunchKernelGGL(k_order_scatter, dim3(og), dim3(ORDER_TPB), 0, c->stream, oa);
+            if (piped) {
+                SK_HIP(hipEventRecord(c->ev_pq[sl], c->stream));
+                SK_HIP(hipStreamWaitEvent(sw, c->ev_pq[sl], 0));
+            }
+            if (siblings) {
+                sdtw_kargs ks = k;
+                ks.tier2 = 2; ks.wl_list = nullptr; ks.wl_count = k.sib_cnt; ks.soft = nullptr; ks.soft_cnt = nullptr;
+                ks.span = tiers ? span2 : span; ks.total_ptr = nullptr; ks.nreads = sib_cap;
+                ks.wstate = (unsigned *)slice(c->sibstate, sl_sibstate, sl);
+                ks.wrec = (char *)ks.wstate + (size_t)sib_cap * state_bytes;
+                const int sgrid = (sib_cap + reads_per_block - 1) / reads_per_block;
+                if (c->stream3) {
+                    if (!piped) SK_HIP(hipEventRecord(c->ev_s[0], c->stream));
+                    SK_HIP(hipStreamWaitEvent(c->stream3, piped ? c->ev_pq[sl] : c->ev_s[0], 0));
+                }
+                hipLaunchKernelGGL(fp, dim3(sgrid), dim3(256), 0, ss, ks);
+                hipLaunchKernelGGL(fw, dim3(sgrid), dim3(256), 0, ss, ks);
+                SK_HIP(hipGetLastError());
+                if (c->stream3) SK_HIP(hipEventRecord(piped ? c->ev_ps[sl] : c->ev_s[1], c->stream3));
+            }
+            if (rel0 && (rc = early->swept(0, s0 + segs[sg]))) return rc;
+            if (rel1 && piped && (rc = early->swept(1, s0))) return rc;
+            if (last_seg) SK_HIP(hipEventRecord(ev[1], c->stream));
+            const int32_t *order = nullptr;
+            if (!nosort && (piped ? k.nreads >= sort_min_piped : (sorted && k.nreads >= sort_min))) {
+                order_args oa;
+                oa.rec = (const wrec *)k.wrec_q; oa.qflag = (const int32_t *)k.qflag;
+                oa.nreads = k.nreads; oa.read0 = k.read0; oa.span = span; oa.ck = ck; oa.nck = nck; oa.L = L; oa.wmax = k.wmax;
+                oa.hint = hint ? 1 : 0;
+                oa.hist = (int32_t *)slice(c->order, sl_order, sl); oa.order = oa.hist + ORDER_BINS;
+                SK_HIP(hipMemsetAsync(oa.hist, 0, ORDER_BINS * sizeof(int32_t), sw));
+                const int og = (k.nreads + ORDER_TPB * ORDER_IPT - 1) / (ORDER_TPB * ORDER_IPT);
+                hipLaunchKernelGGL(k_order_count, dim3(og), dim3(ORDER_TPB), 0, sw, oa);
+                hipLaunchKernelGGL(k_order_scan, dim3(1), dim3(ORDER_BINS), 0, sw, oa.hist);
+                hipLaunchKernelGGL(k_order_scatter, dim3(og), dim3(ORDER_TPB), 0, sw, oa);
+                SK_HIP(hipGetLastError());
+                order = oa.order;
+            }
+            k.tier2 = 0;
+            if (tiers) {
+                int32_t *soft = (int32_t *)slice(c->wsoft, sl_wsoft, sl);
+                SK_HIP(hipMemsetAsync(soft, 0, sizeof(int32_t), sw));
+                k.span = span; k.wl_list = order; k.wl_count = nullptr; k.soft = soft + 1; k.soft_cnt = soft;
+                hipLaunchKernelGGL(fp1, dim3(grid), dim3(256), 0, sw, k);
+                hipLaunchKernelGGL(fw, dim3(grid), dim3(256), 0, sw, k);
+                SK_HIP(hipGetLastError());
+                k.span = span2; k.wl_list = soft + 1; k.wl_count = soft; k.soft = nullptr; k.soft_cnt = nullptr;
+                k.tier2 = 1;
+                k.total_ptr = (int32_t *)c->dtwcnt.p + 1;
+            } else {
+                k.wl_list = order; k.wl_count = nullptr;
+            }
+            hipLaunchKernelGGL(tiers ? fp : fp1, dim3(grid), dim3(256), 0, sw, k);
+            k.total_ptr = nullptr;
+            hipLaunchKernelGGL(fw, dim3(grid), dim3(256), 0, sw, k);
             SK_HIP(hipGetLastError());
-            order = oa.order;
-        }
-        k.tier2 = 0;
-        if (tiers) {
-            int32_t *soft = (int32_t *)c->wsoft.p;
-            SK_HIP(hipMemsetAsync(soft, 0, sizeof(int32_t), c->stream));
-            k.span = span; k.wl_list = order; k.wl_count = nullptr; k.soft = soft + 1; k.soft_cnt = soft;
-            hipLaunchKernelGGL(fp1, dim3(grid), dim3(256), 0, c->stream, k);
-            hipLaunchKernelGGL(fw, dim3(grid), dim3(256), 0, c->stream, k);
-            SK_HIP(hipGetLastError());
-            k.span = span2; k.wl_list = soft + 1; k.wl_count = soft; k.soft = nullptr; k.soft_cnt = nullptr;
-            k.tier2 = 1;
-            k.total_ptr = (int32_t *)c->dtwcnt.p + 1;
-        } else {
-            k.wl_list = order; k.wl_count = nullptr;
-        }
-        hipLaunchKernelGGL(tiers ? fp : fp1, dim3(grid), dim3(256), 0, c->stream, k);
-        k.total_ptr = nullptr;
-        hipLaunchKernelGGL(fw, dim3(grid), dim3(256), 0, c->stream, k);
-        SK_HIP(hipGetLastError());
-        if (siblings) {
-            if (c->stream3) SK_HIP(hipStreamWaitEvent(c->stream, c->ev_s[1], 0));
-            hipLaunchKernelGGL(k_sib_combine, dim3((sib_cap + 255) / 256), dim3(256), 0, c->stream,
-                               (const sibrec *)k.sib, (const int32_t *)k.sib_cnt, sib_cap, (const sk_hit *)k.sib_out, k.out,
-                               d_retry, d_retry_cnt, (int32_t *)c->dtwcnt.p + 8 + 6);
-            SK_HIP(hipGetLastError());
-        }
+            if (siblings) {
+                if (c->stream3) SK_HIP(hipStreamWaitEvent(sw, piped ? c->ev_ps[sl] : c->ev_s[1], 0));
+                hipLaunchKernelGGL(k_sib_combine, dim3((sib_cap + 255) / 256), dim3(256), 0, sw,
+                                   (const sibrec *)k.sib, (const int32_t *)k.sib_cnt, sib_cap, (const sk_hit *)k.sib_out, k.out,
+                                   d_retry, d_retry_cnt, (int32_t *)c->dtwcnt.p + 8 + 6);
+                SK_HIP(hipGetLastError());
+            }
+            if (piped) SK_HIP(hipEventRecord(c->ev_pw[sl], sw));
+        }
+        if (piped) SK_HIP(hipStreamWaitEvent(c->stream, c->ev_pw[(nseg - 1) % nslices], 0));
         SK_HIP(hipEventRecord(ev[2], c->stream));
-        c->prof_reads[c->prof_chunks < 64 ? c->prof_chunks : 63] = k.nreads;
+        c->prof_reads[c->prof_chunks < 64 ? c->prof_chunks : 63] = (int)chunk_n;
         c->prof_chunks++;
+        if (last_chunk && !piped && early && (rc = early->swept(1, 0))) return rc;
     }
     return SK_OK;
 }
```

Result: slower. 16.54 million (-5.9%).
